# uzh-rpg/ess

Hardware: AMD Instinct MI355X
Metric: UDA train-step throughput (voxel grids/s = N*B*T/step_time) (higher is better)
Workload: dtype f16 forward / bf16 backward

## Files before the change

### ess_amd/copies.py

```python
import collections

import torch

_ATTR = 'ess_copies'


class Copies:
    __slots__ = ('stamp', 'c8', 'h16', 'f32c8', 'pair', 'mixed', 'unwritten')

    def __init__(self, stamp, unwritten):
        self.stamp, self.unwritten = stamp, unwritten
        self.c8 = self.h16 = self.f32c8 = self.pair = self.mixed = None


_NONE = collections.namedtuple('NoCopies', Copies.__slots__)(None, None, None, None, None, None, False)
_UNWRITTEN = _NONE._replace(unwritten=True)


def of(t):
    r = getattr(t, _ATTR, None)
    if r is None:
        return _NONE
    if r.stamp == t._version:
        return r
    return _UNWRITTEN if r.unwritten else _NONE


def attach(t, **fields):
    r = getattr(t, _ATTR, None)
    if r is None or r.stamp != t._version:
        r = Copies(t._version, r is not None and r.unwritten)
        setattr(t, _ATTR, r)
    for k, v in fields.items():
        setattr(r, k, v)
    return t


def placeholder(shape, device, **fields):
    return attach(torch.empty((), dtype=torch.float32, device=device).expand(*shape), unwritten=True, **fields)


def carry(dst, src, *names):
    r = of(src)
    found = {k: getattr(r, k) for k in names if getattr(r, k) is not None and getattr(r, k) is not False}
    return attach(dst, **found) if found else dst


def require_fp32(t):
    if of(t).unwritten:
        from .hip import EssHipError
        raise EssHipError('this tensor was produced as a BF16_C8 copy only (lean recurrent state / internal activation); '
                          'its fp32 values do not exist')
    return t
```

### ess_amd/csrc/conv_bf16.hip

```cpp
#include "conv_bf16_common.h"
#include <atomic>

namespace {

using namespace essconv;

__global__ void pack_weights_bf16_kernel(const float* w, const float* w2, __bf16* out, int64_t total, int cot, int ck,
                                         int n_chunks, int ks, int cin, int cout, int epi, int hid, int w_kind, int split, int f16) {
  const int64_t i = (int64_t)blockIdx.x * blockDim.x + threadIdx.x;
  if (i >= total) return;
  int64_t t = i;
  const int kp = t & 7; t >>= 3;
  const int col = t % cot; t /= cot;
  const int cb8 = ck >> 3;
  const int cb = t % cb8; t /= cb8;
  const int tap = t % (ks * ks); t /= ks * ks;
  int lo = 0;
  if (split) { lo = (int)(t & 1); t >>= 1; }
  const int ch = t % n_chunks;
  const int ct = t / n_chunks;
  const int c = ch * ck + cb * 8 + kp;
  int sel;
  const int row = map_row(ct * cot + col, epi, hid, cout, &sel);
  float v = 0.f;
// ... 205 lines not shown
bool wide_pick(const EssConvDesc* d, const EssConvPlan& pl, const Geom& g, const ConvKArgs& a, bool c8, WidePick* out) {
  if (d->epilogue != ESS_EPI_LINEAR) return wide_pick_recurrent(d, pl, g, a, c8, out);
  const int mode = wide_mode();
  if (!mode || !c8 || a.fmt_out != ESS_FMT_BF16_C8 || d->epilogue != ESS_EPI_LINEAR || a.out_bf) return false;
  const bool relu = d->act == ESS_ACT_RELU, res = a.residual != nullptr;
  if (!(d->act == ESS_ACT_NONE || relu)) return false;
  if (a.out_f16 && (relu || res)) return false;
  if (a.f16 && res) return false;
  if (d->out_split > 0 && (relu || res || a.out_f16 || (d->out_split & 15) || a.scale)) return false;
  const double kappa = tuning().kappa;
  const int mb = pl.cout_tile / 32;
  const int std_tiles = g.tiles_x * g.tiles_y * pl.n_cout_tiles * d->N;
  const double c_std = std_cost(std_tiles, pl.cout_tile, 2) * (mb == 1 ? tuning().narrow_tile : 1.0);
  const int cands[4][2] = {{2, 2}, {2, 1}, {1, 2}, {1, 1}};
  double best = 1e300;
  for (const auto& c : cands) {
    const int mbw = c[0], cw = c[1], cot = mbw * cw * 32;
    if ((mb == 2) != (cot >= 64) || mb > 2) continue;
    if (d->C_out % cot) continue;
    if (d->out_split > 0 && (d->out_split % (mbw * 32))) continue;
    int th, tw;
    conv_bf16_wide_tile(mbw, cw, &th, &tw);
    const int tx = ceil_div(d->W_out, tw), ty = ceil_div(d->H_out, th);
    const int tiles = tx * ty * (d->C_out / cot) * d->N;
    const double cost = kappa * ceil_div(tiles, tuning().cus) * (double)cot * th * tw;
    if (cost < best) { best = cost; *out = WidePick{mbw, cw, th, tx, ty, tiles}; }
  }
  if (best >= 1e300) return false;
  return mode >= 2 || best < c_std;
}
}

void conv_bf16_s2d_pick(const EssConvDesc* d, int* cw_out, int* tiles_out, int* tx_out, int* ty_out) {
  const int cus = tuning().cus;
  double best = 1e300;
  *cw_out = 0; *tiles_out = 0; *tx_out = 0; *ty_out = 0;
  for (int cw = 2; cw >= 1; --cw) {
    const int cot = 64 * cw;
    if (d->C_out % cot) continue;
    int th, tw;
    conv_bf16_wide_tile(2, cw, &th, &tw);
    const int tx = ceil_div(d->W_out, tw), ty = ceil_div(d->H_out, th);
    const int tiles = tx * ty * (d->C_out / cot) * d->N;
    const double cost = (double)ceil_div(tiles, cus) * cot * th * tw;
    if (cost < best) { best = cost; *cw_out = cw; *tiles_out = tiles; *tx_out = tx; *ty_out = ty; }
  }
}
bool conv_bf16_s2d_preferred(const EssConvDesc* d) {
  int cw, tiles, tx, ty;
  conv_bf16_s2d_pick(d, &cw, &tiles, &tx, &ty);
  return cw > 0 && 4 * tiles >= 3 * tuning().cus;
}

int conv_bf16_launch(const EssConvDesc* d, const EssConvPlan& pl, const Geom& g, const ConvKArgs& a, hipStream_t st) {
  ESS_CHECK_ARG(g.IH * g.IW <= kpc(d->ksize, d->stride) * 256, "conv(bf16): input tile of %d positions exceeds the staging capacity",
                g.IH * g.IW);
  ESS_CHECK_ARG((int64_t)(d->C0 > d->C1 ? d->C0 : d->C1) * d->H_in * d->W_in * 4 < (int64_t)1 << 31,
                "conv(bf16): one sample of a source must stay below 2 GiB (32-bit buffer offsets)");
  ESS_CHECK_ARG(d->C1 == 0 || (d->C0 % 8) == 0, "conv(bf16): the first source of a concat must have a multiple of 8 channels");
  const dim3 grid((unsigned)(g.tiles_x * g.tiles_y * pl.n_cout_tiles * d->N));
  const int mb = pl.cout_tile / 32;
  const bool c8 = a.fmt0 == ESS_FMT_BF16_C8;
  const bool split_generic = d->ksize == 3 && d->stride == 2 && d->epilogue == ESS_EPI_LINEAR;
  ESS_CHECK_ARG(!a.split || (((ws_enabled() && d->ksize == 3 && d->stride == 1 && pl.ck == 16) || is_paired(d) || split_generic) && !c8 && a.fmt_out == ESS_FMT_F32_NCHW),
                "conv(bf16): split operands run on the 3x3 / stride-1 wave-specialised, the 5x5 tap-paired and the 3x3 / stride-2 generic kernels with fp32 tensors");
  if (c8) ESS_CHECK_ARG((((uintptr_t)a.src0 | (uintptr_t)a.src1) & 15) == 0, "conv(bf16): BF16_C8 sources must be 16-byte aligned");
  if (a.f16)
    ESS_CHECK_ARG(c8 || (is_paired(d) && !a.residual && !a.split && conv_bf16_head_applies(d, pl)),
                  "conv(f16): sources must be F16_C8 tensors (fp32 NCHW only for the 2..5-channel 5x5 head)");
  if (a.f16) ESS_CHECK_ARG(!a.split && d->act != ESS_ACT_SUMPOOL2 && (a.fmt_out == ESS_FMT_F32_NCHW || d->out_split == 0 || d->epilogue != ESS_EPI_LINEAR),
                           "conv(f16): forward forms only");
  if (!c8 && !a.residual && conv_bf16_stem_applies(d, pl)) {
    conv_bf16_launch_stem(d, pl, st, a);
    return ess_launch_status("conv2d_forward(bf16, 7x7 stem)");
  }
  if (is_paired(d) && !c8 && !a.residual && !a.split && conv_bf16_head_applies(d, pl)) {
    conv_bf16_launch_head(d, pl, st, a);
    return ess_launch_status("conv2d_forward(bf16, 5x5 head)");
  }
  if (is_paired(d)) {
    const size_t lds2 = 2 * (size_t)pl.lds_bytes;
    ESS_CHECK_ARG(lds2 <= 160 * 1024, "conv(bf16, 5x5): two stages of %d B exceed the 160 KiB LDS", pl.lds_bytes);
    {
      static const int persist = [] { const char* e = getenv("ESS_WS_PERSIST"); return e ? atoi(e) : 1; }();
      const int by_regs = (d->stride == 2 && mb == 2) ? 1 : 2, by_lds = (int)((160 * 1024) / lds2);
      const int slots = tuning().cus * (by_regs < by_lds ? by_regs : by_lds);
      if (persist && (int)grid.x > slots) {
        ConvKArgs t = a;
        t.persist = 1;
        conv_bf16_launch_pair(d->stride, mb, c8, dim3((unsigned)slots), lds2, st, t);
        return ess_launch_status("conv2d_forward(bf16, tap-paired, persistent)");
      }
    }
    conv_bf16_launch_pair(d->stride, mb, c8, grid, lds2, st, a);
    return ess_launch_status("conv2d_forward(bf16, tap-paired)");
  }
  if (d->mode0 == ESS_SRC_S2D) {
    ESS_CHECK_ARG(c8 && a.fmt_out == ESS_FMT_BF16_C8 && !a.out_bf && !a.residual && !a.out_f16 && pl.ck == 16 && pl.cout_tile == 64 && (!a.hilo || (d->C_out % 64) == 0) &&
                      (d->act == ESS_ACT_NONE || d->act == ESS_ACT_RELU),
                  "conv(bf16, S2D): BF16_C8 in and out, no residual / copy, act in {none, relu}");
    const int cus = tuning().cus;
    int best_cw = 0, best_tiles = 0, best_tx = 0, best_ty = 0;
    conv_bf16_s2d_pick(d, &best_cw, &best_tiles, &best_tx, &best_ty);
    ESS_CHECK_ARG(best_cw > 0, "conv(bf16, S2D): C_out %d is not a multiple of 64", d->C_out);
    ConvKArgs t = a;
    t.tiles_x = best_tx; t.n_tiles = best_tx * best_ty;
    t.persist = best_tiles > cus ? 1 : 0;
    t.slab = pl.cout_tile;
    conv_bf16_launch_wide(2, best_cw, d->epilogue, dim3((unsigned)(best_tiles > cus ? cus : best_tiles)), st, t);
    return ess_launch_status("conv2d_forward(bf16, wide tile, space-to-depth 5x5/s2)");
  }
  static const bool poly_on = [] { const char* e = getenv("ESS_CONV_POLY"); return !(e && e[0] == '0'); }();
  if (poly_on && ws_enabled() && c8 && a.fmt_out == ESS_FMT_BF16_C8 && d->ksize == 3 && d->stride == 1 && d->pad == 1 && pl.ck == 16 &&
      d->mode0 == ESS_SRC_NEAREST_UP2 && d->C1 == 0 && d->epilogue == ESS_EPI_LINEAR && d->out_split == 0 && !a.out_bf &&
      (d->act == ESS_ACT_NONE || d->act == ESS_ACT_RELU) && (d->C_out % 32) == 0 && (d->C0 % 16) == 0 && !(d->H_in & 1) && !(d->W_in & 1) &&
      (pl.cout_tile == 32 || pl.cout_tile == 64)) {
    int th, tw, max_cin;
    conv_bf16_poly_tile(&th, &tw, &max_cin);
    if (d->C0 <= max_cin) {
    ConvKArgs t = a;
    t.Hin = d->H_in >> 1; t.Win = d->W_in >> 1;
    t.tiles_x = ceil_div(t.Win, tw);
    t.n_tiles = t.tiles_x * ceil_div(t.Hin, th);
    t.n_cout_tiles = d->C_out / 32;
    t.slab = pl.cout_tile;
    const int cus = tuning().cus, nct = t.n_cout_tiles, ptiles = t.n_tiles * d->N;
    int per_ct = cus / nct > 0 ? cus / nct : 1;
    if (per_ct > ptiles) per_ct = ptiles;
    t.persist = 1;
    conv_bf16_launch_poly(dim3((unsigned)(per_ct * nct)), st, t);
    return ess_launch_status("conv2d_forward(bf16, polyphase nearest-up2)");
    }
  }
  if (ws_enabled() && d->ksize == 3 && d->stride == 1 && pl.ck == 16) {
    const size_t lds2 = 2 * (size_t)pl.lds_bytes;
    WidePick wp;
    if (wide_pick(d, pl, g, a, c8, &wp)) {
      ConvKArgs t = a;
      t.tiles_x = wp.tiles_x; t.n_tiles = wp.tiles_x * wp.tiles_y;
      const int cus = tuning().cus;
      t.persist = wp.tiles > cus ? 1 : 0;
      t.slab = pl.cout_tile;
      conv_bf16_launch_wide(wp.mbw, wp.cw, d->epilogue, dim3((unsigned)(wp.tiles > cus ? cus : wp.tiles)), st, t);
      return ess_launch_status("conv2d_forward(bf16, wide tile)");
    }
    if (lds2 <= 160 * 1024) {
      static const int persist = [] { const char* e = getenv("ESS_WS_PERSIST"); return e ? atoi(e) : 1; }();
      const int per_cu_lds = (int)((160 * 1024) / lds2), per_cu = (mb == 4 ? 1 : 2) < per_cu_lds ? (mb == 4 ? 1 : 2) : per_cu_lds;
      const int slots = tuning().cus * per_cu;
      if (persist && (int)grid.x > slots) {
        ConvKArgs t = a;
        t.persist = 1;
        conv_bf16_launch_ws(mb, d->epilogue, c8, dim3((unsigned)slots), lds2, st, t);
        return ess_launch_status("conv2d_forward(bf16, wave-specialised, persistent)");
      }
      conv_bf16_launch_ws(mb, d->epilogue, c8, grid, lds2, st, a);
      return ess_launch_status("conv2d_forward(bf16, wave-specialised)");
    }
  }
  const int key = d->ksize * 10 + d->stride;
  ESS_CHECK_ARG(!a.split || split_generic, "conv(bf16): split operands reached the generic tile kernel (k%d s%d, %zu B of LDS for two stages)",
                d->ksize, d->stride, 2 * (size_t)pl.lds_bytes);
  if (c8)
    ESS_CHECK_ARG(d->epilogue == ESS_EPI_LINEAR && (key == 11 || key == 12 || key == 31 || key == 32),
                  "conv(bf16): the generic tile kernel stages BF16_C8 sources for 1x1 and 3x3 LINEAR convolutions only");
  ESS_CHECK_ARG(key == 11 || key == 12 || key == 31 || key == 32 || key == 51 || key == 52 || key == 71 || key == 72,
                "conv: no kernel for k%d s%d", d->ksize, d->stride);
  conv_bf16_launch_generic(key, mb, pl.ck / 8, d->epilogue, c8, grid, pl.lds_bytes, st, a);
  return ess_launch_status("conv2d_forward(bf16)");
}

}
```

### ess_amd/csrc/conv_bf16_wide.hip

```cpp
#include "conv_bf16_common.h"

namespace {

using namespace essconv;

__host__ __device__ constexpr int s2d_ntaps(int q) { return q == 0 ? 9 : (q == 3 ? 4 : 6); }
__host__ __device__ constexpr int s2d_class(int p, int nq) { return p < 2 * nq ? ((p & 1) ? 2 : 0) : ((p & 1) ? 3 : 1); }
__host__ __device__ constexpr int s2d_group(int p, int nq) { return (p < 2 * nq ? p : p - 2 * nq) >> 1; }
constexpr int WIDE_NB = 5;
constexpr int WIDE_RP = 32;
constexpr int WIDE_IW = 18;

template <int MBW, int CW, int EPI = ESS_EPI_LINEAR, bool S2D = false, bool H = false>
__global__ __launch_bounds__(512, 2) void conv_bf16_wide_kernel(const ConvKArgs a) {
  extern __shared__ __attribute__((aligned(16))) u32x4 smem16[];
  constexpr int KS = 3, CB8 = 2, CK = 16, NB = WIDE_NB, RP = WIDE_RP;
  constexpr int PW = 4 / CW;
  constexpr int TH = PW * NB * 2, TW = 16;
  constexpr int IH = TH + 2, IW = WIDE_IW;
  constexpr int PLANE = IH * RP;
  constexpr int COT = MBW * CW * 32;
  constexpr int WSZ = KS * KS * CB8 * COT;
  constexpr int WV = (WSZ + 255) / 256;
  constexpr int NPOS = IH * IW;
  constexpr int KPC = (NPOS + 255) / 256;
  constexpr int BUFSZ = CB8 * PLANE + WSZ;
  const int role = __builtin_amdgcn_readfirstlane(threadIdx.x >> 8);
  const int SLAB = a.slab;
  const int NSLAB = COT / SLAB;
  const int n_ct = a.n_cout_tiles / NSLAB;
  int t_start, t_count, t_first = 0, t_step = 1;
  if (a.persist) {
    const int total = n_ct * a.n_tiles * a.N, q = total >> 3, r = total & 7, xcd = (int)(blockIdx.x & 7);
    t_start = xcd < r ? xcd * (q + 1) : r * (q + 1) + (xcd - r) * q;
    t_count = q + (xcd < r ? 1 : 0);
    t_first = (int)(blockIdx.x >> 3);
    t_step = (int)(gridDim.x >> 3);
  } else {
    t_start = xcd_remap(blockIdx.x, gridDim.x);
    t_count = 1;
  }
#define ESS_TILE_LOOP for (int ti = t_first; ti < t_count; ti += t_step)
#define ESS_TILE_DECODE                                                    \
  const int logical = t_start + ti;                                        \
  const int ct = logical % n_ct;                                           \
  const int sp = logical / n_ct;                                           \
  const int tile = sp % a.n_tiles, n = sp / a.n_tiles;                     \
  const int ty = tile / a.tiles_x, tx = tile - ty * a.tiles_x;             \
  const int y0 = ty * TH, x0 = tx * TW;

  if (role == 1) {
    const int tid = threadIdx.x & 255;
    ESS_TILE_LOOP {
    ESS_TILE_DECODE
    const int iy0 = y0 - a.pad, ix0 = x0 - a.pad;
    const int sh0 = S2D ? 0 : (a.mode0 != ESS_SRC_DIRECT ? 1 : 0), sh1 = a.mode1 != ESS_SRC_DIRECT ? 1 : 0;
    const int Wp0 = S2D ? 2 * a.Win : (a.Win >> sh0), Wp1 = a.Win >> sh1;
    const size_t hw0 = S2D ? (size_t)4 * a.Hin * a.Win : (size_t)(a.Hin >> sh0) * Wp0, hw1 = (size_t)(a.Hin >> sh1) * Wp1;
    const int nb0 = S2D ? (a.C0 >> 5) : ((a.C0 + 7) >> 3), nb1 = (a.C1 + 7) >> 3;
    const int nq = S2D ? (a.n_chunks >> 2) : 1;
    const u32x4* s0 = (const u32x4*)a.src0 + (size_t)n * nb0 * hw0;
    const u32x4* s1 = a.C1 ? (const u32x4*)a.src1 + (size_t)n * nb1 * hw1 : s0;
    unsigned v_pos0[KPC], v_pos1[KPC], v_keep0[KPC], v_keep1[KPC];
    int v_lds[KPC];
#pragma unroll
    for (int k = 0; k < KPC; ++k) {
      const int vi = tid + k * 256;
// ... 201 lines not shown
  {
    ESS_READ_TAP(f0, 0, lds0)
    if constexpr (S2D) {
      const int nq = nch >> 2;
      for (int ch = 0; ch < 2 * nq; ch += 4) {
        ESS_CHUNK(f0, f1, ch)
        ESS_CHUNK6(f1, f0, ch + 1, 1, 3, 4, 6, 7)
        ESS_CHUNK(f1, f0, ch + 2)
        ESS_CHUNK6(f0, f1, ch + 3, 1, 3, 4, 6, 7)
      }
      for (int ch = 2 * nq; ch < nch; ch += 2) {
        ESS_CHUNK6(f0, f1, ch, 1, 2, 3, 4, 5)
        ESS_CHUNK4(f0, f1, ch + 1, 1, 3, 4)
      }
    } else {
    for (int ch = 0; ch < nch; ch += 2) {
      ESS_CHUNK(f0, f1, ch)
      if (ch + 1 < nch) ESS_CHUNK(f1, f0, ch + 1)
    }
    }
    asm volatile("s_waitcnt lgkmcnt(0)" ::: "memory");
  }
#undef ESS_CHUNK4
#undef ESS_CHUNK6
#undef ESS_CHUNK_TAIL_EVEN
#undef ESS_STEP
#undef ESS_READ_TS
#undef ESS_CHUNK
#undef ESS_TIE
#undef ESS_READ_TAP
#undef ESS_WAIT
#undef ESS_MMA
  __builtin_amdgcn_s_setprio(0);
#ifdef ESS_ABLATE
  if (a.deep & 8) continue;
#endif
  if constexpr (EPI == ESS_EPI_LSTM) {
    int pixi[NB];
#pragma unroll
    for (int nb = 0; nb < NB; ++nb) {
      const int y = y0 + ly[nb], x = x0 + ox;
      pixi[nb] = (y < a.Hout && x < a.Wout) ? y * a.Wout + x : -1;
    }
    conv_epilogue_lstm_c8<MBW, NB, H>(a, acc, ct_w, n, half, pixi, (unsigned)(a.Hout * a.Wout));
  } else if constexpr (EPI == ESS_EPI_GRU_UR || EPI == ESS_EPI_GRU_OUT) {
    int pixi[NB];
#pragma unroll
    for (int nb = 0; nb < NB; ++nb) {
      const int y = y0 + ly[nb], x = x0 + ox;
      pixi[nb] = (y < a.Hout && x < a.Wout) ? y * a.Wout + x : -1;
    }
    if constexpr (EPI == ESS_EPI_GRU_UR) conv_epilogue_gru_ur_c8<MBW, NB, H>(a, acc, ct_w, n, half, pixi, (unsigned)(a.Hout * a.Wout));
    else conv_epilogue_gru_out_c8<MBW, NB, H>(a, acc, ct_w, n, half, pixi, (unsigned)(a.Hout * a.Wout));
  } else {
    conv_epilogue_c8_wide<MBW, NB, H>(a, acc, ct_w, n, half, x0 + ox, y0, ly, biased);
  }
  }
#undef ESS_TILE_LOOP
#undef ESS_TILE_DECODE
}

template <int MBW, int CW, int EPI = ESS_EPI_LINEAR, bool S2D = false>
void launch_wide_t(dim3 grid, hipStream_t st, const ConvKArgs& a) {
  constexpr int PW = 4 / CW, TH = PW * WIDE_NB * 2, PLANE = (TH + 2) * WIDE_RP, COT = MBW * CW * 32;
  constexpr size_t lds = 2 * (size_t)(2 * PLANE + 9 * 2 * COT) * 16;
  static_assert(lds <= 160 * 1024, "two stages must fit the 160 KiB LDS");
  if (a.f16) {
    ess_allow_lds(conv_bf16_wide_kernel<MBW, CW, EPI, S2D, true>, lds);
    hipLaunchKernelGGL((conv_bf16_wide_kernel<MBW, CW, EPI, S2D, true>), grid, dim3(512), lds, st, a);
    return;
  }
  ess_allow_lds(conv_bf16_wide_kernel<MBW, CW, EPI, S2D>, lds);
  hipLaunchKernelGGL((conv_bf16_wide_kernel<MBW, CW, EPI, S2D>), grid, dim3(512), lds, st, a);
}

}

namespace essconv {

void conv_bf16_wide_tile(int mbw, int cw, int* th, int* tw) {
  *tw = 16;
  *th = (4 / cw) * WIDE_NB * 2;
  (void)mbw;
}

void conv_bf16_launch_wide(int mbw, int cw, int epi, dim3 grid, hipStream_t st, const ConvKArgs& a) {
  if (a.mode0 == ESS_SRC_S2D) {
    if (cw == 2) launch_wide_t<2, 2, ESS_EPI_LINEAR, true>(grid, st, a);
    else launch_wide_t<2, 1, ESS_EPI_LINEAR, true>(grid, st, a);
    return;
  }
  if (epi == ESS_EPI_LSTM) { launch_wide_t<2, 2, ESS_EPI_LSTM>(grid, st, a); return; }
  if (epi == ESS_EPI_GRU_UR) { launch_wide_t<2, 2, ESS_EPI_GRU_UR>(grid, st, a); return; }
  if (epi == ESS_EPI_GRU_OUT) { launch_wide_t<2, 2, ESS_EPI_GRU_OUT>(grid, st, a); return; }
  if (mbw == 2 && cw == 2) launch_wide_t<2, 2>(grid, st, a);
  else if (mbw == 2 && cw == 1) launch_wide_t<2, 1>(grid, st, a);
  else if (mbw == 1 && cw == 2) launch_wide_t<1, 2>(grid, st, a);
  else launch_wide_t<1, 1>(grid, st, a);
}

}
```

### ess_amd/csrc/conv_bf16_ws.hip

```cpp
#ifdef ESS_CV_TRACE
__device__ unsigned long long g_cv_trace[2048 * 8 * 48];
#define ESS_CT(i_) do { if ((threadIdx.x & 63) == 0 && blockIdx.x < 2048) g_cv_trace[(blockIdx.x * 8 + (threadIdx.x >> 6)) * 48 + (i_)] = __builtin_readcyclecounter(); } while (0)
#define ESS_EPI_STAMP(i_) ESS_CT(i_)
#define ESS_CW(i_) do { if ((threadIdx.x & 63) == 0 && blockIdx.x < 2048) g_cv_trace[(blockIdx.x * 8 + (threadIdx.x >> 6)) * 48 + (i_)] = wall_clock64(); } while (0)
#define ESS_SYNC_ACC(acc_) do { const unsigned long long t0_ = __builtin_readcyclecounter(); __syncthreads(); acc_ += __builtin_readcyclecounter() - t0_; } while (0)
#define ESS_CT_VAL(i_, v_) do { if ((threadIdx.x & 63) == 0 && blockIdx.x < 2048) g_cv_trace[(blockIdx.x * 8 + (threadIdx.x >> 6)) * 48 + (i_)] = (v_); } while (0)
#else
#define ESS_SYNC_ACC(acc_) __syncthreads()
#define ESS_CT_VAL(i_, v_) do { } while (0)
#define ESS_CW(i_) do { } while (0)
#define ESS_CT(i_) do { } while (0)
#endif
#include "conv_bf16_common.h"

namespace {

using namespace essconv;

template <int MB, int EPI, bool SRCBF, bool OUT8 = false, bool H = false>
__global__ __launch_bounds__(512, MB == 4 ? 2 : 4) void conv_bf16_ws_k3s1_kernel(const ConvKArgs a) {
  static_assert(!H || SRCBF, "half operands come as F16_C8 tensors");
  extern __shared__ __attribute__((aligned(16))) u32x4 smem16[];
  constexpr int KS = 3, CB8 = 2, CK = 16;
  constexpr int COT = MB * 32;
  constexpr int KPC = kpc(3, 1);
  constexpr int WSZ = KS * KS * CB8 * COT;
  constexpr int WV = (WSZ + 255) / 256;
  const int role = __builtin_amdgcn_readfirstlane(threadIdx.x >> 8);
  const int tid = threadIdx.x & 255, lane = tid & 63, wave = tid >> 6, half = lane >> 5, p = lane & 31;
  const int BW = 1 << a.bwl, WX = 1 << a.wxl, RB = 32 >> a.bwl;
  const int TW = WX << a.bwl, TH = (4 >> a.wxl) * NBW * RB;
  int t_start, t_count, t_first = 0, t_step = 1;
  if (a.persist) {
    const int total = a.n_cout_tiles * a.n_tiles * a.N, q = total >> 3, r = total & 7, xcd = (int)(blockIdx.x & 7);
    t_start = xcd < r ? xcd * (q + 1) : r * (q + 1) + (xcd - r) * q;
    t_count = q + (xcd < r ? 1 : 0);
    t_first = (int)(blockIdx.x >> 3);
    t_step = (int)(gridDim.x >> 3);
  } else {
    t_start = xcd_remap(blockIdx.x, gridDim.x);
    t_count = 1;
  }
#define ESS_TILE_LOOP for (int ti = t_first; ti < t_count; ti += t_step)
#define ESS_TILE_DECODE                                                    \
  const int logical = t_start + ti;                                        \
  const int ct = logical % a.n_cout_tiles;                                 \
  const int sp = logical / a.n_cout_tiles;                                 \
  const int tile = sp % a.n_tiles, n = sp / a.n_tiles;                     \
  const int ty = tile / a.tiles_x, tx = tile - ty * a.tiles_x;             \
  const int y0 = ty * TH, x0 = tx * TW;
  const int bufsz = CB8 * a.plane + WSZ;
  ESS_CT(0);
  ESS_CW(46);

  if (role == 1 && SRCBF) {
    ESS_TILE_LOOP {
    ESS_TILE_DECODE
    const int iy0 = y0 - a.pad, ix0 = x0 - a.pad;
    const int sh0 = a.mode0 != ESS_SRC_DIRECT ? 1 : 0, sh1 = a.mode1 != ESS_SRC_DIRECT ? 1 : 0;
    const int Wp0 = a.Win >> sh0, Wp1 = a.Win >> sh1;
    const size_t hw0 = (size_t)(a.Hin >> sh0) * Wp0, hw1 = (size_t)(a.Hin >> sh1) * Wp1;
    const int nb0 = (a.C0 + 7) >> 3, nb1 = (a.C1 + 7) >> 3;
    const u32x4* s0 = (const u32x4*)a.src0 + (size_t)n * nb0 * hw0;
    const u32x4* s1 = a.C1 ? (const u32x4*)a.src1 + (size_t)n * nb1 * hw1 : s0;
    unsigned v_pos0[KPC], v_pos1[KPC], v_keep0[KPC], v_keep1[KPC];
    int v_lds[KPC];
    const int npos = a.IH * a.IW;
#pragma unroll
    for (int k = 0; k < KPC; ++k) {
      const int vi = tid + k * 256;
      const int iy = vi / a.IW, ix = vi - iy * a.IW;
      const int gy = iy0 + iy, gx = ix0 + ix;
      const bool in = vi < npos && gy >= 0 && gy < a.Hin && gx >= 0 && gx < a.Win;
      const bool odd = ((gy | gx) & 1) != 0;
// ... 219 lines not shown
    if (ch < 40) ESS_CT(3 + ch);
    const unsigned stage_b = lds0 + (ch & 1) * buf_bytes;
    const unsigned wa = stage_b + w_off + a_base;
    unsigned ba[NBW][KS];
#pragma unroll
    for (int nb = 0; nb < NBW; ++nb)
#pragma unroll
      for (int ky = 0; ky < KS; ++ky) ba[nb][ky] = stage_b + b_base[nb][ky];
    Frags f0, f1;
#define ESS_READ_TAP(F_, TAP_)                                                                                                   \
    {                                                                                                                            \
      constexpr int ky_ = (TAP_) / KS, kx_ = (TAP_) % KS;                                                                        \
      _Pragma("unroll") for (int mb = 0; mb < MB; ++mb)                                                                          \
        asm volatile("ds_read_b128 %0, %1 offset:%2" : "=v"(F_.a[mb]) : "v"(wa + (unsigned)(mb * 32 * 16)), "n"((TAP_) * CB8 * COT * 16)); \
      _Pragma("unroll") for (int nb = 0; nb < NBW; ++nb)                                                                         \
        asm volatile("ds_read_b128 %0, %1 offset:%2" : "=v"(F_.b[nb]) : "v"(ba[nb][ky_]), "n"(kx_ * 16));                       \
    }
#define ESS_WAIT(F_, N_)                                                                                                         \
    {                                                                                                                            \
      if constexpr (MB == 1) asm volatile("s_waitcnt lgkmcnt(%3)" : "+v"(F_.a[0]), "+v"(F_.b[0]), "+v"(F_.b[1]) : "n"(N_));      \
      else if constexpr (MB == 2) asm volatile("s_waitcnt lgkmcnt(%4)" : "+v"(F_.a[0]), "+v"(F_.a[MB > 1 ? 1 : 0]), "+v"(F_.b[0]), "+v"(F_.b[1]) : "n"(N_)); \
      else asm volatile("s_waitcnt lgkmcnt(%6)" : "+v"(F_.a[0]), "+v"(F_.a[MB > 1 ? 1 : 0]), "+v"(F_.a[MB > 2 ? 2 : 0]), "+v"(F_.a[MB > 3 ? 3 : 0]), "+v"(F_.b[0]), "+v"(F_.b[1]) : "n"(N_)); \
    }
#define ESS_MMA(F_)                                                                                                              \
    _Pragma("unroll") for (int mb = 0; mb < MB; ++mb)                                                                            \
      _Pragma("unroll") for (int nb = 0; nb < NBW; ++nb)                                                                         \
        acc[mb][nb] = ess_mfma16<H>(F_.a[mb], F_.b[nb], acc[mb][nb]);
    constexpr int NR = MB + NBW;
#ifdef ESS_ABLATE
    if (a.deep & 2) { __syncthreads(); continue; }
#endif
    ESS_READ_TAP(f0, 0)
    ESS_READ_TAP(f1, 1) ESS_WAIT(f0, NR) ESS_MMA(f0)
    ESS_READ_TAP(f0, 2) ESS_WAIT(f1, NR) ESS_MMA(f1)
    ESS_READ_TAP(f1, 3) ESS_WAIT(f0, NR) ESS_MMA(f0)
    ESS_READ_TAP(f0, 4) ESS_WAIT(f1, NR) ESS_MMA(f1)
    ESS_READ_TAP(f1, 5) ESS_WAIT(f0, NR) ESS_MMA(f0)
    ESS_READ_TAP(f0, 6) ESS_WAIT(f1, NR) ESS_MMA(f1)
    ESS_READ_TAP(f1, 7) ESS_WAIT(f0, NR) ESS_MMA(f0)
    ESS_READ_TAP(f0, 8) ESS_WAIT(f1, NR) ESS_MMA(f1)
    ESS_WAIT(f0, 0) ESS_MMA(f0)
#undef ESS_READ_TAP
#undef ESS_WAIT
#undef ESS_MMA
    if (ch == nvc_c - 1) ESS_CT(44);
    ESS_SYNC_ACC(cbar_acc);
  }
  ESS_CT_VAL(42, cbar_acc);
  ESS_CT(45);
  __builtin_amdgcn_s_setprio(0);
#ifdef ESS_ABLATE
  if (a.deep & 8) continue;
#endif
  if constexpr (OUT8) conv_epilogue_c8<MB, H>(a, acc, ct, n, half, x0 + lx, y0, ly, biased);
  else conv_epilogue<MB, EPI, false, H>(a, acc, ct, n, half, x0 + lx, y0, ly, biased);
  ESS_CT(47);
  if constexpr (EPI != ESS_EPI_LSTM) ESS_CW(43);
  }
#undef ESS_TILE_LOOP
#undef ESS_TILE_DECODE
}


template <int MB, bool SRCBF>
void launch_ws(int epi, dim3 grid, size_t lds, hipStream_t st, const ConvKArgs& a) {
  if constexpr (SRCBF) {
    if (a.f16) {
#define ESS_WSH(E_, O8_) { ess_allow_lds(conv_bf16_ws_k3s1_kernel<MB, E_, true, O8_, true>, lds); hipLaunchKernelGGL((conv_bf16_ws_k3s1_kernel<MB, E_, true, O8_, true>), grid, dim3(512), lds, st, a); }
      if (a.fmt_out == ESS_FMT_BF16_C8) ESS_WSH(ESS_EPI_LINEAR, true)
      else if (epi == ESS_EPI_LSTM) ESS_WSH(ESS_EPI_LSTM, false)
      else if (epi == ESS_EPI_GRU_UR) ESS_WSH(ESS_EPI_GRU_UR, false)
      else if (epi == ESS_EPI_GRU_OUT) ESS_WSH(ESS_EPI_GRU_OUT, false)
      else ESS_WSH(ESS_EPI_LINEAR, false)
#undef ESS_WSH
      return;
    }
  }
  if (a.fmt_out == ESS_FMT_BF16_C8) {
    ess_allow_lds(conv_bf16_ws_k3s1_kernel<MB, ESS_EPI_LINEAR, SRCBF, true>, lds);
    hipLaunchKernelGGL((conv_bf16_ws_k3s1_kernel<MB, ESS_EPI_LINEAR, SRCBF, true>), grid, dim3(512), lds, st, a);
    return;
  }
#define ESS_WS(E_) { ess_allow_lds(conv_bf16_ws_k3s1_kernel<MB, E_, SRCBF>, lds); hipLaunchKernelGGL((conv_bf16_ws_k3s1_kernel<MB, E_, SRCBF>), grid, dim3(512), lds, st, a); }
  switch (epi) {
    case ESS_EPI_LSTM: ESS_WS(ESS_EPI_LSTM) break;
    case ESS_EPI_GRU_UR: ESS_WS(ESS_EPI_GRU_UR) break;
    case ESS_EPI_GRU_OUT: ESS_WS(ESS_EPI_GRU_OUT) break;
    default: ESS_WS(ESS_EPI_LINEAR) break;
  }
#undef ESS_WS
}
template <bool SRCBF>
void launch_ws_mb(int mb, int epi, dim3 grid, size_t lds, hipStream_t st, const ConvKArgs& a) {
  if (mb == 4) launch_ws<4, SRCBF>(epi, grid, lds, st, a);
  else if (mb == 2) launch_ws<2, SRCBF>(epi, grid, lds, st, a);
  else launch_ws<1, SRCBF>(epi, grid, lds, st, a);
}
}

namespace essconv {

void conv_bf16_launch_ws(int mb, int epi, bool c8, dim3 grid, size_t lds, hipStream_t st, const ConvKArgs& a) {
  if (c8) launch_ws_mb<true>(mb, epi, grid, lds, st, a);
  else launch_ws_mb<false>(mb, epi, grid, lds, st, a);
}

}

#ifdef ESS_CV_TRACE
extern "C" int ess_debug_conv_trace(unsigned long long* host_out, size_t n) {
  (void)hipMemset((void*)nullptr, 0, 0);
  return (int)hipMemcpyFromSymbol(host_out, HIP_SYMBOL(g_cv_trace), n * sizeof(unsigned long long));
}
extern "C" int ess_debug_conv_trace_clear() {
  void* p = nullptr;
  if (hipGetSymbolAddress(&p, HIP_SYMBOL(g_cv_trace)) != hipSuccess) return -1;
  return (int)hipMemset(p, 0, sizeof(unsigned long long) * 2048 * 8 * 48);
}
#endif
// ... 1 lines not shown
```

### ess_amd/csrc/conv_common.h

```cpp
#pragma once
#include "common.h"
#include <stdlib.h>

#ifndef ESS_EPI_AUX
#define ESS_EPI_AUX 2
#endif
#ifndef ESS_GRU_AUX
#define ESS_GRU_AUX 2
#endif
#ifndef ESS_C8_AUX
#define ESS_C8_AUX 0
#endif
namespace essconv {

constexpr int NBW = 2;

struct ConvKArgs {
  const float* src0;
  const float* src1;
  const void* wpk;
  const float* scale;
  const float* shift;
  const float* residual;
  const float* aux0;
  const float* aux1;
  float* out;
  float* out2;
  int N, Hin, Win, C0, C1, mode0, mode1;
  int Cout, Hout, Wout, pad;
  int bwl, wxl, tiles_x, n_tiles, n_cout_tiles;
  int IH, IW, row_pitch, par_off, plane;
  int ck, n_chunks;
  int act, hid, out_split;
  void* out_bf;
  int fmt0, fmt1;
  int fmt_out;
  int fmt_res;
  int out_f16;
  int persist;
  int slab;
  int split;
  int deep;
  int f16;
  int hilo;
};

template <bool H> __device__ __forceinline__ uint2 ess_cvt4(float v0, float v1, float v2, float v3);
template <bool H> __device__ __forceinline__ void ess_up4(uint2 r, float (&f)[4]);


#ifndef ESS_EPI_STAMP
#define ESS_EPI_STAMP(i_) do { } while (0)
#endif
typedef __amdgpu_buffer_rsrc_t ess_rsrc;
constexpr unsigned ESS_OOB = 0x80000000u;
__device__ __forceinline__ ess_rsrc ess_make_rsrc(const void* p, size_t bytes) {
  return __builtin_amdgcn_make_buffer_rsrc((void*)p, 0, (int)(unsigned)bytes, 0x00020000);
}
__device__ __forceinline__ _Float16 ess_f16_sat(float v) {
  const float c = __builtin_amdgcn_fmed3f(v, -65504.f, 65504.f);
  return (_Float16)(v != v ? v : c);
}
template <> __device__ __forceinline__ uint2 ess_cvt4<false>(float v0, float v1, float v2, float v3) {
  typedef __bf16 bf16x4 __attribute__((ext_vector_type(4)));
  bf16x4 b;
  b[0] = (__bf16)v0; b[1] = (__bf16)v1; b[2] = (__bf16)v2; b[3] = (__bf16)v3;
  return __builtin_bit_cast(uint2, b);
}
template <> __device__ __forceinline__ uint2 ess_cvt4<true>(float v0, float v1, float v2, float v3) {
  typedef _Float16 f16x4 __attribute__((ext_vector_type(4)));
  f16x4 h;
  h[0] = ess_f16_sat(v0); h[1] = ess_f16_sat(v1); h[2] = ess_f16_sat(v2); h[3] = ess_f16_sat(v3);
  return __builtin_bit_cast(uint2, h);
}
__device__ __forceinline__ uint2 ess_cvt4_lo(float v0, float v1, float v2, float v3) {
  typedef _Float16 f16x4 __attribute__((ext_vector_type(4)));
  f16x4 h;
  h[0] = (_Float16)(v0 - (float)ess_f16_sat(v0)); h[1] = (_Float16)(v1 - (float)ess_f16_sat(v1));
  h[2] = (_Float16)(v2 - (float)ess_f16_sat(v2)); h[3] = (_Float16)(v3 - (float)ess_f16_sat(v3));
  return __builtin_bit_cast(uint2, h);
}
template <> __device__ __forceinline__ void ess_up4<false>(uint2 r, float (&f)[4]) {
  typedef __bf16 bf16x4 __attribute__((ext_vector_type(4)));
  const bf16x4 b = __builtin_bit_cast(bf16x4, r);
#pragma unroll
  for (int i = 0; i < 4; ++i) f[i] = (float)b[i];
}
template <> __device__ __forceinline__ void ess_up4<true>(uint2 r, float (&f)[4]) {
  typedef _Float16 f16x4 __attribute__((ext_vector_type(4)));
  const f16x4 b = __builtin_bit_cast(f16x4, r);
#pragma unroll
  for (int i = 0; i < 4; ++i) f[i] = (float)b[i];
}
__device__ __forceinline__ float ess_bload(ess_rsrc r, unsigned voff, unsigned soff) {
  return __builtin_bit_cast(float, __builtin_amdgcn_raw_buffer_load_b32(r, (int)voff, (int)soff, 0));
}
__device__ __forceinline__ void ess_bstore(float v, ess_rsrc r, unsigned voff, unsigned soff) {
// ... 559 lines not shown
            ess_up4<H>(rr, rf);
#pragma unroll
            for (int i = 0; i < 4; ++i) v[nb][i] += rf[i];
          }
#pragma unroll
          for (int i = 0; i < 4; ++i) {
            if (relu) v[nb][i] = fmaxf(v[nb][i], 0.f);
            if (c0 + i >= c_out) v[nb][i] = 0.f;
          }
        }
        if (pool && blk < nb_first) {
#pragma unroll
          for (int i = 0; i < 4; ++i) {
            if (rows1) {
              v[0][i] = v[0][i] + v[1][i];
              v[0][i] += xor1(v[0][i]);
            } else {
#pragma unroll
              for (int nb = 0; nb < NBW; ++nb) {
                v[nb][i] = v[nb][i] + __shfl_xor(v[nb][i], BW, 64);
                v[nb][i] += xor1(v[nb][i]);
              }
            }
          }
        }
#pragma unroll
        for (int nb = 0; nb < NBW; ++nb) {
          if (H || a.out_f16) {
            pk[jj][nb] = ess_cvt4<true>(v[nb][0], v[nb][1], v[nb][2], v[nb][3]);
          } else {
            pk[jj][nb] = ess_cvt4<false>(v[nb][0], v[nb][1], v[nb][2], v[nb][3]);
          }
        }
      }
      const bool to1 = myblk < nb_first;
#pragma unroll
      for (int nb = 0; nb < NBW; ++nb) {
        const auto s0 = __builtin_amdgcn_permlane32_swap(pk[0][nb].x, pk[1][nb].x, false, false);
        const auto s1 = __builtin_amdgcn_permlane32_swap(pk[0][nb].y, pk[1][nb].y, false, false);
        const u32x4e vec = {s0[0], s1[0], s0[1], s1[1]};
        if (blk0 < nb_first) {
          const unsigned o = (to1 && st1_16[nb] != ESS_OOB) ? (unsigned)myblk * HW1 * 16u + st1_16[nb] : ESS_OOB;
          __builtin_amdgcn_raw_buffer_store_b128(vec, r_o1, (int)o, 0, 0);
        }
        if (split > 0 && blk0 + 1 >= nb_first) {
          const unsigned o = (!to1 && myblk < nb_all && pix16[nb] != ESS_OOB) ? (unsigned)(myblk - nb_first) * HW * 16u + pix16[nb] : ESS_OOB;
          __builtin_amdgcn_raw_buffer_store_b128(vec, r_o2, (int)o, 0, 0);
        }
      }
    }
  }
}

template <int MB, bool SC, bool SH, bool F16, bool RELU, bool RES, int NB, bool H = false, bool HILO = false>
__device__ __forceinline__ void conv_epilogue_c8_plain(const ConvKArgs& a, f32x16 (&acc)[MB][NB], int ct, int n, int half,
                                                       int x, int y0, const int (&ly)[NB]) {
  static_assert(!HILO || H, "a [hi | lo] output is a half tensor");
  typedef unsigned int u32x4e __attribute__((ext_vector_type(4)));
  constexpr int COT = MB * 32;
  const unsigned HW = (unsigned)(a.Hout * a.Wout);
  const int nblk = a.Cout >> 3;
  const ess_rsrc r_o = ess_make_rsrc((const char*)a.out + (size_t)n * (HILO ? 2 : 1) * nblk * HW * 16, (size_t)(HILO ? 2 : 1) * nblk * HW * 16);
  const ess_rsrc r_rs = ess_make_rsrc((const char*)(RES ? a.residual : a.out) + (size_t)n * nblk * HW * 16, RES ? (size_t)nblk * HW * 16 : 0);
  unsigned pix16[NB];
#pragma unroll
  for (int nb = 0; nb < NB; ++nb) {
    const int y = y0 + ly[nb];
    pix16[nb] = ((y < a.Hout) & (x < a.Wout)) ? (unsigned)(y * a.Wout + x) * 16u : ESS_OOB;
  }
#pragma unroll
  for (int mb = 0; mb < MB; ++mb) {
    const int rowbase = ct * COT + mb * 32;
    float4 scv[4], shv[4];
    u32x4e rva[2][NB];
    if constexpr (SC || SH || RES) {
      asm volatile("" ::: "memory");
#pragma unroll
      for (int j = 0; j < 4; ++j) {
        const int c0 = rowbase + j * 8 + 4 * half;
        if constexpr (SC) scv[j] = *(const float4*)(a.scale + c0);
        if constexpr (SH) shv[j] = *(const float4*)(a.shift + c0);
      }
      if constexpr (RES) {
#pragma unroll
        for (int jh = 0; jh < 2; ++jh)
#pragma unroll
          for (int nb = 0; nb < NB; ++nb) {
            const unsigned pl = (unsigned)((rowbase >> 3) + 2 * jh + half) * HW * 16u;
            rva[jh][nb] = __builtin_amdgcn_raw_buffer_load_b128(r_rs, (int)(pix16[nb] != ESS_OOB ? pl + pix16[nb] : ESS_OOB), 0, 0);
          }
      }
    }
#pragma unroll
    for (int jp = 0; jp < 4; jp += 2) {
      uint2 pk[2][NB];
      uint2 pl[HILO ? 2 : 1][HILO ? NB : 1];
      uint2 rr[2][NB];
      if constexpr (RES) {
#pragma unroll
        for (int nb = 0; nb < NB; ++nb) {
          const u32x4e rv = rva[jp >> 1][nb];
          const auto s0 = __builtin_amdgcn_permlane32_swap(rv[0], rv[2], false, false);
          const auto s1 = __builtin_amdgcn_permlane32_swap(rv[1], rv[3], false, false);
          rr[0][nb] = make_uint2(s0[0], s1[0]);
          rr[1][nb] = make_uint2(s0[1], s1[1]);
        }
      }
#pragma unroll
      for (int jj = 0; jj < 2; ++jj) {
        const int j = jp + jj;
#pragma unroll
        for (int nb = 0; nb < NB; ++nb) {
          float v[4];
#pragma unroll
          for (int i = 0; i < 4; ++i) v[i] = acc[mb][nb][4 * j + i];
          if constexpr (SC && SH) {
            v[0] = v[0] * scv[j].x + shv[j].x; v[1] = v[1] * scv[j].y + shv[j].y; v[2] = v[2] * scv[j].z + shv[j].z; v[3] = v[3] * scv[j].w + shv[j].w;
          } else if constexpr (SC) {
            v[0] *= scv[j].x; v[1] *= scv[j].y; v[2] *= scv[j].z; v[3] *= scv[j].w;
          } else if constexpr (SH) {
            v[0] += shv[j].x; v[1] += shv[j].y; v[2] += shv[j].z; v[3] += shv[j].w;
          }
          if constexpr (RES) {
            float rf[4];
            ess_up4<H>(rr[jj][nb], rf);
#pragma unroll
            for (int i = 0; i < 4; ++i) v[i] += rf[i];
          }
          if constexpr (RELU) {
#pragma unroll
            for (int i = 0; i < 4; ++i) v[i] = fmaxf(v[i], 0.f);
          }
          pk[jj][nb] = ess_cvt4<F16 || H>(v[0], v[1], v[2], v[3]);
          if constexpr (HILO) pl[jj][nb] = ess_cvt4_lo(v[0], v[1], v[2], v[3]);
        }
      }
      const unsigned plane = (unsigned)((rowbase >> 3) + jp + half) * HW * 16u;
#pragma unroll
      for (int nb = 0; nb < NB; ++nb) {
        const auto s0 = __builtin_amdgcn_permlane32_swap(pk[0][nb].x, pk[1][nb].x, false, false);
        const auto s1 = __builtin_amdgcn_permlane32_swap(pk[0][nb].y, pk[1][nb].y, false, false);
        const u32x4e vec = {s0[0], s1[0], s0[1], s1[1]};
        __builtin_amdgcn_raw_buffer_store_b128(vec, r_o, (int)(pix16[nb] != ESS_OOB ? plane + pix16[nb] : ESS_OOB), 0, ESS_C8_AUX);
        if constexpr (HILO) {
          const auto t0 = __builtin_amdgcn_permlane32_swap(pl[0][nb].x, pl[1][nb].x, false, false);
          const auto t1 = __builtin_amdgcn_permlane32_swap(pl[0][nb].y, pl[1][nb].y, false, false);
          const u32x4e vlo = {t0[0], t1[0], t0[1], t1[1]};
          __builtin_amdgcn_raw_buffer_store_b128(vlo, r_o, (int)(pix16[nb] != ESS_OOB ? plane + (unsigned)nblk * HW * 16u + pix16[nb] : ESS_OOB), 0, ESS_C8_AUX);
        }
      }
    }
  }
}

template <int MB, bool POOL, int NB>
__device__ __forceinline__ void conv_epilogue_c8_dgrad(const ConvKArgs& a, f32x16 (&acc)[MB][NB], int ct, int n, int half,
                                                       int x, int y0, const int (&ly)[NB]) {
  static_assert(!POOL || NB == 2, "the one-row pooled pairing assumes two pixel blocks per wave");
  typedef __bf16 bf16x4 __attribute__((ext_vector_type(4)));
  typedef unsigned int u32x4e __attribute__((ext_vector_type(4)));
  constexpr int COT = MB * 32;
  const unsigned HW = (unsigned)(a.Hout * a.Wout);
  const int split = a.out_split;
  const int nb_first = (split > 0 ? split : a.Cout) >> 3, nb_second = split > 0 ? (a.Cout - split) >> 3 : 0;
  const int Wl = a.Wout >> 1;
  const unsigned HW1 = POOL ? (unsigned)((a.Hout >> 1) * Wl) : HW;
  const ess_rsrc r_o1 = ess_make_rsrc((const char*)a.out + (size_t)n * nb_first * HW1 * 16, (size_t)nb_first * HW1 * 16);
  const ess_rsrc r_o2 = ess_make_rsrc(split > 0 ? (const char*)a.out2 + (size_t)n * nb_second * HW * 16 : (const char*)a.out,
                                      split > 0 ? (size_t)nb_second * HW * 16 : 0);
  unsigned pix16[NB];
#pragma unroll
  for (int nb = 0; nb < NB; ++nb) {
    const int y = y0 + ly[nb];
    pix16[nb] = ((y < a.Hout) & (x < a.Wout)) ? (unsigned)(y * a.Wout + x) * 16u : ESS_OOB;
  }
  unsigned st_pool = ESS_OOB;
  if constexpr (POOL) {
    const int y = y0 + ly[0];
    if ((y < a.Hout) & (x < a.Wout) & !(x & 1) & !(y & 1)) st_pool = (unsigned)((y >> 1) * Wl + (x >> 1)) * 16u;
  }
  auto xor1 = [](float f) {
    return __builtin_bit_cast(float, __builtin_amdgcn_update_dpp(0, __builtin_bit_cast(int, f), 0xB1, 0xf, 0xf, true));
  };
#pragma unroll
  for (int mb = 0; mb < MB; ++mb) {
    const int rowbase = ct * COT + mb * 32;
#pragma unroll
    for (int jp = 0; jp < 4; jp += 2) {
      const int blk0 = (rowbase >> 3) + jp;
      const bool first = blk0 < nb_first;
      if (POOL && first) {
        uint2 pk[2];
#pragma unroll
        for (int jj = 0; jj < 2; ++jj) {
          bf16x4 b;
#pragma unroll
          for (int i = 0; i < 4; ++i) {
            float p = acc[mb][0][4 * (jp + jj) + i] + acc[mb][1][4 * (jp + jj) + i];
            p += xor1(p);
            b[i] = (__bf16)p;
          }
// ... 85 lines not shown
    else conv_epilogue_c8_sel<MB, false, false, H>(a, acc, ct, n, half, x, y0, ly);
  }
  return;
#endif
  if (biased) {
    conv_epilogue_c8_impl<MB, false, false>(a, acc, ct, n, half, x, y0, ly);
  } else if (a.scale) {
    if (a.shift) conv_epilogue_c8_impl<MB, true, true>(a, acc, ct, n, half, x, y0, ly);
    else conv_epilogue_c8_impl<MB, true, false>(a, acc, ct, n, half, x, y0, ly);
  } else {
    if (a.shift) conv_epilogue_c8_impl<MB, false, true>(a, acc, ct, n, half, x, y0, ly);
    else conv_epilogue_c8_impl<MB, false, false>(a, acc, ct, n, half, x, y0, ly);
  }
}

template <int MB, bool SC, bool SH, int NB, bool H = false>
__device__ __forceinline__ void conv_epilogue_c8_wide_sel(const ConvKArgs& a, f32x16 (&acc)[MB][NB], int ct, int n, int half, int x,
                                                          int y0, const int (&ly)[NB]) {
  const bool relu = a.act == ESS_ACT_RELU, res = a.residual != nullptr;
  if constexpr (H) {
    if (a.hilo) {
      if (relu) conv_epilogue_c8_plain<MB, SC, SH, true, true, false, NB, true, true>(a, acc, ct, n, half, x, y0, ly);
      else conv_epilogue_c8_plain<MB, SC, SH, true, false, false, NB, true, true>(a, acc, ct, n, half, x, y0, ly);
    } else {
      if (relu) conv_epilogue_c8_plain<MB, SC, SH, true, true, false, NB, true>(a, acc, ct, n, half, x, y0, ly);
      else conv_epilogue_c8_plain<MB, SC, SH, true, false, false, NB, true>(a, acc, ct, n, half, x, y0, ly);
    }
    return;
  }
  if constexpr (!SC && !SH) {
    if (a.out_split > 0) { conv_epilogue_c8_dgrad<MB, false>(a, acc, ct, n, half, x, y0, ly); return; }
  }
  if (a.out_f16) {
    conv_epilogue_c8_plain<MB, SC, SH, true, false, false>(a, acc, ct, n, half, x, y0, ly);
  } else if (res) {
    if (relu) conv_epilogue_c8_plain<MB, SC, SH, false, true, true>(a, acc, ct, n, half, x, y0, ly);
    else conv_epilogue_c8_plain<MB, SC, SH, false, false, true>(a, acc, ct, n, half, x, y0, ly);
  } else {
    if (relu) conv_epilogue_c8_plain<MB, SC, SH, false, true, false>(a, acc, ct, n, half, x, y0, ly);
    else conv_epilogue_c8_plain<MB, SC, SH, false, false, false>(a, acc, ct, n, half, x, y0, ly);
  }
}
template <int MB, int NB, bool H = false>
__device__ __forceinline__ void conv_epilogue_c8_wide(const ConvKArgs& a, f32x16 (&acc)[MB][NB], int ct, int n, int half, int x,
                                                      int y0, const int (&ly)[NB], bool biased) {
  if (biased) {
    conv_epilogue_c8_wide_sel<MB, false, false, NB, H>(a, acc, ct, n, half, x, y0, ly);
  } else if (a.scale) {
    if (a.shift) conv_epilogue_c8_wide_sel<MB, true, true, NB, H>(a, acc, ct, n, half, x, y0, ly);
    else conv_epilogue_c8_wide_sel<MB, true, false, NB, H>(a, acc, ct, n, half, x, y0, ly);
  } else {
    if (a.shift) conv_epilogue_c8_wide_sel<MB, false, true, NB, H>(a, acc, ct, n, half, x, y0, ly);
    else conv_epilogue_c8_wide_sel<MB, false, false, NB, H>(a, acc, ct, n, half, x, y0, ly);
  }
}

template <int MB, int NB, bool H = false>
__device__ __forceinline__ void conv_epilogue_lstm_c8(const ConvKArgs& a, f32x16 (&acc)[MB][NB], int ct, int n, int half,
                                                      const int (&pixi)[NB], unsigned HW) {
  typedef unsigned int u32x4c __attribute__((ext_vector_type(4)));
  const int nbh = a.hid >> 3;
  const int ncp = (H && a.hilo) ? 2 : 1;
  const size_t state_b = (size_t)nbh * HW * 32;
  const ess_rsrc r_prev = ess_make_rsrc(a.aux0 ? (const char*)(a.aux0 + (size_t)n * nbh * 8 * HW) : (const char*)a.out2, a.aux0 ? state_b : 0);
  const ess_rsrc r_c = ess_make_rsrc(a.out2 + (size_t)n * nbh * 8 * HW, state_b);
  const ess_rsrc r_h = ess_make_rsrc(a.out ? a.out + (size_t)n * nbh * 8 * HW : a.out2, a.out ? state_b : 0);
  const ess_rsrc r_hb = ess_make_rsrc(a.out_bf ? (const char*)a.out_bf + (size_t)n * ncp * nbh * HW * 16 : (const char*)a.out2, a.out_bf ? (size_t)ncp * nbh * HW * 16 : 0);
  unsigned vo[MB][NB];
  u32x4c cp[MB][NB];
#pragma unroll
  for (int mb = 0; mb < MB; ++mb)
#pragma unroll
    for (int nb = 0; nb < NB; ++nb) {
      vo[mb][nb] = pixi[nb] >= 0 ? ((unsigned)(ct * MB + mb) * HW + (unsigned)pixi[nb]) * 32u + 16u * half : ESS_OOB;
      cp[mb][nb] = __builtin_amdgcn_raw_buffer_load_b128(r_prev, (int)vo[mb][nb], 0, ESS_EPI_AUX);
    }
  __builtin_amdgcn_sched_barrier(0);
  float igc[MB][NB][4], gf[MB][NB][4], go[MB][NB][4];
#pragma unroll
  for (int mb = 0; mb < MB; ++mb)
#pragma unroll
    for (int nb = 0; nb < NB; ++nb)
#pragma unroll
      for (int jj = 0; jj < 4; ++jj) {
        igc[mb][nb][jj] = ess_sigmoid(acc[mb][nb][jj]) * ess_tanh(acc[mb][nb][12 + jj]);
        gf[mb][nb][jj] = ess_sigmoid(acc[mb][nb][4 + jj]);
        go[mb][nb][jj] = ess_sigmoid(acc[mb][nb][8 + jj]);
      }
  float hn[MB][NB][4];
#pragma unroll
  for (int mb = 0; mb < MB; ++mb)
#pragma unroll
    for (int nb = 0; nb < NB; ++nb) {
      u32x4c cv;
#pragma unroll
      for (int jj = 0; jj < 4; ++jj) {
        const float cprev = __builtin_bit_cast(float, (unsigned)cp[mb][nb][jj]);
        const float cn = gf[mb][nb][jj] * cprev + igc[mb][nb][jj];
        cv[jj] = __builtin_bit_cast(unsigned, cn);
        hn[mb][nb][jj] = go[mb][nb][jj] * ess_tanh(cn);
      }
      __builtin_amdgcn_raw_buffer_store_b128(cv, r_c, (int)vo[mb][nb], 0, ESS_EPI_AUX);
    }
  if (a.out) {
#pragma unroll
    for (int mb = 0; mb < MB; ++mb)
// ... 435 lines not shown
__device__ __forceinline__ int map_row(int prow, int epi, int hid, int cout, int* sel) {
  *sel = 0;
  if (epi == ESS_EPI_LSTM) {
    const int b = prow >> 5, q = (prow & 31) >> 3, j = prow & 7;
    const int hc = b * 8 + j;
    return hc < hid ? q * hid + hc : -1;
  }
  if (epi == ESS_EPI_GRU_UR) {
    const int b = prow >> 5, q = (prow & 31) >> 3, j = prow & 7;
    const int hc = b * 16 + (q >> 1) * 8 + j;
    *sel = q & 1;
    return hc < hid ? hc : -1;
  }
  return prow < cout ? prow : -1;
}

static __global__ void pack_weights_kernel(const float* w, const float* w2, float* out, int64_t total, int cot, int ck,
                                    int n_chunks, int ks, int cin, int cout, int epi, int hid, int w_kind) {
  const int64_t i = (int64_t)blockIdx.x * blockDim.x + threadIdx.x;
  if (i >= total) return;
  int64_t t = i;
  const int col = t % cot; t /= cot;
  const int cb = t % ck; t /= ck;
  const int tap = t % (ks * ks); t /= ks * ks;
  const int ch = t % n_chunks;
  const int ct = t / n_chunks;
  const int c = ch * ck + cb;
  int sel;
  const int row = map_row(ct * cot + col, epi, hid, cout, &sel);
  float v = 0.f;
  if (row >= 0 && c < cin) {
    const int ky = tap / ks, kx = tap - ky * ks;
    const float* src = sel ? w2 : w;
    if (w_kind == ESS_W_CONV) {
      v = src[(((size_t)row * cin + c) * ks + ky) * ks + kx];
    } else {
      const int rows_src = (epi == ESS_EPI_GRU_UR) ? hid : cout;
      v = src[(((size_t)c * rows_src + row) * ks + (ks - 1 - ky)) * ks + (ks - 1 - kx)];
    }
  }
  out[i] = v;
}

static __global__ void pack_rows_kernel(const float* v, const float* v2, float fill, float* out, int rows_padded, int epi,
                                 int hid, int cout) {
  const int i = blockIdx.x * blockDim.x + threadIdx.x;
  if (i >= rows_padded) return;
  int sel;
  const int row = map_row(i, epi, hid, cout, &sel);
  out[i] = row >= 0 ? (sel ? v2[row] : v[row]) : fill;
}


int conv_bf16_launch(const EssConvDesc* d, const EssConvPlan& pl, const Geom& g, const ConvKArgs& a, hipStream_t st);
int conv_bf16_pack_weights(const EssConvDesc* d, const EssConvPlan& pl, int w_kind, const float* w, const float* w2, void* packed,
                           hipStream_t st, bool split = false, bool f16 = false);
int conv_bf16_pack_weights_multi(const EssConvDesc* descs, const int32_t* kinds, const float* const* w, void* const* packed, int count,
                                 hipStream_t st);
void conv_bf16_s2d_pick(const EssConvDesc* d, int* cw, int* tiles, int* tiles_x, int* tiles_y);
bool conv_bf16_s2d_preferred(const EssConvDesc* d);

}
```

### ess_amd/csrc/conv_fwd.hip

```cpp
#include "conv_common.h"

namespace {

using namespace essconv;

constexpr int kpc32(int ks, int s) { return stage_kpc(ks, s); }
constexpr unsigned OOB32 = 0x80000000u;

template <int KS, int S, int MB, int EPI, int CB>
__global__ __launch_bounds__(256) void conv_f32_kernel(const ConvKArgs a) {
  extern __shared__ __attribute__((aligned(16))) float smem[];
  constexpr int COT = MB * 32;
  constexpr int KPC = kpc32(KS, S);
  constexpr int WSZ = KS * KS * CB * COT;
  constexpr int WV = (WSZ / 4 + 255) / 256;
  const int tid = threadIdx.x, lane = tid & 63, wave = tid >> 6, half = lane >> 5, p = lane & 31;
  const int BW = 1 << a.bwl, WX = 1 << a.wxl, RB = 32 >> a.bwl;
  const int TW = WX << a.bwl, TH = (4 >> a.wxl) * NBW * RB;
  const int logical = xcd_remap(blockIdx.x, gridDim.x);
  const int ct = logical % a.n_cout_tiles;
  const int sp = logical / a.n_cout_tiles;
  const int tile = sp % a.n_tiles, n = sp / a.n_tiles;
  const int ty = tile / a.tiles_x, tx = tile - ty * a.tiles_x;
  const int y0 = ty * TH, x0 = tx * TW;
// ... 137 lines not shown
  if (rc) return rc;
  ESS_CHECK_ARG(plan != nullptr, "conv: null plan");
  const ResolvedDesc rd = resolve_compute(d);
  make_plan(&rd.d, plan, rd.split);
  return ESS_OK;
}

extern "C" int ess_conv2d_s2d_preferred(const EssConvDesc* d) {
  if (validate(d) != ESS_OK || d->mode0 != ESS_SRC_S2D) return 0;
  return conv_bf16_s2d_preferred(d) ? 1 : 0;
}

extern "C" int ess_conv2d_pack_weights(const EssConvDesc* d, int w_kind, const float* w, const float* w2, void* packed,
                                       ess_stream_t stream) {
  int rc = validate(d);
  if (rc) return rc;
  ESS_CHECK_ARG(w && packed, "pack_weights: null pointer");
  ESS_CHECK_ARG(d->epilogue != ESS_EPI_GRU_UR || w2, "pack_weights: GRU_UR needs the reset-gate weight as w2");
  ESS_CHECK_ARG(w_kind == ESS_W_CONV || w_kind == ESS_W_TRANSPOSED || w_kind == ESS_W_CONV5_S2D, "pack_weights: bad w_kind");
  ESS_CHECK_ARG((w_kind == ESS_W_CONV5_S2D) == (d->mode0 == ESS_SRC_S2D), "pack_weights: ESS_W_CONV5_S2D goes with an ESS_SRC_S2D descriptor, and only with one");
  const ResolvedDesc rd = resolve_compute(d);
  d = &rd.d;
  EssConvPlan pl;
  make_plan(d, &pl, rd.split);
  if (is_bf16(d)) return conv_bf16_pack_weights(d, pl, w_kind, w, w2, packed, (hipStream_t)stream, rd.split, rd.f16);
  const int64_t total = pl.packed_elems;
  hipLaunchKernelGGL(pack_weights_kernel, dim3((unsigned)ceil_div64(total, 256)), dim3(256), 0, (hipStream_t)stream, w, w2,
                     (float*)packed, total, pl.cout_tile, pl.ck, pl.n_chunks, d->ksize, d->C0 + d->C1, d->C_out, d->epilogue,
                     d->hidden, w_kind);
  return ess_launch_status("pack_weights");
}

extern "C" int ess_conv2d_pack_weights_multi(const EssConvDesc* descs, const int32_t* w_kinds, const float* const* w,
                                             void* const* packed, int32_t count, ess_stream_t stream) {
  ESS_CHECK_ARG(descs && w_kinds && w && packed && count > 0, "pack_weights_multi: bad arguments");
  return conv_bf16_pack_weights_multi(descs, w_kinds, w, packed, count, (hipStream_t)stream);
}

extern "C" int ess_conv2d_pack_rows(const EssConvDesc* d, const float* v, const float* v2, float fill, float* packed,
                                    ess_stream_t stream) {
  int rc = validate(d);
  if (rc) return rc;
  ESS_CHECK_ARG(v && packed, "pack_rows: null pointer");
  ESS_CHECK_ARG(d->epilogue != ESS_EPI_GRU_UR || v2, "pack_rows: GRU_UR needs the reset-gate vector as v2");
  const ResolvedDesc rd = resolve_compute(d);
  d = &rd.d;
  EssConvPlan pl;
  make_plan(d, &pl, rd.split);
  hipLaunchKernelGGL(pack_rows_kernel, dim3(ceil_div(pl.rows_padded, 256)), dim3(256), 0, (hipStream_t)stream, v, v2, fill,
                     packed, pl.rows_padded, d->epilogue, d->hidden, d->C_out);
  return ess_launch_status("pack_rows");
}

extern "C" int ess_conv2d_forward(const EssConvDesc* d, const void* src0, const void* src1, const void* packed_w,
                                  const float* scale, const float* shift, const void* residual, const float* aux0,
                                  const float* aux1, void* out, void* out2, void* out_bf16, ess_stream_t stream) {
  EssConvDesc dcopy;
  bool out_f16 = false;
  if (d && d->fmt_out == ESS_FMT_F16_C8 && d->compute != ESS_COMPUTE_F16) {
    ESS_CHECK_ARG(d->act != ESS_ACT_SUMPOOL2 && d->out_split == 0 && (d->fmt_res == ESS_FMT_F32_NCHW || d->fmt_res == ESS_FMT_BF16_C8),
                  "conv: an F16_C8 output takes no SUMPOOL2 / out_split; a residual comes as BF16_C8");
    dcopy = *d;
    dcopy.fmt_out = ESS_FMT_BF16_C8;
    if (residual) dcopy.fmt_res = ESS_FMT_BF16_C8;
    d = &dcopy;
    out_f16 = true;
  }
  int rc = validate(d);
  if (rc) return rc;
  const ResolvedDesc rd = resolve_compute(d);
  d = &rd.d;
  ESS_CHECK_ARG(src0 && packed_w, "conv: null pointer");
  ESS_CHECK_ARG(d->mode0 != ESS_SRC_S2D || (d->fmt0 == ESS_FMT_BF16_C8 && d->fmt_out == ESS_FMT_BF16_C8), "conv: an ESS_SRC_S2D source is a BF16_C8 tensor, and so is the output");
  ESS_CHECK_ARG(out || (out_bf16 && d->out_split == 0 && (d->epilogue == ESS_EPI_LINEAR || d->epilogue == ESS_EPI_LSTM || d->epilogue == ESS_EPI_GRU_OUT)),
                "conv: `out` may only be NULL when the BF16_C8 copy is requested (LINEAR / LSTM / GRU_OUT epilogues)");
  ESS_CHECK_ARG(d->C1 == 0 || src1, "conv: second source missing");
  if (d->epilogue != ESS_EPI_LINEAR) ESS_CHECK_ARG(shift && !scale && !residual, "conv: a recurrent epilogue takes a bias (shift) and no scale / residual");
  if (d->epilogue == ESS_EPI_LSTM) ESS_CHECK_ARG(out2, "conv: the LSTM epilogue needs the second output (c')");
  if (d->epilogue == ESS_EPI_GRU_UR) ESS_CHECK_ARG(out2 || out_bf16 || !aux0, "conv: GRU_UR needs an output for r*h (out2 or out_bf16)");
  if (d->epilogue == ESS_EPI_GRU_OUT) ESS_CHECK_ARG(aux1, "conv: GRU_OUT needs u (aux1); h_prev (aux0) may be NULL = zeros");
  if (d->out_split > 0) ESS_CHECK_ARG(out2, "conv: out_split needs out2");
  if (out_bf16)
    ESS_CHECK_ARG(d->compute == ESS_COMPUTE_BF16 && d->out_split == 0, "conv: the BF16_C8 output copy exists for bf16 compute, no out_split");
  if (d->act == ESS_ACT_SUMPOOL2)
    ESS_CHECK_ARG(out && !scale && !residual && !out_bf16, "conv: SUMPOOL2 takes no scale / residual / BF16_C8 copy");
  if (d->fmt_out == ESS_FMT_BF16_C8) {
    ESS_CHECK_ARG(out && !out_bf16, "conv: a BF16_C8 output goes to `out` (no separate copy)");
    ESS_CHECK_ARG(((((uintptr_t)out) | ((uintptr_t)out2) | ((uintptr_t)residual)) & 15) == 0, "conv: BF16_C8 tensors must be 16-byte aligned");
  }
  ESS_CHECK_ARG(!residual || d->fmt_res == d->fmt_out, "conv: the residual must come in the output's format");
  EssConvPlan pl;
  make_plan(d, &pl, rd.split);
  ESS_CHECK_ARG(pl.lds_bytes <= 160 * 1024, "conv: LDS tile %d B exceeds 160 KiB", pl.lds_bytes);
  if (d->epilogue == ESS_EPI_GRU_UR && d->act == ESS_GRU_U_F16 && d->fmt_out == ESS_FMT_F32_C8)
    ESS_CHECK_ARG(shift && d->fmt0 == ESS_FMT_BF16_C8 && (d->hidden % (pl.cout_tile / 2)) == 0 && out && !out2 && (!aux0 || d->fmt_res == ESS_FMT_F32_C8),
                  "conv(GRU_UR): an F16_C8 update gate (ESS_GRU_U_F16 with channel-blocked outputs) needs BF16_C8 sources, a bias, hidden %% %d == 0, "
                  "no fp32 r*h output and a channel-blocked h_prev", pl.cout_tile / 2);
  const Geom g = choose_geom(d);
  ConvKArgs a{};
  a.src0 = (const float*)src0; a.src1 = (const float*)src1; a.wpk = packed_w;
  a.out_bf = out_bf16; a.fmt0 = d->fmt0; a.fmt1 = d->C1 ? d->fmt1 : d->fmt0; a.scale = scale; a.shift = shift; a.residual = (const float*)residual;
  a.aux0 = aux0; a.aux1 = aux1; a.out = (float*)out; a.out2 = (float*)out2; a.fmt_out = d->fmt_out; a.fmt_res = d->fmt_res;
#ifdef ESS_ABLATE
  { static const int abl = [] { const char* b = getenv("ESS_WS_ABL"); return b ? atoi(b) & ~1 : 0; }(); a.deep = abl; }
#endif
  a.out_f16 = out_f16 ? 1 : 0;
  a.split = rd.split ? 1 : 0;
  a.f16 = rd.f16 ? 1 : 0;
  a.hilo = rd.hilo ? 1 : 0;
  if (rd.hilo && d->epilogue == ESS_EPI_LINEAR)
    ESS_CHECK_ARG(!residual && (d->C_out % pl.cout_tile) == 0 && d->fmt_out == ESS_FMT_BF16_C8, "conv(f16): a [hi | lo] output takes no residual and whole channel tiles");
  if (rd.hilo && d->epilogue == ESS_EPI_GRU_OUT)
    ESS_CHECK_ARG(out_bf16 && shift && d->fmt_res == ESS_FMT_F32_C8 && aux1 && (!out || d->fmt_out == ESS_FMT_F32_C8) && (d->hidden % pl.cout_tile) == 0,
                  "conv(f16, GRU_OUT): a [hi | lo] copy of h' exists in the straight-line form only (channel-blocked states, whole tiles of hidden channels)");
  if (rd.hilo && d->epilogue == ESS_EPI_LSTM)
    ESS_CHECK_ARG(out_bf16 && shift && d->fmt_out == ESS_FMT_F32_C8 && (!aux0 || d->fmt_res == ESS_FMT_F32_C8) && (d->hidden % (8 * (pl.cout_tile / 32))) == 0 && pl.cout_tile >= 64,
                  "conv(f16, LSTM): a [hi | lo] copy of h' exists in the lean form only (channel-blocked cell states, whole hidden blocks per tile)");
  a.N = d->N; a.Hin = d->H_in; a.Win = d->W_in; a.C0 = d->C0; a.C1 = d->C1; a.mode0 = d->mode0; a.mode1 = d->mode1;
  a.Cout = d->C_out; a.Hout = d->H_out; a.Wout = d->W_out; a.pad = d->pad;
  a.bwl = g.bwl; a.wxl = g.wxl; a.tiles_x = g.tiles_x; a.n_tiles = g.tiles_x * g.tiles_y; a.n_cout_tiles = pl.n_cout_tiles;
  a.IH = g.IH; a.IW = g.IW; a.row_pitch = g.row_pitch; a.par_off = g.par_off; a.plane = g.plane;
  a.ck = pl.ck; a.n_chunks = pl.n_chunks; a.act = d->act; a.hid = d->hidden; a.out_split = d->out_split;
  hipStream_t st = (hipStream_t)stream;
  if (is_bf16(d)) return conv_bf16_launch(d, pl, g, a, st);
  ESS_CHECK_ARG(g.IH * g.IW <= kpc32(d->ksize, d->stride) * 256, "conv: input tile of %d positions exceeds the staging capacity",
                g.IH * g.IW);
  ESS_CHECK_ARG((int64_t)(d->C0 > d->C1 ? d->C0 : d->C1) * d->H_in * d->W_in * 4 < (int64_t)1 << 31,
                "conv: one sample of a source must stay below 2 GiB (32-bit buffer offsets)");
  const dim3 grid((unsigned)(g.tiles_x * g.tiles_y * pl.n_cout_tiles * d->N));
  const int mb = pl.cout_tile / 32;
  const int key = d->ksize * 10 + d->stride;
  switch (key) {
    case 11: launch_mb<1, 1>(mb, pl.ck, d->epilogue, grid, pl.lds_bytes, st, a); break;
    case 12: launch_mb<1, 2>(mb, pl.ck, d->epilogue, grid, pl.lds_bytes, st, a); break;
    case 31: launch_mb<3, 1>(mb, pl.ck, d->epilogue, grid, pl.lds_bytes, st, a); break;
    case 32: launch_mb<3, 2>(mb, pl.ck, d->epilogue, grid, pl.lds_bytes, st, a); break;
    case 51: launch_mb<5, 1>(mb, pl.ck, d->epilogue, grid, pl.lds_bytes, st, a); break;
    case 52: launch_mb<5, 2>(mb, pl.ck, d->epilogue, grid, pl.lds_bytes, st, a); break;
    case 71: launch_mb<7, 1>(mb, pl.ck, d->epilogue, grid, pl.lds_bytes, st, a); break;
    case 72: launch_mb<7, 2>(mb, pl.ck, d->epilogue, grid, pl.lds_bytes, st, a); break;
    default: ess_set_error("conv: no kernel for k%d s%d", d->ksize, d->stride); return ESS_ENOTSUP;
  }
  return ess_launch_status("conv2d_forward");
}
```

### ess_amd/csrc/norm_c8.hip

```cpp
#include <atomic>
#include "common.h"
#include <stdlib.h>

#ifndef ESS_REDUCE1_U
#define ESS_REDUCE1_U 4
#endif
namespace {

typedef unsigned int u32x4n __attribute__((ext_vector_type(4)));
typedef __bf16 bf16x8n __attribute__((ext_vector_type(8)));

__device__ __forceinline__ void unpack8(u32x4n v, float (&f)[8]) {
#pragma unroll
  for (int q = 0; q < 4; ++q) {
    f[2 * q] = __builtin_bit_cast(float, v[q] << 16);
    f[2 * q + 1] = __builtin_bit_cast(float, v[q] & 0xffff0000u);
  }
}
__device__ __forceinline__ void unpack8h(u32x4n v, float (&f)[8]) {
  typedef _Float16 f16x2n __attribute__((ext_vector_type(2)));
#pragma unroll
  for (int q = 0; q < 4; ++q) {
    const unsigned w = v[q];
    const f16x2n h = __builtin_bit_cast(f16x2n, w);
// ... 367 lines not shown
#pragma unroll
          for (int j = 0; j < 8; ++j) { p0[j] += f[j]; p1[j] = fmaf(f[j], f[j], p1[j]); }
        } else {
          float gg[8], yy[8];
          unpack8(gv[u], gg);
          if (relu && relu_from_y) unpack8(yv[u], yy);
#pragma unroll
          for (int j = 0; j < 8; ++j) {
            const float xh = (f[j] - mean[j]) * rstd[j];
            const bool off = relu && (relu_from_y ? yy[j] <= 0.f : (affine_mask ? f[j] * ma[j] + mb[j] <= 0.f : xh <= 0.f));
            const float gr = off ? 0.f : gg[j];
            p0[j] += gr;
            p1[j] = fmaf(gr, xh, p1[j]);
          }
        }
      }
#pragma unroll
      for (int j = 0; j < 8; ++j) { s0[j] += (double)p0[j]; s1[j] += (double)p1[j]; }
    }
  }
  const int lane = threadIdx.x & 63, w = threadIdx.x >> 6;
#pragma unroll
  for (int j = 0; j < 8; ++j) {
    const double a = wave_sum_d(s0[j]), b = wave_sum_d(s1[j]);
    if (lane == 0) { redd[w * 16 + 2 * j] = a; redd[w * 16 + 2 * j + 1] = b; }
  }
  __syncthreads();
  if (threadIdx.x < 16) {
    double t = 0;
    for (int i = 0; i < 4; ++i) t += redd[i * 16 + threadIdx.x];
    sums[((size_t)g * nsl + sl) * 16 + threadIdx.x] = t;
  }
}

__device__ __forceinline__ void group_total8(const double* sums, int g, int nsl, double (&t0)[8], double (&t1)[8]) {
  __shared__ double part[64 * 16];
  __shared__ double tot[16];
  const int j = threadIdx.x & 15, k0 = threadIdx.x >> 4, ng = blockDim.x >> 4;
  {
    const double* p = sums + (size_t)g * nsl * 16 + j;
    double t = 0;
    for (int k = k0; k < nsl; k += ng) t += p[(size_t)k * 16];
    part[k0 * 16 + j] = t;
  }
  __syncthreads();
  if (threadIdx.x < 16) {
    double t = 0;
    for (int i = 0; i < ng; ++i) t += part[i * 16 + threadIdx.x];
    tot[threadIdx.x] = t;
  }
  __syncthreads();
#pragma unroll
  for (int jj = 0; jj < 8; ++jj) { t0[jj] = tot[2 * jj]; t1[jj] = tot[2 * jj + 1]; }
}

__global__ __launch_bounds__(256) void in_apply_c8_kernel(const u32x4n* __restrict__ x, const u32x4n* __restrict__ res,
                                                          u32x4n* __restrict__ y, float* __restrict__ stats, const double* sums,
                                                          int nsl, int CB, int C, int hw, float eps, int relu) {
  const int xf16 = relu >> 8;
  relu &= 0xff;
  const int g = blockIdx.x, n = g / CB, cb = g - n * CB;
  double t0[8], t1[8];
  group_total8(sums, g, nsl, t0, t1);
  float mean[8], rstd[8];
#pragma unroll
  for (int j = 0; j < 8; ++j) {
    const double m = t0[j] / hw;
    double var = t1[j] / hw - m * m;
    if (var < 0) var = 0;
    mean[j] = (float)m;
    rstd[j] = (float)(1.0 / sqrt(var + (double)eps));
  }
  if (blockIdx.y == 0 && threadIdx.x == 0) {
#pragma unroll
    for (int j = 0; j < 8; ++j)
      if (cb * 8 + j < C) { stats[2 * ((size_t)n * C + cb * 8 + j)] = mean[j]; stats[2 * ((size_t)n * C + cb * 8 + j) + 1] = rstd[j]; }
  }
  const size_t base = (size_t)g * hw;
  constexpr int U = 4;
  const int stride = gridDim.y * 256;
  for (int i = blockIdx.y * 256 + threadIdx.x; i < hw; i += stride * U) {
    u32x4n xv[U], rv[U];
#pragma unroll
    for (int u = 0; u < U; ++u) {
      const int ii = i + u * stride, ic = ii < hw ? ii : hw - 1;
      xv[u] = x[base + ic];
      if (res) rv[u] = res[base + ic];
    }
#pragma unroll
    for (int u = 0; u < U; ++u) {
      const int ii = i + u * stride;
      if (ii >= hw) continue;
      float f[8], rf[8];
      unpack8x(xv[u], f, xf16);
      if (res) unpack8(rv[u], rf);
#pragma unroll
      for (int j = 0; j < 8; ++j) {
        float t = (f[j] - mean[j]) * rstd[j];
        if (relu) t = fmaxf(t, 0.f);
        if (res) t += rf[j];
        f[j] = cb * 8 + j < C ? t : 0.f;
      }
      y[base + ii] = pack8n(f);
    }
  }
}
// ... 376 lines not shown
  }
  int rc = need_ws(workspace, ess_norm_workspace_c8(groups), workspace_bytes, "instnorm_backward_c8");
  if (rc) return rc;
  const int nsl = split_for8(groups, hw);
  hipLaunchKernelGGL((c8_reduce_kernel<1>), dim3(groups, nsl), dim3(256), 0, st, xs, nullptr, gs, stats, (double*)workspace, hw, 1, 0, CB,
                     C, 1, relu, 0, nullptr, nullptr, xcb);
  hipLaunchKernelGGL(in_bwd_apply_c8_kernel, dim3(groups, chunks_for8(groups, hw)), dim3(256), 0, st, xs, gs, stats,
                     (const double*)workspace, nsl, ds, CB, C, hw, relu, xcb);
  return ess_launch_status("instnorm_backward_c8(split)");
}

extern "C" int ess_batchnorm_train_forward_c8(const void* x, const void* residual, const float* gamma, const float* beta,
                                              float* running_mean, float* running_var, float momentum, float eps, void* y,
                                              float* stats, int32_t N, int32_t C, int32_t hw, int32_t relu, int32_t x_f16, void* workspace,
                                              size_t workspace_bytes, ess_stream_t stream) {
  ESS_CHECK_ARG(x && gamma && beta && y && stats && N > 0 && C > 0 && hw > 0, "batchnorm_train_forward_c8: bad arguments");
  ESS_CHECK_ARG((running_mean == nullptr) == (running_var == nullptr), "batchnorm_train_forward_c8: running stats come in pairs");
  ESS_CHECK_ARG(al16(x, residual, y), "batchnorm_train_forward_c8: BF16_C8 tensors must be 16-byte aligned");
  hipStream_t st = (hipStream_t)stream;
  relu = (relu & 1) | (x_f16 ? 0x100 : 0);
  const int CB = (C + 7) / 8;
  int rc = need_ws(workspace, ess_norm_workspace_c8(CB), workspace_bytes, "batchnorm_train_forward_c8");
  if (rc) return rc;
  const int nsl = split_for8(CB, hw);
  hipLaunchKernelGGL((c8_reduce_kernel<0>), dim3(CB, nsl), dim3(256), 0, st, (const u32x4n*)x, nullptr, nullptr, nullptr,
                     (double*)workspace, hw, N, CB, CB, C, 0, relu & 0x100, 0);
  hipLaunchKernelGGL(bn_apply_c8_kernel, dim3(N * CB, chunks_for8(N * CB, hw)), dim3(256), 0, st, (const u32x4n*)x,
                     (const u32x4n*)residual, gamma, beta, running_mean, running_var, momentum, eps, (u32x4n*)y, stats,
                     (const double*)workspace, nsl, N, CB, C, hw, relu);
  return ess_launch_status("batchnorm_train_forward_c8");
}

extern "C" int ess_batchnorm_train_backward_c8(const void* x, const void* y, const void* dy, const float* gamma, const float* beta,
                                               const float* stats, void* dx, void* d_residual, float* dgamma, float* dbeta,
                                               int32_t accumulate, int32_t N, int32_t C, int32_t hw, int32_t relu, int32_t x_f16,
                                               void* workspace, size_t workspace_bytes, ess_stream_t stream) {
  const bool mask_x = (relu & 1) && beta != nullptr;
  ESS_CHECK_ARG(x && (y || mask_x || !(relu & 1)) && dy && gamma && stats && N > 0 && C > 0 && hw > 0, "batchnorm_train_backward_c8: bad arguments");
  ESS_CHECK_ARG(!(mask_x && d_residual), "batchnorm_train_backward_c8: a residual gradient needs the mask of the saved output (beta must be NULL)");
  ESS_CHECK_ARG(al16(x, y, dy, dx, d_residual), "batchnorm_train_backward_c8: BF16_C8 tensors must be 16-byte aligned");
  hipStream_t st = (hipStream_t)stream;
  relu = (relu & 1) | (x_f16 ? 0x100 : 0);
  const int CB = (C + 7) / 8;
  int rc = need_ws(workspace, ess_norm_workspace_c8(CB), workspace_bytes, "batchnorm_train_backward_c8");
  if (rc) return rc;
  const int nsl = split_for8(CB, hw);
  hipLaunchKernelGGL((c8_reduce_kernel<1>), dim3(CB, nsl), dim3(256), 0, st, (const u32x4n*)x, (const u32x4n*)y, (const u32x4n*)dy,
                     stats, (double*)workspace, hw, N, CB, CB, C, 0, relu, mask_x ? 0 : 1, mask_x ? gamma : nullptr, mask_x ? beta : nullptr);
  hipLaunchKernelGGL(bn_bwd_apply_c8_kernel, dim3(N * CB, chunks_for8(N * CB, hw)), dim3(256), 0, st, (const u32x4n*)x,
                     (const u32x4n*)y, (const u32x4n*)dy, gamma, stats, (const double*)workspace, nsl, (u32x4n*)dx,
                     (u32x4n*)d_residual, dgamma, dbeta, accumulate, N, CB, C, hw, relu, mask_x ? beta : nullptr);
  return ess_launch_status("batchnorm_train_backward_c8");
}
```

### ess_amd/functional.py

```python
import os
import weakref

import torch

from . import copies, hip

DIRECT_GRAD_ACCUM = False

class direct_grad_accum:

    def __init__(self, on):
        self.on = bool(on)

    def __enter__(self):
        global DIRECT_GRAD_ACCUM
        self.prev, DIRECT_GRAD_ACCUM = DIRECT_GRAD_ACCUM, self.on

    def __exit__(self, *a):
        global DIRECT_GRAD_ACCUM
        DIRECT_GRAD_ACCUM = self.prev


def _direct(p):
    return DIRECT_GRAD_ACCUM and getattr(p, '_ess_direct_grad', False) and p.is_leaf and p.grad is not None and p.grad.is_contiguous()
# ... 140 lines not shown


def packed_weight(spec, w, w2=None, kind=hip.W_CONV):
    return derived((w,) if w2 is None else (w, w2), ('pack', spec.key, kind),
                   lambda: hip.pack_weights(spec, w.detach(), None if w2 is None else w2.detach(), kind))


def packed_rows(spec, v, v2=None):
    def build():
        pr = hip.pack_rows(spec, v.detach(), None if v2 is None else v2.detach())
        pr.ess_spec = spec
        return pr
    return derived((v,) if v2 is None else (v, v2), ('rows', spec.plan.rows_padded, spec.desc.epilogue), build)


def columns(weight, cols):
    cols = tuple(cols)
    tf = FIRST_COLUMNS if len(cols) == 1 and cols[0][0] == 0 else REPEATED_COLUMNS

    def build():
        with torch.no_grad():
            w = weight.detach()
            return torch.cat([w[:, a:b] for (a, b) in cols], dim=1).contiguous()
    return derived((weight,), ('cols', cols), build, tf)


def _virt(x, mode):
    m = 2 if mode != hip.SRC_DIRECT else 1
    return x.shape[2] * m, x.shape[3] * m


def _blocked(x):
    return hip.is_c8(x)


def _channels(x):
    return x.shape[1] * 8 if _blocked(x) else x.shape[1]


def _fmt(x):
    return hip.FMT_BF16_C8 if hip.is_c8(x) else hip.FMT_F32_NCHW


PRE_NORM = 'f16'
PRE_NORM_HILO = 'f16hilo'


def mixed():
    return hip.mixed()


def half_of(x):
    return copies.of(x).h16 or (hip.bf16_c8_to_f16_c8(x.detach().contiguous()), False)


def _hilo_placeholder(N, C, H, W, device, buf):
    return copies.attach(torch.empty((), dtype=torch.bfloat16, device=device).expand(N, C // 8, H, W, 8), pair=buf)


def _empty_act(N, C, H, W, device, c8):
    if c8:
        if C % 8:
            raise hip.EssHipError(f'a BF16_C8 activation needs a multiple of 8 channels, got {C}')
        return hip.f16_c8_empty(N, C, H, W, device) if c8 == PRE_NORM else hip.bf16_c8_empty(N, C, H, W, device)
    return torch.empty(N, C, H, W, dtype=torch.float32, device=device)


def pre_norm_fmt():
    import os
    if not c8_mode():
        return False
    return PRE_NORM if os.environ.get('ESS_PRE_NORM_F16', '1')[:1] != '0' else True


def c8_mode():
    return hip.get_compute() == 'bf16'


class ToC8Fn(torch.autograd.Function):

    @staticmethod
    def forward(ctx, x):
        ctx.C = x.shape[1]
        return hip.to_bf16_c8(x.contiguous())

    @staticmethod
    def backward(ctx, dy):
        return hip.from_bf16_c8(dy.contiguous(), ctx.C)


class FromC8Fn(torch.autograd.Function):
    @staticmethod
    def forward(ctx, x, C):
        return hip.from_bf16_c8(x.contiguous(), C)

    @staticmethod
    def backward(ctx, dy):
        return hip.to_bf16_c8(dy.contiguous()), None


def as_c8(x, want_hilo=False):
    if hip.is_c8(x):
        return x
    if x.shape[1] % 8:
        raise hip.EssHipError(f'as_c8: {x.shape[1]} channels are not a whole number of 8-channel blocks')
    if hip.mixed() and not x.requires_grad:
# ... 14 lines not shown
        copies.attach(c8t, h16=h)
        copies.attach(x, mixed=(c8t, want_hilo))
        return c8t
    r = copies.of(x)
    if r.c8 is not None and not x.requires_grad:
        return r.c8
    if r.unwritten:
        raise hip.EssHipError('as_c8: the tensor was produced as a staging copy only and the copy is gone (modified / detached without '
                              'detach_keep_c8): its fp32 values were never written')
    return ToC8Fn.apply(x)


def from_c8(x, C=None):
    return FromC8Fn.apply(x, x.shape[1] * 8 if C is None else C) if hip.is_c8(x) else x


def detach_keep_c8(x):
    return copies.carry(x.detach(), x, 'c8', 'h16', 'unwritten')


class ForkFn(torch.autograd.Function):

    @staticmethod
    def forward(ctx, x, n):
        ctx.set_materialize_grads(False)
        return tuple(copies.carry(x.detach(), x, 'h16') for _ in range(n))

    @staticmethod
    def backward(ctx, *gs):
        gs = [g.contiguous() for g in gs if g is not None]
        if not gs:
            return None, None
        acc = gs[0]
        if acc.dtype == torch.bfloat16:
            i = 1
            while i < len(gs):
                acc = hip.add_bf16(acc, gs[i], gs[i + 1] if i + 1 < len(gs) else None)
                i += 2
        else:
            for g in gs[1:]:
                acc = hip.add(acc, g)
        return acc, None


def fork(x, n=2):
    if n == 1 or not (torch.is_grad_enabled() and x.requires_grad):
        return (x,) * n
    return ForkFn.apply(x, n)


class Conv2dFn(torch.autograd.Function):

    @staticmethod
    def forward(ctx, x0, x1, weight, bias, stride, pad, mode0, mode1, passthrough=False, out_c8=None, half=False):
        c8in = hip.is_c8(x0)
        if x1 is not None and hip.is_c8(x1) != c8in:
            raise hip.EssHipError('Conv2dFn: the two sources must use the same storage format')
        if out_c8 is None:
            out_c8 = c8in
        N, C0 = x0.shape[0], _channels(x0)
        C1 = _channels(x1) if x1 is not None else 0
        Hv, Wv = _virt(x0, mode0)
        if x1 is not None and _virt(x1, mode1) != (Hv, Wv):
            raise hip.EssHipError('Conv2dFn: the two sources disagree on the (virtual) extent')
        Cout, k = weight.shape[0], weight.shape[2]
        if weight.shape[1] != C0 + C1:
            raise hip.EssHipError(f'Conv2dFn: weight expects {weight.shape[1]} input channels, got {C0}+{C1}')
        spec = hip.conv_spec(N, Hv, Wv, C0, C1, Cout, k, stride, pad, mode0, mode1)
        if half and c8in and hip.mixed():
            h0, hl0 = half_of(x0)
            h1, hl1 = half_of(x1) if x1 is not None else (None, False)
            fspec = hip.conv_spec(N, Hv, Wv, C0 * (2 if hl0 else 1), C1 * (2 if hl1 else 1), Cout, k, stride, pad, mode0, mode1,
                                  compute=hip.COMPUTE_F16)
            cols = [(0, C0)] * (2 if hl0 else 1) + ([(C0, C0 + C1)] * (2 if hl1 else 1) if C1 else [])
            pw = packed_weight(fspec, columns(weight, cols) if (hl0 or hl1) else weight)
            shift = packed_rows(fspec, bias) if bias is not None else None
            if out_c8 == PRE_NORM_HILO and Cout % fspec.plan.cout_tile:
                out_c8 = PRE_NORM
            if out_c8 == PRE_NORM_HILO:
                buf = hip.f16_blocks_empty(N, Cout, spec.H_out, spec.W_out, x0.device, hilo=True)
                hip.conv_forward_h16(fspec, h0, h1, pw, None, shift, out=buf, out_fmt=hip.FMT_F16_C8_HILO)
                out = _hilo_placeholder(N, Cout, spec.H_out, spec.W_out, x0.device, buf)
            elif out_c8 == PRE_NORM:
                out = hip.f16_c8_empty(N, Cout, spec.H_out, spec.W_out, x0.device)
                hip.conv_forward_h16(fspec, h0, h1, pw, None, shift, out=out.view(torch.float16), out_fmt=hip.FMT_F16_C8)
            elif not out_c8:
                out = torch.empty(N, Cout, spec.H_out, spec.W_out, dtype=torch.float32, device=x0.device)
                hip.conv_forward_h16(fspec, h0, h1, pw, None, shift, out=out, out_fmt=hip.FMT_F32_NCHW)
            else:
                raise hip.EssHipError('Conv2dFn(mixed): a half-operand convolution writes a pre-norm tensor or fp32 NCHW')
        else:
            if out_c8 == PRE_NORM_HILO:
                out_c8 = PRE_NORM
            shift = packed_rows(spec, bias) if bias is not None else None
            out = _empty_act(N, Cout, spec.H_out, spec.W_out, x0.device, out_c8)
            hip.conv_forward(spec, x0, x1, packed_weight(spec, weight), None, shift, out=out, src_fmt=_fmt(x0),
                             out_fmt=hip.FMT_F16_C8 if out_c8 == PRE_NORM else _fmt(out))
        ctx.spec = spec
        ctx.has_x1, ctx.has_bias = x1 is not None, bias is not None
        ctx.bias_ref = weakref.ref(bias) if bias is not None else None
        ctx.save_for_backward(x0, x1, weight)
        ctx.passthrough = passthrough
        return (out, x0) if passthrough else out

    @staticmethod
    def backward(ctx, dy, d_skip=None):
        x0, x1, weight = ctx.saved_tensors
        spec = ctx.spec
        (N, Hv, Wv, C0, C1, mode0, mode1, Cout, k, s, p, _, _, _, _, _) = spec.key
        dy = dy.contiguous()
        c8in = hip.is_c8(x0)
        need0, need1, needw, needb = ctx.needs_input_grad[0], ctx.needs_input_grad[1] and ctx.has_x1, \
            ctx.needs_input_grad[2], ctx.needs_input_grad[3] and ctx.has_bias
        d0 = d1 = dw = db = None
        if need0 or need1:
            split = C0 if C1 > 0 else 0
            wd, c_dg = weight, C0 + C1
            if C1 > 0 and need0 and not need1:
                wd, c_dg, split = columns(weight, [(0, C0)]), C0, 0
            pool0 = s == 1 and need0 and mode0 == hip.SRC_NEAREST_UP2 and (C1 == 0 or mode1 == hip.SRC_DIRECT) and \
                not (Hv & 1) and not (Wv & 1)
            if c8in and ((mode0 == hip.SRC_NEAREST_UP2 and need0 and not pool0) or (mode1 == hip.SRC_NEAREST_UP2 and need1)):
                raise hip.EssHipError('Conv2dFn(BF16_C8): only the first source may be nearest-upsampled (pooled data-gradient)')
            if s == 1:
                dspec = hip.conv_spec(N, spec.H_out, spec.W_out, Cout, 0, c_dg, k, 1, k - 1 - p, out_split=split,
                                      act=hip.ACT_SUMPOOL2 if pool0 else hip.ACT_NONE)
            else:
                if (Hv & 1) or (Wv & 1):
                    raise hip.EssHipError('data-gradient of a stride-2 conv needs even input extents')
                dspec = hip.conv_spec(N, 2 * spec.H_out, 2 * spec.W_out, Cout, 0, c_dg, k, 1, k - 1 - p,
                                      mode0=hip.SRC_ZERO_UP2, out_split=split)
            assert (dspec.H_out, dspec.W_out) == (Hv, Wv), (dspec.H_out, dspec.W_out, Hv, Wv)
            dv0 = _empty_act(N, C0, Hv // 2 if (s == 1 and pool0) else Hv, Wv // 2 if (s == 1 and pool0) else Wv, dy.device, c8in)
            dv1 = _empty_act(N, C1, Hv, Wv, dy.device, c8in) if split > 0 else None
            fuse_skip = d_skip is not None and need0 and C1 == 0 and mode0 == hip.SRC_DIRECT
            hip.conv_forward(dspec, dy, None, packed_weight(dspec, wd, kind=hip.W_TRANSPOSED),
                             residual=d_skip.contiguous() if fuse_skip else None, out=dv0, out2=dv1, src_fmt=_fmt(dy),
                             out_fmt=_fmt(dv0))
            if fuse_skip:
                d_skip = None
            if need0:
                d0 = hip.sumpool2x2(dv0) if (mode0 == hip.SRC_NEAREST_UP2 and not (s == 1 and pool0)) else dv0
            if need1:
                d1 = hip.sumpool2x2(dv1) if mode1 == hip.SRC_NEAREST_UP2 else dv1
        s2_1x1 = s == 2 and k == 1 and C1 == 0 and mode0 == hip.SRC_DIRECT and not (Hv & 1) and not (Wv & 1)
        s2_lib = s == 2 and k == 3 and p == 1 and c8in and C1 == 0 and mode0 == hip.SRC_DIRECT and not (Hv & 1) and not (Wv & 1)
        direct = needw and _direct(weight) and (not (s == 2 and k == 3) or s2_lib)
        if direct:
            bias = ctx.bias_ref() if ctx.bias_ref is not None else None
            db_t = bias.grad if (needb and bias is not None and _direct(bias)) else None
            if needb and db_t is None:
                direct = False
        if direct:
            if s2_1x1 and not c8in:
                sp1 = hip.conv_spec(N, Hv // 2, Wv // 2, C0, 0, Cout, 1, 1, 0)
                hip.conv_wgrad(sp1, x0[:, :, ::2, ::2].contiguous(), None, dy, weight.grad, db_t, accumulate=True)
                done = True
            else:
                done = True
                defer = WGRAD_DEFER is not None and c8in and hip.is_c8(dy) and k == 3 and s == 1 and p == 1
                held = WGRAD_DEFER.pop(id(weight), None) if defer else None
                if held is not None and held[0].key == spec.key and held[4] is weight:
                    hip.conv_wgrad_sets(spec, [(held[1], held[2], held[3]), (x0, x1, dy)], weight.grad, db_t, accumulate=True)
                elif defer and held is None and WGRAD_STASHING:
                    WGRAD_DEFER[id(weight)] = (spec, x0, x1, dy, weight, db_t)
                    done = False
                else:
                    if held is not None:
                        hip.conv_wgrad(held[0], held[1], held[2], held[3], weight.grad, held[5], accumulate=True)
                    hip.conv_wgrad(spec, x0, x1, dy, weight.grad, db_t, accumulate=True)
            dw = db = None
            if done and GRAD_READY_HOOK is not None:
                GRAD_READY_HOOK(weight)
        elif needw or needb:
            dw = torch.empty_like(weight)
            db = torch.empty(Cout, dtype=torch.float32, device=dy.device) if ctx.has_bias else None
            if s == 2 and C1 == 0 and mode0 == hip.SRC_DIRECT and not (Hv & 1) and not (Wv & 1) and not s2_lib and \
                    ((k == 3 and p == 1) or (k == 1 and p == 0 and not c8in)):
                _wgrad_stride2_by_phases(x0, dy, dw, db, k)
            else:
                hip.conv_wgrad(spec, x0, x1, dy, dw, db)
            if not needw:
                dw = None
            if not needb:
                db = None
            if dw is not None and _direct(weight) and (db is None or (ctx.bias_ref is not None and ctx.bias_ref() is not None and _direct(ctx.bias_ref()))):
                hip.add(weight.grad, dw, out=weight.grad)
                if db is not None:
                    hip.add(ctx.bias_ref().grad, db, out=ctx.bias_ref().grad)
                dw = db = None
                if GRAD_READY_HOOK is not None:
                    GRAD_READY_HOOK(weight)
        if d_skip is not None and need0:
            d0 = d_skip if d0 is None else (hip.add_bf16(d0, d_skip.contiguous()) if c8in else hip.add(d0, d_skip.contiguous()))
        return d0, d1, dw, db, None, None, None, None, None, None, None


def _wgrad_stride2_by_phases(x, dy, dw, db, k):
    N, C, H, W = x.shape[0], _channels(x), x.shape[2], x.shape[3]
    Cout = _channels(dy)
    Ho, Wo = H // 2, W // 2
    if k == 1:
        spec = hip.conv_spec(N, Ho, Wo, C, 0, Cout, 1, 1, 0)
        hip.conv_wgrad(spec, x[:, :, ::2, ::2].contiguous(), None, dy, dw, db)
        return
    spec = hip.conv_spec(N, Ho, Wo, C, 0, Cout, 3, 1, 1)
    tmp = torch.empty_like(dw)
    for p in (0, 1):
        for q in (0, 1):
            hip.conv_wgrad(spec, x[:, :, p::2, q::2].contiguous(), None, dy, tmp, db if (p, q) == (0, 0) else None)
            kys = (1,) if p == 0 else (0, 2)
            kxs = (1,) if q == 0 else (0, 2)
            for ky in kys:
                for kx in kxs:
                    dw[:, :, ky, kx] = tmp[:, :, 0 if ky == 0 else 1, 0 if kx == 0 else 1]


def conv2d(x0, weight, bias=None, stride=1, pad=0, x1=None, mode0=hip.SRC_DIRECT, mode1=hip.SRC_DIRECT, out_c8=None, half=False):
    return Conv2dFn.apply(x0, x1, weight, bias, stride, pad, mode0, mode1, False, out_c8, half)


def conv2d_passthrough(x0, weight, bias=None, stride=1, pad=0, out_c8=None, half=False):
    return Conv2dFn.apply(x0, None, weight, bias, stride, pad, hip.SRC_DIRECT, hip.SRC_DIRECT, True, out_c8, half)


class InstanceNormFn(torch.autograd.Function):

    @staticmethod
    def forward(ctx, x, residual, relu, eps, x_f16=False):
        x_f16 = bool(x_f16) or hip.is_f16_c8(x)
        if _blocked(x) and hip.mixed():
            buf = copies.of(x).pair
            xin, x_fmt = (buf, 2) if buf is not None else (x, 1 if x_f16 else 0)
            res = residual
            if residual is not None:
                h = copies.of(residual).h16
                if h is not None:
                    res = h[0]
            y, y16, stats = hip.instnorm_forward_c8_mixed(xin, _channels(x), res, relu, eps, x_fmt)
            copies.attach(y, h16=(y16, False))
            ctx.relu, ctx.x_f16 = relu, x_fmt
            ctx.save_for_backward(xin, stats)
            return y
        if _blocked(x):
            y, stats = hip.instnorm_forward_c8(x, _channels(x), residual, relu, eps, x_f16)
        else:
            y, stats = hip.instnorm_forward(x, residual, relu, eps)
        ctx.relu, ctx.x_f16 = relu, x_f16
        ctx.save_for_backward(x, stats)
        return y

    @staticmethod
    def backward(ctx, dy):
        x, stats = ctx.saved_tensors
        dy = dy.contiguous()
        dx = None
        if ctx.needs_input_grad[0]:
            if _blocked(dy):
                dx = hip.instnorm_backward_c8(x, _channels(dy), dy, stats, ctx.relu, ctx.x_f16)
            else:
                dx = hip.instnorm_backward(x, dy, stats, ctx.relu)
        dres = dy if ctx.needs_input_grad[1] else None
        return dx, dres, None, None, None


def instance_norm(x, residual=None, relu=False, eps=1e-5, x_f16=False):
    return InstanceNormFn.apply(x, residual, relu, eps, x_f16)


_MASK_FROM_X = os.environ.get('ESS_BN_MASK_FROM_X', '1') != '0'


class BatchNormTrainFn(torch.autograd.Function):

    @staticmethod
    def forward(ctx, x, residual, gamma, beta, running_mean, running_var, momentum, eps, relu, x_f16=False):
        x_f16 = bool(x_f16) or hip.is_f16_c8(x)
        ctx.x_f16 = x_f16
        if _blocked(x):
            y, stats = hip.batchnorm_train_forward_c8(x, _channels(x), residual, gamma.detach(), beta.detach(), running_mean,
                                                      running_var, momentum, eps, relu, x_f16)
        else:
            y, stats = hip.batchnorm_train_forward(x, residual, gamma.detach(), beta.detach(), running_mean, running_var,
                                                   momentum, eps, relu)
        ctx.relu = relu
        ctx.has_res = residual is not None
        ctx.beta_ref = weakref.ref(beta)
        ctx.save_for_backward(x, y, gamma, stats)
        return y

    @staticmethod
    def backward(ctx, dy):
        x, y, gamma, stats = ctx.saved_tensors
        dy = dy.contiguous()
        need_dx, need_dres, need_g, need_b = ctx.needs_input_grad[0:4]
        beta = ctx.beta_ref()
        if _blocked(x):
            C = _channels(x)
            mask_beta = beta.detach() if (ctx.relu and not ctx.has_res and beta is not None and _MASK_FROM_X) else None
            bwd = lambda *a, **k: hip.batchnorm_train_backward_c8(x, C, *a, x_f16=ctx.x_f16, beta=mask_beta, **k)
        else:
            bwd = lambda *a, **k: hip.batchnorm_train_backward(x, *a, **k)
        direct = need_g and need_b and beta is not None and _direct(gamma) and _direct(beta)
        if direct:
            dx, dres = bwd(y, dy, gamma.detach(), stats, ctx.relu, need_dx, need_dres, gamma.grad, beta.grad, accumulate=True)
            return dx, dres, None, None, None, None, None, None, None, None
        dgamma = torch.empty_like(gamma) if (need_g or need_b) else None
        dbeta = torch.empty_like(gamma) if (need_g or need_b) else None
        dx, dres = bwd(y, dy, gamma.detach(), stats, ctx.relu, need_dx, need_dres, dgamma, dbeta)
        return dx, dres, (dgamma if need_g else None), (dbeta if need_b else None), None, None, None, None, None, None


def batch_norm_train(x, gamma, beta, running_mean, running_var, residual=None, relu=False, momentum=0.1, eps=1e-5, x_f16=False):
    return BatchNormTrainFn.apply(x, residual, gamma, beta, running_mean, running_var, momentum, eps, relu, x_f16)


_UNIT_GRAD = {}


def _unit_grad(device):
    u = _UNIT_GRAD.get(device)
    if u is None:
        u = _UNIT_GRAD[device] = torch.ones((), dtype=torch.float32, device=device)
    return u


def unit_backward(terms):
    terms = [t for t in terms if t.requires_grad]
    if terms:
        torch.autograd.backward(terms, [_unit_grad(t.device) for t in terms])


def _times(grad, g):
    u = _UNIT_GRAD.get(g.device)
# ... 74 lines not shown
```

### ess_amd/hip.py

```python
import ctypes
import os
from ctypes import POINTER, Structure, byref, c_char_p, c_float, c_int, c_int32, c_int64, c_size_t, c_void_p

import torch

from . import copies

_HERE = os.path.dirname(os.path.abspath(__file__))
LIB_PATH = os.path.join(_HERE, 'libess_hip.so')

SRC_DIRECT, SRC_NEAREST_UP2, SRC_ZERO_UP2, SRC_S2D = 0, 1, 2, 3
EPI_LINEAR, EPI_LSTM, EPI_GRU_UR, EPI_GRU_OUT = 0, 1, 2, 3
ACT_NONE, ACT_RELU, ACT_SIGMOID, ACT_TANH, ACT_SUMPOOL2 = 0, 1, 2, 3, 4
W_CONV, W_TRANSPOSED, W_ROWS, W_CONV5_S2D = 0, 1, 2, 3
GRU_U_F32, GRU_U_F16 = 0, 1
COMPUTE_FP32, COMPUTE_BF16, COMPUTE_BF16X3, COMPUTE_F16 = 0, 1, 2, 3
FMT_F32_NCHW, FMT_BF16_C8, FMT_F32_C8, FMT_F16_C8, FMT_F16_C8_HILO = 0, 1, 2, 3, 4
LSTM_H_HILO = 1
GRU_H_HILO = 2

_default_compute = COMPUTE_FP32
_mixed = False


def set_compute(kind):
    global _default_compute, _mixed
    _mixed = kind == 'mixed'
    if _mixed:
        kind = 'bf16'
    _default_compute = {'fp32': COMPUTE_FP32, 'bf16': COMPUTE_BF16, 'bf16x3': COMPUTE_BF16X3, COMPUTE_FP32: COMPUTE_FP32,
                        COMPUTE_BF16: COMPUTE_BF16, COMPUTE_BF16X3: COMPUTE_BF16X3}[kind]


def get_compute():
    return {COMPUTE_FP32: 'fp32', COMPUTE_BF16: 'bf16', COMPUTE_BF16X3: 'bf16x3'}[_default_compute]


def mixed():
    return _mixed


def compute_name():
    return 'mixed' if _mixed else get_compute()

EXPORTS = [
    'ess_last_error', 'ess_version', 'ess_conv2d_plan', 'ess_conv2d_pack_weights', 'ess_conv2d_pack_rows',
    'ess_conv2d_forward', 'ess_to_bf16_c8', 'ess_conv2d_wgrad_workspace', 'ess_conv2d_wgrad', 'ess_conv2d_wgrad_sets', 'ess_norm_workspace', 'ess_instnorm_forward',
    'ess_instnorm_backward', 'ess_batchnorm_train_forward', 'ess_batchnorm_train_backward',
    'ess_upsample_bilinear2x_add', 'ess_sumpool2x2', 'ess_add', 'ess_event_normalize', 'ess_task_loss_workspace',
    'ess_task_loss', 'ess_sym_js_loss', 'ess_l1_loss', 'ess_radam_step', 'ess_argmax_confusion', 'ess_resize_nearest', 'ess_conv2d_pack_weights_multi',
    'ess_voxel_grid_trilinear', 'ess_voxel_grid_trilinear_workspace', 'ess_voxel_grid_temporal', 'ess_voxel_normalize_workspace', 'ess_voxel_normalize',
    'ess_from_bf16_c8', 'ess_norm_workspace_c8', 'ess_instnorm_forward_c8', 'ess_instnorm_backward_c8', 'ess_batchnorm_train_forward_c8',
    'ess_batchnorm_train_backward_c8', 'ess_l1_loss_c8', 'ess_augment_image_label', 'ess_radam_step_dev', 'ess_upsample_bilinear2x_add_c8',
    'ess_upsample_bilinear2x_add_c8_from_c8', 'ess_add_bf16', 'ess_event_normalize_slices', 'ess_sum_scalars',
    'ess_label_confusion', 'ess_augment_perspective_filter', 'ess_tuning_set', 'ess_tuning_get', 'ess_conv2d_s2d_preferred',
    'ess_to_f16_c8', 'ess_bf16_c8_to_f16_c8', 'ess_f16_c8_to_bf16_c8', 'ess_instnorm_forward_c8_mixed', 'ess_seg_head',
    'ess_event_normalize_samples', 'ess_state_carry_masked',
]


class EssConvDesc(Structure):
    _fields_ = [(n, c_int32) for n in (
        'N', 'H_in', 'W_in', 'C0', 'C1', 'mode0', 'mode1', 'C_out', 'H_out', 'W_out', 'ksize', 'stride', 'pad',
        'epilogue', 'act', 'hidden', 'out_split', 'compute', 'fmt0', 'fmt1', 'fmt_out', 'fmt_res')]


class EssConvPlan(Structure):
    _fields_ = [('cout_tile', c_int32), ('ck', c_int32), ('n_chunks', c_int32), ('n_cout_tiles', c_int32),
                ('packed_elems', c_int64), ('packed_bytes', c_int64), ('rows_padded', c_int32), ('lds_bytes', c_int32)]


class EssHipError(RuntimeError):
    pass


_lib = None


def lib():
    global _lib
    if _lib is None:
        if not os.path.exists(LIB_PATH):
            raise EssHipError(f'{LIB_PATH} not found: build it with `python -c "import __graft_entry__ as g; g.build()"` '
                              '(hipcc --offload-arch=gfx950). ess_amd has no CPU or eager fallback.')
        L = ctypes.CDLL(LIB_PATH)
        L.ess_last_error.restype = c_char_p
        L.ess_conv2d_wgrad_workspace.restype = c_size_t
        L.ess_conv2d_wgrad_workspace.argtypes = [POINTER(EssConvDesc)]
        L.ess_task_loss_workspace.restype = c_size_t
        L.ess_task_loss_workspace.argtypes = [c_int32]
        L.ess_norm_workspace.restype = c_size_t
        L.ess_norm_workspace.argtypes = [c_int32]
        L.ess_norm_workspace_c8.restype = c_size_t
        L.ess_norm_workspace_c8.argtypes = [c_int32]
        L.ess_voxel_normalize_workspace.restype = c_size_t
        L.ess_voxel_normalize_workspace.argtypes = [c_int32]
        L.ess_voxel_grid_trilinear_workspace.restype = c_size_t
        L.ess_voxel_grid_trilinear_workspace.argtypes = [c_int64, c_int32, c_int32, c_int32]
        P, F, I, I64 = c_void_p, c_float, c_int32, c_int64
        D = POINTER(EssConvDesc)
        sig = {
            'ess_conv2d_plan': [D, POINTER(EssConvPlan)],
            'ess_conv2d_s2d_preferred': [D],
            'ess_conv2d_pack_weights': [D, c_int, P, P, P, P],
            'ess_conv2d_pack_rows': [D, P, P, F, P, P],
            'ess_conv2d_forward': [D, P, P, P, P, P, P, P, P, P, P, P, P],
            'ess_to_bf16_c8': [P, P, I, I, I, I, P],
            'ess_conv2d_wgrad': [D, P, P, P, P, P, c_int, P, c_size_t, P],
            'ess_conv2d_wgrad_sets': [D, I, P, P, P, P, P, c_int, P, c_size_t, P],
            'ess_instnorm_forward': [P, P, P, P, I, I, F, I, P, c_size_t, P],
            'ess_instnorm_backward': [P, P, P, P, I, I, I, P, c_size_t, P],
            'ess_batchnorm_train_forward': [P, P, P, P, P, P, F, F, P, P, I, I, I, I, P, c_size_t, P],
            'ess_batchnorm_train_backward': [P, P, P, P, P, P, P, P, P, I, I, I, I, I, P, c_size_t, P],
            'ess_upsample_bilinear2x_add': [P, P, P, I, I, I, P],
            'ess_sumpool2x2': [P, P, I, I, I, I, P],
            'ess_add': [P, P, P, I64, P],
            'ess_add_bf16': [P, P, P, P, I64, P],
            'ess_sum_scalars': [P, I, P, P],
            'ess_event_normalize': [P, P, I64, P, P],
            'ess_event_normalize_slices': [P, P, I, I, I64, P, P],
            'ess_task_loss': [P, P, P, P, F, I, I, I, I, I, I, P, c_size_t, P],
            'ess_sym_js_loss': [P, P, P, P, F, I, I, I, P, c_size_t, P],
            'ess_l1_loss': [P, P, P, P, F, I64, P, c_size_t, P],
            'ess_radam_step': [P, P, P, P, I64, F, F, F, F, F, I, P],
            'ess_argmax_confusion': [P, P, P, P, I, I, I, I, P],
            'ess_resize_nearest': [P, P, I, I, I, I, I, P],
            'ess_conv2d_pack_weights_multi': [P, P, P, P, I, P],
            'ess_voxel_grid_trilinear': [P, P, P, P, P, I64, I, I, I, I, P, P, c_size_t, I64, P],
            'ess_voxel_grid_temporal': [P, P, P, P, P, I64, I, I, I, I, I, P, P],
            'ess_voxel_normalize': [P, I, I64, I, P, c_size_t, P],
            'ess_from_bf16_c8': [P, P, I, I, I, I, P],
            'ess_instnorm_forward_c8': [P, P, P, P, I, I, I, F, I, I, P, c_size_t, P],
            'ess_instnorm_backward_c8': [P, P, P, P, I, I, I, I, I, P, c_size_t, P],
            'ess_batchnorm_train_forward_c8': [P, P, P, P, P, P, F, F, P, P, I, I, I, I, I, P, c_size_t, P],
            'ess_batchnorm_train_backward_c8': [P, P, P, P, P, P, P, P, P, P, I, I, I, I, I, I, P, c_size_t, P],
            'ess_l1_loss_c8': [P, P, P, P, F, I64, I64, P, c_size_t, P],
            'ess_to_f16_c8': [P, P, I, I, I, I, I, P],
            'ess_bf16_c8_to_f16_c8': [P, P, I64, P],
            'ess_f16_c8_to_bf16_c8': [P, P, I, I, I, I, I, P],
            'ess_instnorm_forward_c8_mixed': [P, P, P, P, P, I, I, I, F, I, I, I, P, c_size_t, P],
            'ess_augment_image_label': [P, P, P, P, P, P, I, I, I, I, I, P],
            'ess_radam_step_dev': [P, P, P, P, I64, F, F, F, P, P],
            'ess_upsample_bilinear2x_add_c8': [P, P, P, I, I, I, I, P],
            'ess_upsample_bilinear2x_add_c8_from_c8': [P, P, P, I, I, I, I, P],
            'ess_seg_head': [P, I, P, P, P, P, P, P, I, I, I, I, I, I, I, I, I, I, I, P],
            'ess_event_normalize_samples': [P, P, I, I64, P, P, P],
            'ess_state_carry_masked': [P, P, P, I, I, P, P],
        }
        for name, argtypes in sig.items():
            fn = getattr(L, name)
            fn.argtypes = argtypes
            fn.restype = c_int
        _lib = L
    return _lib


def _check(rc, what):
    if rc != 0:
        raise EssHipError(f'{what} failed (rc={rc}): {lib().ess_last_error().decode()}')


def stream():
    return c_void_p(torch.cuda.current_stream().cuda_stream)


def ptr(t, dtype=torch.float32, allow_none=True):
    if t is None:
        if not allow_none:
            raise EssHipError('required tensor is None')
        return c_void_p(0)
    if not t.is_cuda:
        raise EssHipError('ess_amd kernels need CUDA(HIP) tensors; there is no CPU path (got a CPU tensor)')
    if t.dtype != dtype:
        raise EssHipError(f'expected {dtype}, got {t.dtype}')
    if not t.is_contiguous():
        raise EssHipError('expected a contiguous tensor')
    return c_void_p(t.data_ptr())


_desc_cache = {}


class ConvSpec:

    def __init__(self, key):
        (N, H_in, W_in, C0, C1, mode0, mode1, C_out, k, s, p, epi, act, hidden, out_split, compute) = key
        H_out = (H_in + 2 * p - k) // s + 1
        W_out = (W_in + 2 * p - k) // s + 1
        self.desc = EssConvDesc(N, H_in, W_in, C0, C1, mode0, mode1, C_out, H_out, W_out, k, s, p, epi, act, hidden,
                                out_split, compute, FMT_F32_NCHW, FMT_F32_NCHW, FMT_F32_NCHW, FMT_F32_NCHW)
        self._desc_fmt = {}
        self.plan = EssConvPlan()
        _check(lib().ess_conv2d_plan(byref(self.desc), byref(self.plan)), 'ess_conv2d_plan')
        self.key = key
        self.H_out, self.W_out = H_out, W_out
        self.wgrad_ws = None

    def desc_fmt(self, src_fmt=FMT_F32_NCHW, out_fmt=FMT_F32_NCHW, res_fmt=FMT_F32_NCHW):
        key = (src_fmt, out_fmt, res_fmt)
        d = self._desc_fmt.get(key)
# ... 6 lines not shown

    def desc_c8(self):
        return self.desc_fmt(FMT_BF16_C8)


def conv_spec(N, H_in, W_in, C0, C1, C_out, k, s, p, mode0=SRC_DIRECT, mode1=SRC_DIRECT, epi=EPI_LINEAR, act=ACT_NONE,
              hidden=0, out_split=0, compute=None):
    if compute is None:
        compute = _default_compute
    key = (N, H_in, W_in, C0, C1, mode0, mode1, C_out, k, s, p, epi, act, hidden, out_split, compute)
    sp = _desc_cache.get(key)
    if sp is None:
        sp = _desc_cache[key] = ConvSpec(key)
    return sp


def s2d_preferred(spec):
    v = getattr(spec, '_s2d_pref', None)
    if v is None:
        v = spec._s2d_pref = bool(lib().ess_conv2d_s2d_preferred(byref(spec.desc)))
    return v


def spec_of(key):
    sp = _desc_cache.get(key)
    if sp is None:
        sp = _desc_cache[key] = ConvSpec(key)
    return sp


def pack_weights(spec, w, w2=None, kind=W_CONV):
    out = torch.empty(spec.plan.packed_bytes, dtype=torch.uint8, device=w.device)
    _check(lib().ess_conv2d_pack_weights(byref(spec.desc), kind, ptr(w), ptr(w2), c_void_p(out.data_ptr()), stream()),
           'ess_conv2d_pack_weights')
    return out


def pack_weights_multi(jobs):
    n = len(jobs)
    descs = (EssConvDesc * n)(*[j[0].desc for j in jobs])
    kinds = (c_int32 * n)(*[int(j[1]) for j in jobs])
    ws = (c_void_p * n)(*[ptr(j[2]).value for j in jobs])
    outs = (c_void_p * n)(*[j[3].data_ptr() for j in jobs])
    _check(lib().ess_conv2d_pack_weights_multi(descs, kinds, ws, outs, n, stream()), 'ess_conv2d_pack_weights_multi')


def pack_rows(spec, v, v2=None, fill=0.0):
    out = torch.empty(spec.plan.rows_padded, dtype=torch.float32, device=v.device)
    _check(lib().ess_conv2d_pack_rows(byref(spec.desc), ptr(v), ptr(v2), c_float(fill), ptr(out), stream()),
           'ess_conv2d_pack_rows')
    return out


def conv_forward(spec, src0, src1, packed_w, scale=None, shift=None, residual=None, aux0=None, aux1=None, out=None,
                 out2=None, out_bf=None, src_fmt=FMT_F32_NCHW, out_fmt=FMT_F32_NCHW, aux_fmt=FMT_F32_NCHW):
    if is_f16_c8(src0) or is_f16_c8(src1) or is_f16_c8(residual):
        raise EssHipError('conv_forward: an F16_C8 (pre-norm) tensor is read by the norm kernels only, not as a BF16_C8 source / residual')
    if out_fmt == FMT_F16_C8 and not is_f16_c8(out):
        raise EssHipError('conv_forward: an F16_C8 output must come from f16_c8_empty (the tag is how its consumers know the format)')
    sdt = torch.bfloat16 if src_fmt == FMT_BF16_C8 else torch.float32
    odt = torch.bfloat16 if out_fmt in (FMT_BF16_C8, FMT_F16_C8) else torch.float32
    rdt = torch.bfloat16 if out_fmt in (FMT_BF16_C8, FMT_F16_C8) else torch.float32
    res_fmt = aux_fmt if aux_fmt != FMT_F32_NCHW else ((FMT_BF16_C8 if out_fmt == FMT_F16_C8 else out_fmt) if residual is not None else FMT_F32_NCHW)
    desc = spec.desc if (src_fmt, out_fmt, res_fmt) == (FMT_F32_NCHW,) * 3 else spec.desc_fmt(src_fmt, out_fmt, res_fmt)
    u16 = spec.desc.act == GRU_U_F16 and spec.desc.epilogue in (EPI_GRU_UR, EPI_GRU_OUT)
    udt_out = torch.float16 if (u16 and spec.desc.epilogue == EPI_GRU_UR and out_fmt == FMT_F32_C8) else odt
    udt_aux = torch.float16 if (u16 and spec.desc.epilogue == EPI_GRU_OUT and res_fmt == FMT_F32_C8) else torch.float32
    _check(lib().ess_conv2d_forward(byref(desc), ptr(src0, sdt), ptr(src1, sdt),
                                    ptr(packed_w, torch.uint8), ptr(scale), ptr(shift), ptr(residual, rdt), ptr(aux0), ptr(aux1, udt_aux),
                                    ptr(out, udt_out), ptr(out2, odt), ptr(out_bf, torch.bfloat16), stream()),
           'ess_conv2d_forward')
    return out


def c8_stageable(ksize, stride, pad):
    if ksize in (1, 3):
        return True
    if ksize == 5:
        return os.environ.get('ESS_CONV_PAIR', '1')[:1] != '0'
    return False


def bf16_c8_empty(N, C, H, W, device):
    return torch.empty(N, (C + 7) // 8, H, W, 8, dtype=torch.bfloat16, device=device)


def f16_c8_raw_empty(N, C, H, W, device):
    return torch.empty(N, (C + 7) // 8, H, W, 8, dtype=torch.float16, device=device)


def f32_c8_empty(N, C, H, W, device):
    return torch.empty(N, (C + 7) // 8, H, W, 8, dtype=torch.float32, device=device)


def to_bf16_c8(x):
    N, C, H, W = x.shape
    y = bf16_c8_empty(N, C, H, W, x.device)
    _check(lib().ess_to_bf16_c8(ptr(x), ptr(y, torch.bfloat16), N, C, H, W, stream()), 'ess_to_bf16_c8')
    return y


def from_bf16_c8(y, C):
    N, nb, H, W, _ = y.shape
    if is_f16_c8(y):
        raise EssHipError('from_bf16_c8: the tensor holds IEEE half elements (F16_C8): use f16_c8_to_float')
    if not 0 < C <= nb * 8:
        raise EssHipError(f'from_bf16_c8: {C} channels do not fit {nb} blocks')
    x = torch.empty(N, C, H, W, dtype=torch.float32, device=y.device)
    _check(lib().ess_from_bf16_c8(ptr(y, torch.bfloat16), ptr(x), N, C, H, W, stream()), 'ess_from_bf16_c8')
    return x


def is_c8(t):
    return t is not None and t.dtype == torch.bfloat16 and t.dim() == 5 and t.shape[-1] == 8


def f16_c8_empty(N, C, H, W, device):
    t = torch.empty(N, (C + 7) // 8, H, W, 8, dtype=torch.bfloat16, device=device)
    t.ess_f16 = True
    return t


def is_f16_c8(t):
    return t is not None and getattr(t, 'ess_f16', False)

# ... 52 lines not shown
    ws = workspace(nbytes, dy.device, 'wgrad')
    n = len(sets)
    a0s = (c_void_p * n)(*[ptr(t[0], sdt).value for t in sets])
    a1s = (c_void_p * n)(*[(ptr(t[1], sdt).value if t[1] is not None else None) for t in sets])
    gs = (c_void_p * n)(*[ptr(t[2], ddt).value for t in sets])
    _check(lib().ess_conv2d_wgrad_sets(byref(desc), n, a0s, a1s, gs, ptr(dw), ptr(db), int(accumulate), c_void_p(ws.data_ptr()),
                                       c_size_t(ws.numel()), stream()), 'ess_conv2d_wgrad_sets')


def instnorm_forward(x, residual, relu, eps=1e-5):
    N, C, H, W = x.shape
    y = torch.empty_like(x)
    stats = torch.empty(N * C, 2, dtype=torch.float32, device=x.device)
    ws = workspace(lib().ess_norm_workspace(N * C), x.device, 'norm')
    _check(lib().ess_instnorm_forward(ptr(x), ptr(residual), ptr(y), ptr(stats), N * C, H * W, c_float(eps), int(relu),
                                      c_void_p(ws.data_ptr()), c_size_t(ws.numel()), stream()), 'ess_instnorm_forward')
    return y, stats


def instnorm_backward(x, dy, stats, relu):
    N, C, H, W = x.shape
    dx = torch.empty_like(x)
    ws = workspace(lib().ess_norm_workspace(N * C), x.device, 'norm')
    _check(lib().ess_instnorm_backward(ptr(x), ptr(dy), ptr(stats), ptr(dx), N * C, H * W, int(relu),
                                       c_void_p(ws.data_ptr()), c_size_t(ws.numel()), stream()), 'ess_instnorm_backward')
    return dx


def batchnorm_train_forward(x, residual, gamma, beta, running_mean, running_var, momentum, eps, relu):
    N, C, H, W = x.shape
    y = torch.empty_like(x)
    stats = torch.empty(C, 2, dtype=torch.float32, device=x.device)
    ws = workspace(lib().ess_norm_workspace(C), x.device, 'norm')
    _check(lib().ess_batchnorm_train_forward(ptr(x), ptr(residual), ptr(gamma), ptr(beta), ptr(running_mean),
                                             ptr(running_var), c_float(momentum), c_float(eps), ptr(y), ptr(stats), N, C,
                                             H * W, int(relu), c_void_p(ws.data_ptr()), c_size_t(ws.numel()), stream()),
           'ess_batchnorm_train_forward')
    return y, stats


def batchnorm_train_backward(x, y, dy, gamma, stats, relu, need_dx=True, need_dres=False, dgamma=None, dbeta=None,
                             accumulate=False):
    N, C, H, W = x.shape
    dx = torch.empty_like(x) if need_dx else None
    dres = torch.empty_like(x) if need_dres else None
    ws = workspace(lib().ess_norm_workspace(C), x.device, 'norm')
    _check(lib().ess_batchnorm_train_backward(ptr(x), ptr(y), ptr(dy), ptr(gamma), ptr(stats), ptr(dx), ptr(dres),
                                              ptr(dgamma), ptr(dbeta), int(accumulate), N, C, H * W, int(relu),
                                              c_void_p(ws.data_ptr()), c_size_t(ws.numel()), stream()),
           'ess_batchnorm_train_backward')
    return dx, dres


def instnorm_forward_c8(x, C, residual, relu, eps=1e-5, x_f16=False):
    N, CB, H, W, _ = x.shape
    y = torch.empty(x.shape, dtype=torch.bfloat16, device=x.device)
    stats = torch.empty(N * C, 2, dtype=torch.float32, device=x.device)
    L = lib()
    xdt, xf = torch.bfloat16, int(bool(x_f16))
    ws = workspace(L.ess_norm_workspace_c8(N * CB), x.device, 'norm8')
    _check(L.ess_instnorm_forward_c8(ptr(x, xdt), ptr(residual, torch.bfloat16), ptr(y, torch.bfloat16), ptr(stats), N, C,
                                     H * W, c_float(eps), int(relu), xf, c_void_p(ws.data_ptr()), c_size_t(ws.numel()), stream()),
           'ess_instnorm_forward_c8')
    return y, stats


def instnorm_backward_c8(x, C, dy, stats, relu, x_f16=False):
    N, CB, H, W, _ = x.shape
    if int(x_f16) == 2:
        CB //= 2
    dx = torch.empty(N, CB, H, W, 8, dtype=torch.bfloat16, device=x.device)
    L = lib()
    xdt, xf = x.dtype, int(x_f16)
    ws = workspace(L.ess_norm_workspace_c8(N * CB), x.device, 'norm8')
    _check(L.ess_instnorm_backward_c8(ptr(x, xdt), ptr(dy, torch.bfloat16), ptr(stats), ptr(dx, torch.bfloat16), N, C, H * W,
                                      int(relu), xf, c_void_p(ws.data_ptr()), c_size_t(ws.numel()), stream()), 'ess_instnorm_backward_c8')
    return dx


def batchnorm_train_forward_c8(x, C, residual, gamma, beta, running_mean, running_var, momentum, eps, relu, x_f16=False):
    N, CB, H, W, _ = x.shape
    y = torch.empty(x.shape, dtype=torch.bfloat16, device=x.device)
    stats = torch.empty(2, C, 2, dtype=torch.float32, device=x.device)
    L = lib()
    xdt, xf = torch.bfloat16, int(bool(x_f16))
    ws = workspace(L.ess_norm_workspace_c8(CB), x.device, 'norm8')
    _check(L.ess_batchnorm_train_forward_c8(ptr(x, xdt), ptr(residual, torch.bfloat16), ptr(gamma), ptr(beta),
                                            ptr(running_mean), ptr(running_var), c_float(momentum), c_float(eps),
                                            ptr(y, torch.bfloat16), ptr(stats), N, C, H * W, int(relu), xf, c_void_p(ws.data_ptr()),
                                            c_size_t(ws.numel()), stream()), 'ess_batchnorm_train_forward_c8')
    return y, stats


def batchnorm_train_backward_c8(x, C, y, dy, gamma, stats, relu, need_dx=True, need_dres=False, dgamma=None, dbeta=None,
                                accumulate=False, x_f16=False, beta=None):
    if stats.numel() != 4 * C:
        raise EssHipError(f'batchnorm_train_backward_c8: stats must be the forward\'s [2, C, 2] tensor, got {tuple(stats.shape)}')
    N, CB, H, W, _ = x.shape
    dx = torch.empty(x.shape, dtype=torch.bfloat16, device=x.device) if need_dx else None
    dres = torch.empty(x.shape, dtype=torch.bfloat16, device=x.device) if need_dres else None
    L = lib()
    xdt, xf = torch.bfloat16, int(bool(x_f16))
    ws = workspace(L.ess_norm_workspace_c8(CB), x.device, 'norm8')
    _check(L.ess_batchnorm_train_backward_c8(ptr(x, xdt), ptr(y, torch.bfloat16), ptr(dy, torch.bfloat16), ptr(gamma), ptr(beta),
                                             ptr(stats), ptr(dx, torch.bfloat16), ptr(dres, torch.bfloat16), ptr(dgamma), ptr(dbeta),
                                             int(accumulate), N, C, H * W, int(relu), xf, c_void_p(ws.data_ptr()), c_size_t(ws.numel()),
                                             stream()), 'ess_batchnorm_train_backward_c8')
    return dx, dres


def upsample_bilinear2x_add(a, b=None):
    N, C, H, W = a.shape
    y = torch.empty(N, C, 2 * H, 2 * W, dtype=torch.float32, device=a.device)
    _check(lib().ess_upsample_bilinear2x_add(ptr(a), ptr(b), ptr(y), N * C, H, W, stream()), 'ess_upsample_bilinear2x_add')
    return y


def upsample_bilinear2x_add_c8(a, b=None):
    N, C, H, W = a.shape
    y = bf16_c8_empty(N, C, 2 * H, 2 * W, a.device)
    _check(lib().ess_upsample_bilinear2x_add_c8(ptr(a), ptr(b), ptr(y, torch.bfloat16), N, C, H, W, stream()),
           'ess_upsample_bilinear2x_add_c8')
    return y


def upsample_bilinear2x_add_c8_from_c8(a8, b8=None):
    N, CB, H, W, _ = a8.shape
    y = torch.empty(N, CB, 2 * H, 2 * W, 8, dtype=torch.bfloat16, device=a8.device)
    _check(lib().ess_upsample_bilinear2x_add_c8_from_c8(ptr(a8, torch.bfloat16), ptr(b8, torch.bfloat16), ptr(y, torch.bfloat16), N,
                                                        CB * 8, H, W, stream()), 'ess_upsample_bilinear2x_add_c8_from_c8')
    return y


def sumpool2x2(x, out=None, accumulate=False):
    N, C, H, W = x.shape
    if out is None:
        out = torch.empty(N, C, H // 2, W // 2, dtype=torch.float32, device=x.device)
    _check(lib().ess_sumpool2x2(ptr(x), ptr(out), N * C, H // 2, W // 2, int(accumulate), stream()), 'ess_sumpool2x2')
# ... 322 lines not shown
        got = f'{palette.dtype}{tuple(palette.shape)}' if torch.is_tensor(palette) else type(palette).__name__
        raise EssHipError(f'seg_head: palette must be a uint8 [K={K}, 3] tensor, got {got}')
    y0, x0, h, w = (0, 0, H, W) if window is None else (int(v) for v in window)
    if y0 < 0 or x0 < 0 or h <= 0 or w <= 0 or y0 + h > H or x0 + w > W:
        raise EssHipError(f'seg_head: window {(y0, x0, h, w)} leaves the {H} x {W} source plane')
    Ho, Wo = (h, w) if out_hw is None else (int(out_hw[0]), int(out_hw[1]))
    if Ho <= 0 or Wo <= 0:
        raise EssHipError(f'seg_head: out_hw {(Ho, Wo)} is empty')
    dev = x.device
    labels = torch.empty(N, Ho, Wo, dtype=torch.uint8, device=dev)
    colour = torch.empty(N, Ho, Wo, 3, dtype=torch.uint8, device=dev) if palette is not None else None
    conf = torch.empty(N, Ho, Wo, dtype=torch.float32, device=dev) if want_confidence else None
    _check(lib().ess_seg_head(ptr(x, x.dtype, allow_none=False), fmt, ptr(weight.detach(), allow_none=False), ptr(bias.detach(), allow_none=False),
                              ptr(palette, torch.uint8), ptr(labels, torch.uint8), ptr(colour, torch.uint8), ptr(conf), N, C, K, H, W,
                              y0, x0, h, w, Ho, Wo, stream()), 'ess_seg_head')
    return labels, colour, conf


def f16_blocks_empty(N, C, H, W, device, hilo=False):
    return torch.empty(N, ((C + 7) // 8) * (2 if hilo else 1), H, W, 8, dtype=torch.float16, device=device)


def h16_of(t):
    return copies.of(t).h16


def attach_h16(t, h16, hilo=False):
    return copies.attach(t, h16=(h16, bool(hilo)))


def to_f16_c8(x, hilo=False):
    N, C, H, W = x.shape
    y = f16_blocks_empty(N, C, H, W, x.device, hilo)
    _check(lib().ess_to_f16_c8(ptr(x), ptr(y, torch.float16), N, C, H, W, int(bool(hilo)), stream()), 'ess_to_f16_c8')
    return y


def bf16_c8_to_f16_c8(x):
    y = torch.empty(x.shape, dtype=torch.float16, device=x.device)
    _check(lib().ess_bf16_c8_to_f16_c8(ptr(x, torch.bfloat16), ptr(y, torch.float16), x.numel() // 8, stream()), 'ess_bf16_c8_to_f16_c8')
    return y


def f16_c8_to_bf16_c8(x, hilo=False):
    N, nb, H, W, _ = x.shape
    CB = nb // 2 if hilo else nb
    y = torch.empty(N, CB, H, W, 8, dtype=torch.bfloat16, device=x.device)
    _check(lib().ess_f16_c8_to_bf16_c8(ptr(x, torch.float16), ptr(y, torch.bfloat16), N, CB * 8, H, W, int(bool(hilo)), stream()),
           'ess_f16_c8_to_bf16_c8')
    return y


def conv_forward_h16(spec, src0, src1, packed_w, scale=None, shift=None, residual=None, aux0=None, aux1=None, out=None, out2=None,
                     out_h16=None, out_fmt=FMT_F32_NCHW, aux_fmt=FMT_F32_NCHW, src_fp32=False):
    if spec.desc.compute != COMPUTE_F16:
        raise EssHipError('conv_forward_h16: the spec was not created with compute=COMPUTE_F16')
    sdt = torch.float32 if src_fp32 else torch.float16
    sfmt = FMT_F32_NCHW if src_fp32 else FMT_F16_C8
    half_out = out_fmt in (FMT_F16_C8, FMT_F16_C8_HILO)
    odt = torch.float16 if half_out else torch.float32
    res_fmt = aux_fmt if aux_fmt != FMT_F32_NCHW else ((FMT_F16_C8 if half_out else out_fmt) if residual is not None else FMT_F32_NCHW)
    desc = spec.desc_fmt(sfmt, out_fmt, res_fmt)
    u16 = (spec.desc.act & 1) == GRU_U_F16 and spec.desc.epilogue in (EPI_GRU_UR, EPI_GRU_OUT)
    udt_out = torch.float16 if (u16 and spec.desc.epilogue == EPI_GRU_UR and out_fmt == FMT_F32_C8) else odt
    udt_aux = torch.float16 if (u16 and spec.desc.epilogue == EPI_GRU_OUT and res_fmt == FMT_F32_C8) else torch.float32
    _check(lib().ess_conv2d_forward(byref(desc), ptr(src0, sdt), ptr(src1, sdt), ptr(packed_w, torch.uint8), ptr(scale), ptr(shift),
                                    ptr(residual, torch.float16 if half_out else torch.float32), ptr(aux0), ptr(aux1, udt_aux),
                                    ptr(out, udt_out), ptr(out2, odt), ptr(out_h16, torch.float16), stream()), 'ess_conv2d_forward(f16)')
    return out


def instnorm_forward_c8_mixed(x, C, residual, relu, eps=1e-5, x_fmt=1, want_bf16=True):
    N, nb, H, W, _ = x.shape
    CB = nb // 2 if x_fmt == 2 else nb
    y = torch.empty(N, CB, H, W, 8, dtype=torch.bfloat16, device=x.device) if want_bf16 else None
    y16 = torch.empty(N, CB, H, W, 8, dtype=torch.float16, device=x.device)
    stats = torch.empty(N * C, 2, dtype=torch.float32, device=x.device)
    L = lib()
    ws = workspace(L.ess_norm_workspace_c8(N * CB), x.device, 'norm8')
    res_f16 = 0
    if residual is not None and residual.dtype == torch.float16:
        res_f16 = 2 if residual.shape[1] == 2 * CB else 1
    _check(L.ess_instnorm_forward_c8_mixed(ptr(x, x.dtype), ptr(residual, residual.dtype if residual is not None else torch.float16),
                                           ptr(y, torch.bfloat16), ptr(y16, torch.float16), ptr(stats), N, C, H * W, c_float(eps),
                                           int(relu), int(x_fmt), int(res_f16), c_void_p(ws.data_ptr()), c_size_t(ws.numel()), stream()),
           'ess_instnorm_forward_c8_mixed')
    return y, y16, stats
```

### ess_amd/models/style_networks.py

```python
import torch
import torch.nn as nn

from .. import functional as Fn
from .. import copies, hip
from .submodules import InterpolationLayer


def gaussian_weights_init(m):
    if m.__class__.__name__.find('Conv') == 0:
        m.weight.data.normal_(0.0, 0.02)


class ReLUINSConv2d(nn.Module):

    def __init__(self, n_in, n_out, kernel_size, stride, padding=0):
        super().__init__()
        self.model = nn.Sequential(nn.Conv2d(n_in, n_out, kernel_size=kernel_size, stride=stride, padding=padding, bias=True),
                                   nn.InstanceNorm2d(n_out, affine=False), nn.ReLU(inplace=True))
        self.model.apply(gaussian_weights_init)

    def forward_fused(self, x, skip=None, up=False):
        c = self.model[0]
        pre = Fn.pre_norm_fmt() if hip.is_c8(x) else None
        y = Fn.conv2d(x, c.weight, c.bias, c.stride[0], c.padding[0], x1=skip,
                      mode0=hip.SRC_NEAREST_UP2 if up else hip.SRC_DIRECT, out_c8=pre, half=True)
        return Fn.instance_norm(y, None, True, self.model[1].eps, x_f16=pre == Fn.PRE_NORM)

    def forward(self, x):
        return self.forward_fused(x)


class INSResBlock(nn.Module):

    def conv3x3(self, inplanes, out_planes, stride=1):
        return [nn.Conv2d(inplanes, out_planes, kernel_size=3, stride=stride, padding=1)]

    def __init__(self, inplanes, planes, stride=1, dropout=0.0):
        super().__init__()
        if dropout > 0:
            raise NotImplementedError('INSResBlock dropout is never enabled by SemSegE2VID')
        layers = self.conv3x3(inplanes, planes, stride) + [nn.InstanceNorm2d(planes), nn.ReLU(inplace=True)]
        layers += self.conv3x3(planes, planes) + [nn.InstanceNorm2d(planes)]
        self.model = nn.Sequential(*layers)
        self.model.apply(gaussian_weights_init)

    def forward(self, x, first=False):
        c1, c2 = self.model[0], self.model[3]
        pre = Fn.pre_norm_fmt() if hip.is_c8(x) else None
        pre1 = pre
        if first and pre == Fn.PRE_NORM and Fn.mixed() and c1.out_channels % 64 == 0:
            pre1 = Fn.PRE_NORM_HILO
        y, skip = Fn.conv2d_passthrough(x, c1.weight, c1.bias, c1.stride[0], 1, out_c8=pre1, half=True)
        if copies.of(skip).h16 is None:
            copies.carry(skip, x, 'h16')
        y = Fn.instance_norm(y, None, True, self.model[1].eps, x_f16=pre == Fn.PRE_NORM)
        y = Fn.conv2d(y, c2.weight, c2.bias, 1, 1, out_c8=pre, half=True)
        return Fn.instance_norm(y, skip, False, self.model[4].eps, x_f16=pre == Fn.PRE_NORM)


class SemSegE2VID(nn.Module):

    def __init__(self, input_c, output_c, skip_connect=False, skip_type='sum', input_index_map=False):
        super().__init__()
        if input_index_map:
            raise NotImplementedError('input_index_map is never enabled by the ESS trainers')
        if skip_connect and skip_type != 'concat':
            raise ValueError("skip_connect=True only works with skip_type='concat' (decoder_scale_2 is built for "
                             "2x channels, reference :25)")
        self.skip_connect, self.skip_type, self.input_index_map = skip_connect, skip_type, input_index_map
        self.index_coords = None
        tch = input_c
        if skip_connect:
            blocks = [INSResBlock(tch, tch) for _ in range(5)]
            blocks += [ReLUINSConv2d(tch, tch // 2, kernel_size=3, stride=1, padding=1)]
            self.decoder_scale_1 = nn.Sequential(*blocks)
            self.decoder_scale_2 = nn.Sequential(ReLUINSConv2d(tch, tch // 2, kernel_size=3, stride=1, padding=1),
                                                 ReLUINSConv2d(tch // 2, tch // 4, kernel_size=3, stride=1, padding=1))
            tch //= 2
            self.decoder_scale_3 = nn.Sequential(ReLUINSConv2d(tch, tch // 2, kernel_size=3, stride=1, padding=1),
                                                 ReLUINSConv2d(tch // 2, tch // 2, kernel_size=3, stride=1, padding=1))
            tch //= 2
            self.decoder_scale_4 = nn.Sequential(ReLUINSConv2d(tch, tch // 2, kernel_size=3, stride=1, padding=1))
            tch //= 2
        else:
            self.decoder_scale_1 = nn.Sequential(*[INSResBlock(tch, tch) for _ in range(3)])
            for name in ('decoder_scale_2', 'decoder_scale_3', 'decoder_scale_4'):
                setattr(self, name, nn.Sequential(InterpolationLayer(scale_factor=2, mode='nearest'),
                                                  ReLUINSConv2d(tch, tch // 2, kernel_size=3, stride=1, padding=1)))
                tch //= 2
        self.decoder_scale_5 = nn.Sequential(nn.Conv2d(tch, output_c, kernel_size=1, stride=1, padding=0))

    def update_skip_dict(self, skips, x, sz_in):
        rem, scale = sz_in % x.shape[3], sz_in // x.shape[3]
        assert rem == 0
        skips[scale] = x

    def forward(self, input_dict):
        sz_in = input_dict[1].shape[3]
        out = {8: input_dict[8]}
        x = self._trunk(input_dict, out, sz_in)
        c5 = self.decoder_scale_5[0]
        x = Fn.conv2d(x, c5.weight, c5.bias, 1, 0, out_c8=False, half=True)
        self.update_skip_dict(out, x, sz_in)
        return out

    def _trunk(self, input_dict, out, sz_in):
        x = input_dict[8]
        c8 = Fn.c8_mode()
        lat = (lambda t, deep=False: Fn.as_c8(t, want_hilo=deep).contiguous()) if c8 else (lambda t, deep=False: t.contiguous())
# ... 10 lines not shown
            x = self.decoder_scale_1[0](x, first=True)
            for blk in list(self.decoder_scale_1)[1:]:
                x = blk(x)
            x = self.decoder_scale_2[0].forward_fused(x, lat(input_dict[4]), up=True)
            x = record(self.decoder_scale_2[1](x))
            x = self.decoder_scale_3[0].forward_fused(x, lat(input_dict[2]), up=True)
            x = record(self.decoder_scale_3[1](x))
            x = self.decoder_scale_4[0].forward_fused(x, None, up=True)
        else:
            x = self.decoder_scale_1[0](x, first=True)
            for blk in list(self.decoder_scale_1)[1:]:
                x = blk(x)
            x = record(self.decoder_scale_2[1].forward_fused(x, None, up=True))
            x = record(self.decoder_scale_3[1].forward_fused(x, None, up=True))
            x = self.decoder_scale_4[1].forward_fused(x, None, up=True)
        return x

    def predict(self, input_dict, out_hw=None, window=None, palette=None, want_confidence=False):
        with torch.no_grad():
            x = self._trunk(input_dict, None, input_dict[1].shape[3])
            c5 = self.decoder_scale_5[0]
            if hip.is_c8(x):
                C = x.shape[1] * 8
                if hip.mixed():
                    h, hilo = Fn.half_of(x)
                    if hilo:
                        raise hip.EssHipError('SemSegE2VID.predict: the last activation came as a [hi | lo] half pair')
                    x = h
            else:
                C = x.shape[1]
            return hip.seg_head(x.contiguous(), C, c5.weight, c5.bias, out_hw=out_hw, window=window, palette=palette,
                                want_confidence=want_confidence)


_PENDING_BN_COUNTERS = []


def flush_bn_counters():
    if _PENDING_BN_COUNTERS:
        with torch.no_grad():
            torch._foreach_add_(_PENDING_BN_COUNTERS, 1)
        _PENDING_BN_COUNTERS.clear()


class _ConvBN(nn.Module):

    @staticmethod
    def run(conv, bn, x, residual=None, relu=True, passthrough=False):
        out_c8 = Fn.c8_mode()
        if bn.training:
            pre = Fn.pre_norm_fmt()
            if passthrough:
                y, skip = Fn.Conv2dFn.apply(x, None, conv.weight, None, conv.stride[0], conv.padding[0], hip.SRC_DIRECT,
                                            hip.SRC_DIRECT, True, pre)
            else:
                y = Fn.conv2d(x, conv.weight, None, conv.stride[0], conv.padding[0], out_c8=pre)
            out = Fn.batch_norm_train(y, bn.weight, bn.bias, bn.running_mean, bn.running_var, residual, relu,
                                      bn.momentum, bn.eps, x_f16=pre == Fn.PRE_NORM)
            _PENDING_BN_COUNTERS.append(bn.num_batches_tracked)
            return (out, skip) if passthrough else out
        if passthrough:
            raise NotImplementedError('passthrough is a train-mode (autograd) feature')
        if torch.is_grad_enabled() and (x.requires_grad or conv.weight.requires_grad):
            raise NotImplementedError('eval-mode BatchNorm is forward-only here (validation runs under no_grad, '
                                      'training/base_trainer.py:419)')
        N, C, H, W = x.shape[0], Fn._channels(x), x.shape[2], x.shape[3]
        spec = hip.conv_spec(N, H, W, C, 0, conv.out_channels, conv.kernel_size[0], conv.stride[0], conv.padding[0],
                             act=hip.ACT_RELU if relu else hip.ACT_NONE)
        with torch.no_grad():
            scale = bn.weight / torch.sqrt(bn.running_var + bn.eps)
            shift = bn.bias - bn.running_mean * scale
        out = Fn._empty_act(N, conv.out_channels, spec.H_out, spec.W_out, x.device, out_c8)
        return hip.conv_forward(spec, x.contiguous(), None, Fn.packed_weight(spec, conv.weight),
                                hip.pack_rows(spec, scale.contiguous(), fill=1.0), hip.pack_rows(spec, shift.contiguous()),
                                residual, out=out, src_fmt=Fn._fmt(x), out_fmt=Fn._fmt(out))


class BasicBlock(nn.Module):
    expansion = 1

    def __init__(self, inplanes, planes, stride=1):
        super().__init__()
        self.conv1 = nn.Conv2d(inplanes, planes, 3, stride, 1, bias=False)
        self.bn1 = nn.BatchNorm2d(planes)
        self.relu = nn.ReLU(inplace=True)
        self.conv2 = nn.Conv2d(planes, planes, 3, 1, 1, bias=False)
        self.bn2 = nn.BatchNorm2d(planes)
        self.downsample = None
        if stride != 1 or inplanes != planes:
            self.downsample = nn.Sequential(nn.Conv2d(inplanes, planes, 1, stride, bias=False), nn.BatchNorm2d(planes))
        self.stride = stride

    def forward(self, x):
        if self.downsample is not None:
            xa, xb = Fn.fork(x)
            identity = _ConvBN.run(self.downsample[0], self.downsample[1], xa, None, relu=False)
            out = _ConvBN.run(self.conv1, self.bn1, xb, None, relu=True)
        elif self.bn1.training:
            out, identity = _ConvBN.run(self.conv1, self.bn1, x, None, relu=True, passthrough=True)
        else:
            identity = x
            out = _ConvBN.run(self.conv1, self.bn1, x, None, relu=True)
        return _ConvBN.run(self.conv2, self.bn2, out, identity, relu=True)


def _resnet_init(module):
    for m in module.modules():
        if isinstance(m, nn.Conv2d):
            nn.init.kaiming_normal_(m.weight, mode='fan_out', nonlinearity='relu')
# ... 71 lines not shown
```

### include/ess_hip.h

```cpp
#ifndef ESS_HIP_H
#define ESS_HIP_H

#include <stddef.h>
#include <stdint.h>

#ifdef __cplusplus
extern "C" {
#endif

typedef void* ess_stream_t;

enum { ESS_OK = 0, ESS_EINVAL = -22, ESS_ENOTSUP = -95, ESS_ELAUNCH = -5 };

enum { ESS_SRC_DIRECT = 0, ESS_SRC_NEAREST_UP2 = 1, ESS_SRC_ZERO_UP2 = 2,
       ESS_SRC_S2D = 3  };
enum {
  ESS_EPI_LINEAR = 0,
  ESS_EPI_LSTM = 1,
  ESS_EPI_GRU_UR = 2,
  ESS_EPI_GRU_OUT = 3
};
enum { ESS_ACT_NONE = 0, ESS_ACT_RELU = 1, ESS_ACT_SIGMOID = 2, ESS_ACT_TANH = 3, ESS_ACT_SUMPOOL2 = 4 };
enum { ESS_COMPUTE_FP32 = 0, ESS_COMPUTE_BF16 = 1,
       ESS_COMPUTE_BF16X3 = 2,
// ... 6 lines not shown
enum {
  ESS_W_CONV = 0,
  ESS_W_TRANSPOSED = 1,
  ESS_W_ROWS = 2,
  ESS_W_CONV5_S2D = 3
};

typedef struct EssConvDesc {
  int32_t N;
  int32_t H_in, W_in;
  int32_t C0, C1;
  int32_t mode0, mode1;
  int32_t C_out, H_out, W_out;
  int32_t ksize, stride, pad;
  int32_t epilogue;
  int32_t act;
  int32_t hidden;
  int32_t out_split;
  int32_t compute;
  int32_t fmt0, fmt1;
  int32_t fmt_out;
  int32_t fmt_res;
} EssConvDesc;

typedef struct EssConvPlan {
  int32_t cout_tile;
  int32_t ck;
  int32_t n_chunks, n_cout_tiles;
  int64_t packed_elems;
  int64_t packed_bytes;
  int32_t rows_padded;
  int32_t lds_bytes;
} EssConvPlan;

const char* ess_last_error(void);
int ess_version(void);

int ess_conv2d_plan(const EssConvDesc* d, EssConvPlan* plan);

int ess_conv2d_s2d_preferred(const EssConvDesc* d);

int ess_conv2d_pack_weights(const EssConvDesc* d, int w_kind, const float* w, const float* w2,
                            void* packed, ess_stream_t stream);
int ess_conv2d_pack_weights_multi(const EssConvDesc* descs, const int32_t* w_kinds, const float* const* w,
                                  void* const* packed, int32_t count, ess_stream_t stream);

int ess_conv2d_pack_rows(const EssConvDesc* d, const float* v, const float* v2, float fill,
                         float* packed, ess_stream_t stream);

int ess_conv2d_forward(const EssConvDesc* d, const void* src0, const void* src1, const void* packed_w,
                       const float* scale, const float* shift, const void* residual, const float* aux0,
                       const float* aux1, void* out, void* out2, void* out_bf16, ess_stream_t stream);

int ess_to_bf16_c8(const float* x, void* y, int32_t N, int32_t C, int32_t H, int32_t W, ess_stream_t stream);
int ess_from_bf16_c8(const void* x, float* y, int32_t N, int32_t C, int32_t H, int32_t W, ess_stream_t stream);
int ess_to_f16_c8(const float* x, void* y, int32_t N, int32_t C, int32_t H, int32_t W, int32_t hilo, ess_stream_t stream);
int ess_bf16_c8_to_f16_c8(const void* x, void* y, int64_t n_vec, ess_stream_t stream);
int ess_f16_c8_to_bf16_c8(const void* x, void* y, int32_t N, int32_t C, int32_t H, int32_t W, int32_t hilo, ess_stream_t stream);

size_t ess_conv2d_wgrad_workspace(const EssConvDesc* d);
int ess_conv2d_wgrad(const EssConvDesc* d, const void* src0, const void* src1, const void* dy,
                     float* dw, float* db, int accumulate, void* workspace, size_t workspace_bytes,
                     ess_stream_t stream);
int ess_conv2d_wgrad_sets(const EssConvDesc* d, int32_t n_sets, const void* const* src0, const void* const* src1,
                          const void* const* dy, float* dw, float* db, int32_t accumulate, void* workspace,
                          size_t workspace_bytes, ess_stream_t stream);

size_t ess_norm_workspace(int32_t groups);
int ess_instnorm_forward(const float* x, const float* residual, float* y, float* stats, int32_t planes,
                         int32_t hw, float eps, int32_t relu, void* workspace, size_t workspace_bytes,
                         ess_stream_t stream);
int ess_instnorm_backward(const float* x, const float* dy, const float* stats, float* dx, int32_t planes,
                          int32_t hw, int32_t relu, void* workspace, size_t workspace_bytes, ess_stream_t stream);

size_t ess_norm_workspace_c8(int32_t groups);
int ess_instnorm_forward_c8(const void* x, const void* residual, void* y, float* stats, int32_t N, int32_t C, int32_t hw,
                            float eps, int32_t relu, int32_t x_f16, void* workspace, size_t workspace_bytes, ess_stream_t stream);
int ess_instnorm_forward_c8_mixed(const void* x, const void* residual, void* y, void* y16, float* stats, int32_t N, int32_t C, int32_t hw,
                                  float eps, int32_t relu, int32_t x_fmt, int32_t res_f16, void* workspace, size_t workspace_bytes,
                                  ess_stream_t stream);
int ess_instnorm_backward_c8(const void* x, const void* dy, const float* stats, void* dx, int32_t N, int32_t C, int32_t hw,
                             int32_t relu, int32_t x_f16, void* workspace, size_t workspace_bytes, ess_stream_t stream);
int ess_batchnorm_train_forward_c8(const void* x, const void* residual, const float* gamma, const float* beta,
                                   float* running_mean, float* running_var, float momentum, float eps, void* y, float* stats,
                                   int32_t N, int32_t C, int32_t hw, int32_t relu, int32_t x_f16, void* workspace,
                                   size_t workspace_bytes, ess_stream_t stream);
int ess_batchnorm_train_backward_c8(const void* x, const void* y, const void* dy, const float* gamma, const float* beta,
                                    const float* stats, void* dx, void* d_residual, float* dgamma, float* dbeta, int32_t accumulate,
                                    int32_t N, int32_t C, int32_t hw, int32_t relu, int32_t x_f16, void* workspace,
                                    size_t workspace_bytes, ess_stream_t stream);

int ess_batchnorm_train_forward(const float* x, const float* residual, const float* gamma, const float* beta,
                                float* running_mean, float* running_var, float momentum, float eps, float* y,
                                float* stats, int32_t N, int32_t C, int32_t hw, int32_t relu, void* workspace,
                                size_t workspace_bytes, ess_stream_t stream);
int ess_batchnorm_train_backward(const float* x, const float* y, const float* dy, const float* gamma,
                                 const float* stats, float* dx, float* d_residual, float* dgamma, float* dbeta,
                                 int32_t accumulate, int32_t N, int32_t C, int32_t hw, int32_t relu,
                                 void* workspace, size_t workspace_bytes, ess_stream_t stream);

int ess_upsample_bilinear2x_add(const float* a, const float* b, float* y, int32_t planes, int32_t H,
                                int32_t W, ess_stream_t stream);
int ess_upsample_bilinear2x_add_c8(const float* a, const float* b, void* y, int32_t N, int32_t C, int32_t H, int32_t W,
                                   ess_stream_t stream);

int ess_upsample_bilinear2x_add_c8_from_c8(const void* a, const void* b, void* y, int32_t N, int32_t C, int32_t H, int32_t W,
                                           ess_stream_t stream);
int ess_sumpool2x2(const float* x, float* y, int32_t planes, int32_t H_out, int32_t W_out, int32_t accumulate,
                   ess_stream_t stream);
int ess_add(const float* a, const float* b, float* y, int64_t n, ess_stream_t stream);
int ess_sum_scalars(const float* const* terms, int32_t n, float* out, ess_stream_t stream);
int ess_add_bf16(const void* a, const void* b, const void* c, void* y, int64_t n_vectors, ess_stream_t stream);

int ess_event_normalize(const float* x, float* y, int64_t n, void* workspace, ess_stream_t stream);
int ess_event_normalize_slices(const float* x, float* y, int32_t B, int32_t T, int64_t chunk, void* workspace, ess_stream_t stream);
int ess_event_normalize_samples(const float* x, float* y, int32_t S, int64_t chunk, const int32_t* mode, void* workspace,
                                ess_stream_t stream);

enum { ESS_CARRY_HOLD = 0, ESS_CARRY_TAKE = 1, ESS_CARRY_ZERO = 2 };
int ess_state_carry_masked(void* const* dst, const void* const* src, const int64_t* bytes_per_sample, int32_t n_tensors,
                           int32_t n_samples, const int32_t* mode, ess_stream_t stream);

int ess_voxel_grid_trilinear(const float* x, const float* y, const float* pol, const float* t,
                             const int64_t* slice_offsets, int64_t n_events, int32_t n_slices, int32_t channels,
                             int32_t height, int32_t width, float* out, void* workspace, size_t workspace_bytes,
                             int64_t max_events_per_slice, ess_stream_t stream);
size_t ess_voxel_grid_trilinear_workspace(int64_t n_events, int32_t n_slices, int32_t height, int32_t width);
int ess_voxel_grid_temporal(const int32_t* x, const int32_t* y, const double* t, const float* pol,
                            const int64_t* slice_offsets, int64_t n_events, int32_t n_slices, int32_t bins,
                            int32_t height, int32_t width, int32_t separate_pol, float* out, ess_stream_t stream);
size_t ess_voxel_normalize_workspace(int32_t n_slices);
int ess_voxel_normalize(float* grid, int32_t n_slices, int64_t elems_per_slice, int32_t mode, void* workspace,
                        size_t workspace_bytes, ess_stream_t stream);

int ess_augment_image_label(const float* img, const int64_t* label, const float* params, const int64_t* id_lut, float* out_img,
                            int64_t* out_label, int32_t N, int32_t H_src, int32_t W_src, int32_t H, int32_t W,
                            ess_stream_t stream);

int ess_augment_perspective_filter(const float* img, const int64_t* label, const float* params, const int64_t* id_lut,
                                   float* scratch, float* out_img, int64_t* out_label, int32_t N, int32_t H, int32_t W,
                                   ess_stream_t stream);

size_t ess_task_loss_workspace(int32_t K);
// ... 41 lines not shown
```

Before: 1745.

## Fuse norm statistics partials into 3x3 conv epilogues, skip separate reduction pass

The 3x3 stride-1 wave-specialised and wide conv kernels gain a STATS variant whose epilogue reduces per-channel sum and sum-of-squares of the half output into double partials. A finalize kernel turns these into per-channel sums, and new instance/batch norm '_sums' entry points consume them, so the norm layers no longer re-read the activation just to compute statistics. Style network and ResNet call sites request the fusion through norm='in'/'bn'. The cost is extra shuffles and stores in the conv epilogue, more register pressure, and an extra finalize launch; routes that cannot produce partials fall back to the old path.

```diff
diff --git a/ess_amd/copies.py b/ess_amd/copies.py
--- a/ess_amd/copies.py
+++ b/ess_amd/copies.py
@@ -6,14 +6,14 @@
 
 
 class Copies:
-    __slots__ = ('stamp', 'c8', 'h16', 'f32c8', 'pair', 'mixed', 'unwritten')
+    __slots__ = ('stamp', 'c8', 'h16', 'f32c8', 'pair', 'mixed', 'stats', 'unwritten')
 
     def __init__(self, stamp, unwritten):
         self.stamp, self.unwritten = stamp, unwritten
-        self.c8 = self.h16 = self.f32c8 = self.pair = self.mixed = None
+        self.c8 = self.h16 = self.f32c8 = self.pair = self.mixed = self.stats = None
 
 
-_NONE = collections.namedtuple('NoCopies', Copies.__slots__)(None, None, None, None, None, None, False)
+_NONE = collections.namedtuple('NoCopies', Copies.__slots__)(None, None, None, None, None, None, None, False)
 _UNWRITTEN = _NONE._replace(unwritten=True)
 
 
diff --git a/ess_amd/csrc/conv_bf16.hip b/ess_amd/csrc/conv_bf16.hip
--- a/ess_amd/csrc/conv_bf16.hip
+++ b/ess_amd/csrc/conv_bf16.hip
@@ -281,7 +281,16 @@
   return cw > 0 && 4 * tiles >= 3 * tuning().cus;
 }
 
-int conv_bf16_launch(const EssConvDesc* d, const EssConvPlan& pl, const Geom& g, const ConvKArgs& a, hipStream_t st) {
+int conv_bf16_launch(const EssConvDesc* d, const EssConvPlan& pl, const Geom& g, const ConvKArgs& a, hipStream_t st, int* query_nsl,
+                     size_t stats_bytes) {
+  const bool want_stats = a.stats != nullptr || query_nsl != nullptr;
+  if (query_nsl) *query_nsl = 0;
+#define ESS_NO_STATS(ROUTE_)                                                                                                     \
+  if (want_stats) {                                                                                                              \
+    if (query_nsl) return ESS_OK;                                                                                                \
+    ess_set_error("conv: statistics partials were requested, but this launch runs on the %s kernel, which writes none", ROUTE_); \
+    return ESS_ENOTSUP;                                                                                                          \
+  }
   ESS_CHECK_ARG(g.IH * g.IW <= kpc(d->ksize, d->stride) * 256, "conv(bf16): input tile of %d positions exceeds the staging capacity",
                 g.IH * g.IW);
   ESS_CHECK_ARG((int64_t)(d->C0 > d->C1 ? d->C0 : d->C1) * d->H_in * d->W_in * 4 < (int64_t)1 << 31,
@@ -300,14 +309,17 @@
   if (a.f16) ESS_CHECK_ARG(!a.split && d->act != ESS_ACT_SUMPOOL2 && (a.fmt_out == ESS_FMT_F32_NCHW || d->out_split == 0 || d->epilogue != ESS_EPI_LINEAR),
                            "conv(f16): forward forms only");
   if (!c8 && !a.residual && conv_bf16_stem_applies(d, pl)) {
+    ESS_NO_STATS("7x7 stem")
     conv_bf16_launch_stem(d, pl, st, a);
     return ess_launch_status("conv2d_forward(bf16, 7x7 stem)");
   }
   if (is_paired(d) && !c8 && !a.residual && !a.split && conv_bf16_head_applies(d, pl)) {
+    ESS_NO_STATS("5x5 head")
     conv_bf16_launch_head(d, pl, st, a);
     return ess_launch_status("conv2d_forward(bf16, 5x5 head)");
   }
   if (is_paired(d)) {
+    ESS_NO_STATS("5x5 tap-paired")
     const size_t lds2 = 2 * (size_t)pl.lds_bytes;
     ESS_CHECK_ARG(lds2 <= 160 * 1024, "conv(bf16, 5x5): two stages of %d B exceed the 160 KiB LDS", pl.lds_bytes);
     {
@@ -325,6 +337,7 @@
     return ess_launch_status("conv2d_forward(bf16, tap-paired)");
   }
   if (d->mode0 == ESS_SRC_S2D) {
+    ESS_NO_STATS("space-to-depth 5x5")
     ESS_CHECK_ARG(c8 && a.fmt_out == ESS_FMT_BF16_C8 && !a.out_bf && !a.residual && !a.out_f16 && pl.ck == 16 && pl.cout_tile == 64 && (!a.hilo || (d->C_out % 64) == 0) &&
                       (d->act == ESS_ACT_NONE || d->act == ESS_ACT_RELU),
                   "conv(bf16, S2D): BF16_C8 in and out, no residual / copy, act in {none, relu}");
@@ -347,6 +360,7 @@
     int th, tw, max_cin;
     conv_bf16_poly_tile(&th, &tw, &max_cin);
     if (d->C0 <= max_cin) {
+    ESS_NO_STATS("polyphase nearest-up2")
     ConvKArgs t = a;
     t.Hin = d->H_in >> 1; t.Win = d->W_in >> 1;
     t.tiles_x = ceil_div(t.Win, tw);
@@ -364,8 +378,22 @@
   if (ws_enabled() && d->ksize == 3 && d->stride == 1 && pl.ck == 16) {
     const size_t lds2 = 2 * (size_t)pl.lds_bytes;
     WidePick wp;
-    if (wide_pick(d, pl, g, a, c8, &wp)) {
+    const bool wide = wide_pick(d, pl, g, a, c8, &wp);
+    int stats_nsl = 0;
+    if (want_stats) {
+      const bool form = c8 && a.fmt_out == ESS_FMT_BF16_C8 && d->epilogue == ESS_EPI_LINEAR && (a.out_f16 || a.f16) && !a.hilo && !a.split &&
+                        d->act == ESS_ACT_NONE && !a.residual && d->out_split == 0 && !a.out_bf && (d->C_out % pl.cout_tile) == 0 &&
+                        (wide || lds2 <= 160 * 1024);
+      if (!form) { ESS_NO_STATS("3x3 / stride-1 kernel in a form other than the plain pre-norm output") }
+      stats_nsl = wide ? wp.tiles_x * wp.tiles_y * (4 / wp.cw) : g.tiles_x * g.tiles_y * 4;
+      if (query_nsl) { *query_nsl = stats_nsl; return ESS_OK; }
+      const size_t need = (size_t)d->N * (d->C_out / 8) * stats_nsl * 16 * sizeof(double);
+      ESS_CHECK_ARG(stats_bytes >= need, "conv: the statistics partials need %zu bytes, got %zu", need, stats_bytes);
+      ESS_CHECK_ARG(((uintptr_t)a.stats & 7) == 0, "conv: the statistics partials must be 8-byte aligned");
+    }
+    if (wide) {
       ConvKArgs t = a;
+      t.stats_nsl = stats_nsl;
       t.tiles_x = wp.tiles_x; t.n_tiles = wp.tiles_x * wp.tiles_y;
       const int cus = tuning().cus;
       t.persist = wp.tiles > cus ? 1 : 0;
@@ -377,16 +405,19 @@
       static const int persist = [] { const char* e = getenv("ESS_WS_PERSIST"); return e ? atoi(e) : 1; }();
       const int per_cu_lds = (int)((160 * 1024) / lds2), per_cu = (mb == 4 ? 1 : 2) < per_cu_lds ? (mb == 4 ? 1 : 2) : per_cu_lds;
       const int slots = tuning().cus * per_cu;
+      ConvKArgs t = a;
+      t.stats_nsl = stats_nsl;
       if (persist && (int)grid.x > slots) {
-        ConvKArgs t = a;
         t.persist = 1;
         conv_bf16_launch_ws(mb, d->epilogue, c8, dim3((unsigned)slots), lds2, st, t);
         return ess_launch_status("conv2d_forward(bf16, wave-specialised, persistent)");
       }
-      conv_bf16_launch_ws(mb, d->epilogue, c8, grid, lds2, st, a);
+      conv_bf16_launch_ws(mb, d->epilogue, c8, grid, lds2, st, t);
       return ess_launch_status("conv2d_forward(bf16, wave-specialised)");
     }
   }
+  ESS_NO_STATS("generic tile")
+#undef ESS_NO_STATS
   const int key = d->ksize * 10 + d->stride;
   ESS_CHECK_ARG(!a.split || split_generic, "conv(bf16): split operands reached the generic tile kernel (k%d s%d, %zu B of LDS for two stages)",
                 d->ksize, d->stride, 2 * (size_t)pl.lds_bytes);
diff --git a/ess_amd/csrc/conv_bf16_wide.hip b/ess_amd/csrc/conv_bf16_wide.hip
--- a/ess_amd/csrc/conv_bf16_wide.hip
+++ b/ess_amd/csrc/conv_bf16_wide.hip
@@ -11,8 +11,9 @@
 constexpr int WIDE_RP = 32;
 constexpr int WIDE_IW = 18;
 
-template <int MBW, int CW, int EPI = ESS_EPI_LINEAR, bool S2D = false, bool H = false>
+template <int MBW, int CW, int EPI = ESS_EPI_LINEAR, bool S2D = false, bool H = false, bool STATS = false>
 __global__ __launch_bounds__(512, 2) void conv_bf16_wide_kernel(const ConvKArgs a) {
+  static_assert(!STATS || (EPI == ESS_EPI_LINEAR && !S2D), "statistics come with the LINEAR epilogue of a plain 3x3");
   extern __shared__ __attribute__((aligned(16))) u32x4 smem16[];
   constexpr int KS = 3, CB8 = 2, CK = 16, NB = WIDE_NB, RP = WIDE_RP;
   constexpr int PW = 4 / CW;
@@ -320,6 +321,8 @@
     }
     if constexpr (EPI == ESS_EPI_GRU_UR) conv_epilogue_gru_ur_c8<MBW, NB, H>(a, acc, ct_w, n, half, pixi, (unsigned)(a.Hout * a.Wout));
     else conv_epilogue_gru_out_c8<MBW, NB, H>(a, acc, ct_w, n, half, pixi, (unsigned)(a.Hout * a.Wout));
+  } else if constexpr (STATS) {
+    conv_epilogue_c8_stats<MBW, NB, H>(a, acc, ct_w, n, half, x0 + ox, y0, ly, biased, tile * PW + pw);
   } else {
     conv_epilogue_c8_wide<MBW, NB, H>(a, acc, ct_w, n, half, x0 + ox, y0, ly, biased);
   }
@@ -333,6 +336,18 @@
   constexpr int PW = 4 / CW, TH = PW * WIDE_NB * 2, PLANE = (TH + 2) * WIDE_RP, COT = MBW * CW * 32;
   constexpr size_t lds = 2 * (size_t)(2 * PLANE + 9 * 2 * COT) * 16;
   static_assert(lds <= 160 * 1024, "two stages must fit the 160 KiB LDS");
+  if constexpr (EPI == ESS_EPI_LINEAR && !S2D) {
+    if (a.stats) {
+      if (a.f16) {
+        ess_allow_lds(conv_bf16_wide_kernel<MBW, CW, EPI, false, true, true>, lds);
+        hipLaunchKernelGGL((conv_bf16_wide_kernel<MBW, CW, EPI, false, true, true>), grid, dim3(512), lds, st, a);
+      } else {
+        ess_allow_lds(conv_bf16_wide_kernel<MBW, CW, EPI, false, false, true>, lds);
+        hipLaunchKernelGGL((conv_bf16_wide_kernel<MBW, CW, EPI, false, false, true>), grid, dim3(512), lds, st, a);
+      }
+      return;
+    }
+  }
   if (a.f16) {
     ess_allow_lds(conv_bf16_wide_kernel<MBW, CW, EPI, S2D, true>, lds);
     hipLaunchKernelGGL((conv_bf16_wide_kernel<MBW, CW, EPI, S2D, true>), grid, dim3(512), lds, st, a);
diff --git a/ess_amd/csrc/conv_bf16_ws.hip b/ess_amd/csrc/conv_bf16_ws.hip
--- a/ess_amd/csrc/conv_bf16_ws.hip
+++ b/ess_amd/csrc/conv_bf16_ws.hip
@@ -17,9 +17,10 @@
 
 using namespace essconv;
 
-template <int MB, int EPI, bool SRCBF, bool OUT8 = false, bool H = false>
+template <int MB, int EPI, bool SRCBF, bool OUT8 = false, bool H = false, bool STATS = false>
 __global__ __launch_bounds__(512, MB == 4 ? 2 : 4) void conv_bf16_ws_k3s1_kernel(const ConvKArgs a) {
   static_assert(!H || SRCBF, "half operands come as F16_C8 tensors");
+  static_assert(!STATS || (OUT8 && SRCBF && EPI == ESS_EPI_LINEAR), "statistics come with a LINEAR C8 output of C8 sources");
   extern __shared__ __attribute__((aligned(16))) u32x4 smem16[];
   constexpr int KS = 3, CB8 = 2, CK = 16;
   constexpr int COT = MB * 32;
@@ -345,7 +346,8 @@
 #ifdef ESS_ABLATE
   if (a.deep & 8) continue;
 #endif
-  if constexpr (OUT8) conv_epilogue_c8<MB, H>(a, acc, ct, n, half, x0 + lx, y0, ly, biased);
+  if constexpr (STATS) conv_epilogue_c8_stats<MB, NBW, H>(a, acc, ct, n, half, x0 + lx, y0, ly, biased, tile * 4 + wave);
+  else if constexpr (OUT8) conv_epilogue_c8<MB, H>(a, acc, ct, n, half, x0 + lx, y0, ly, biased);
   else conv_epilogue<MB, EPI, false, H>(a, acc, ct, n, half, x0 + lx, y0, ly, biased);
   ESS_CT(47);
   if constexpr (EPI != ESS_EPI_LSTM) ESS_CW(43);
@@ -358,6 +360,16 @@
 template <int MB, bool SRCBF>
 void launch_ws(int epi, dim3 grid, size_t lds, hipStream_t st, const ConvKArgs& a) {
   if constexpr (SRCBF) {
+    if (a.stats) {
+      if (a.f16) {
+        ess_allow_lds(conv_bf16_ws_k3s1_kernel<MB, ESS_EPI_LINEAR, true, true, true, true>, lds);
+        hipLaunchKernelGGL((conv_bf16_ws_k3s1_kernel<MB, ESS_EPI_LINEAR, true, true, true, true>), grid, dim3(512), lds, st, a);
+      } else {
+        ess_allow_lds(conv_bf16_ws_k3s1_kernel<MB, ESS_EPI_LINEAR, true, true, false, true>, lds);
+        hipLaunchKernelGGL((conv_bf16_ws_k3s1_kernel<MB, ESS_EPI_LINEAR, true, true, false, true>), grid, dim3(512), lds, st, a);
+      }
+      return;
+    }
     if (a.f16) {
 #define ESS_WSH(E_, O8_) { ess_allow_lds(conv_bf16_ws_k3s1_kernel<MB, E_, true, O8_, true>, lds); hipLaunchKernelGGL((conv_bf16_ws_k3s1_kernel<MB, E_, true, O8_, true>), grid, dim3(512), lds, st, a); }
       if (a.fmt_out == ESS_FMT_BF16_C8) ESS_WSH(ESS_EPI_LINEAR, true)
diff --git a/ess_amd/csrc/conv_common.h b/ess_amd/csrc/conv_common.h
--- a/ess_amd/csrc/conv_common.h
+++ b/ess_amd/csrc/conv_common.h
@@ -43,6 +43,8 @@
   int deep;
   int f16;
   int hilo;
+  double* stats;
+  int stats_nsl;
 };
 
 template <bool H> __device__ __forceinline__ uint2 ess_cvt4(float v0, float v1, float v2, float v3);
@@ -708,10 +710,11 @@
   }
 }
 
-template <int MB, bool SC, bool SH, bool F16, bool RELU, bool RES, int NB, bool H = false, bool HILO = false>
+template <int MB, bool SC, bool SH, bool F16, bool RELU, bool RES, int NB, bool H = false, bool HILO = false, bool STATS = false>
 __device__ __forceinline__ void conv_epilogue_c8_plain(const ConvKArgs& a, f32x16 (&acc)[MB][NB], int ct, int n, int half,
-                                                       int x, int y0, const int (&ly)[NB]) {
+                                                       int x, int y0, const int (&ly)[NB], int sl = 0) {
   static_assert(!HILO || H, "a [hi | lo] output is a half tensor");
+  static_assert(!STATS || ((F16 || H) && !RELU && !RES && !HILO), "statistics come with a plain pre-norm (half) output");
   typedef unsigned int u32x4e __attribute__((ext_vector_type(4)));
   constexpr int COT = MB * 32;
   const unsigned HW = (unsigned)(a.Hout * a.Wout);
@@ -803,6 +806,41 @@
           const auto t1 = __builtin_amdgcn_permlane32_swap(pl[0][nb].y, pl[1][nb].y, false, false);
           const u32x4e vlo = {t0[0], t1[0], t0[1], t1[1]};
           __builtin_amdgcn_raw_buffer_store_b128(vlo, r_o, (int)(pix16[nb] != ESS_OOB ? plane + (unsigned)nblk * HW * 16u + pix16[nb] : ESS_OOB), 0, ESS_C8_AUX);
+        }
+      }
+      if constexpr (STATS) {
+        double v[16];
+#pragma unroll
+        for (int jj = 0; jj < 2; ++jj) {
+          float s[4] = {0.f, 0.f, 0.f, 0.f}, q[4] = {0.f, 0.f, 0.f, 0.f};
+#pragma unroll
+          for (int nb = 0; nb < NB; ++nb) {
+            float f[4];
+            ess_up4<true>(pk[jj][nb], f);
+#pragma unroll
+            for (int i = 0; i < 4; ++i) {
+              const float g = pix16[nb] != ESS_OOB ? f[i] : 0.f;
+              s[i] += g;
+              q[i] = fmaf(g, g, q[i]);
+            }
+          }
+#pragma unroll
+          for (int i = 0; i < 4; ++i) { v[jj * 8 + i * 2] = (double)s[i]; v[jj * 8 + i * 2 + 1] = (double)q[i]; }
+        }
+        const int pxl = (int)(threadIdx.x & 31);
+#pragma unroll
+        for (int m = 16, h = 8; h >= 1; m >>= 1, h >>= 1) {
+          const bool up = (pxl & m) != 0;
+#pragma unroll
+          for (int t = 0; t < h; ++t) {
+            const double keep = up ? v[t + h] : v[t], send = up ? v[t] : v[t + h];
+            v[t] = keep + __shfl_xor(send, m, 64);
+          }
+        }
+        v[0] += __shfl_xor(v[0], 1, 64);
+        if (!(pxl & 1)) {
+          const int blk = (rowbase >> 3) + jp + (pxl >> 4), ch = 4 * half + ((pxl >> 2) & 3), qi = (pxl >> 1) & 1;
+          a.stats[((((size_t)n * nblk + blk) * a.stats_nsl + sl) * 8 + ch) * 2 + qi] = v[0];
         }
       }
     }
@@ -994,6 +1032,19 @@
   } else {
     if (a.shift) conv_epilogue_c8_wide_sel<MB, false, true, NB, H>(a, acc, ct, n, half, x, y0, ly);
     else conv_epilogue_c8_wide_sel<MB, false, false, NB, H>(a, acc, ct, n, half, x, y0, ly);
+  }
+}
+
+template <int MB, int NB, bool H>
+__device__ __forceinline__ void conv_epilogue_c8_stats(const ConvKArgs& a, f32x16 (&acc)[MB][NB], int ct, int n, int half, int x,
+                                                       int y0, const int (&ly)[NB], bool biased, int sl) {
+  if (biased || (!a.scale && !a.shift)) {
+    conv_epilogue_c8_plain<MB, false, false, true, false, false, NB, H, false, true>(a, acc, ct, n, half, x, y0, ly, sl);
+  } else if (a.scale) {
+    if (a.shift) conv_epilogue_c8_plain<MB, true, true, true, false, false, NB, H, false, true>(a, acc, ct, n, half, x, y0, ly, sl);
+    else conv_epilogue_c8_plain<MB, true, false, true, false, false, NB, H, false, true>(a, acc, ct, n, half, x, y0, ly, sl);
+  } else {
+    conv_epilogue_c8_plain<MB, false, true, true, false, false, NB, H, false, true>(a, acc, ct, n, half, x, y0, ly, sl);
   }
 }
 
@@ -1535,7 +1586,8 @@
 }
 
 
-int conv_bf16_launch(const EssConvDesc* d, const EssConvPlan& pl, const Geom& g, const ConvKArgs& a, hipStream_t st);
+int conv_bf16_launch(const EssConvDesc* d, const EssConvPlan& pl, const Geom& g, const ConvKArgs& a, hipStream_t st, int* query_nsl = nullptr,
+                     size_t stats_bytes = 0);
 int conv_bf16_pack_weights(const EssConvDesc* d, const EssConvPlan& pl, int w_kind, const float* w, const float* w2, void* packed,
                            hipStream_t st, bool split = false, bool f16 = false);
 int conv_bf16_pack_weights_multi(const EssConvDesc* descs, const int32_t* kinds, const float* const* w, void* const* packed, int count,
diff --git a/ess_amd/csrc/conv_fwd.hip b/ess_amd/csrc/conv_fwd.hip
--- a/ess_amd/csrc/conv_fwd.hip
+++ b/ess_amd/csrc/conv_fwd.hip
@@ -213,9 +213,10 @@
   return ess_launch_status("pack_rows");
 }
 
-extern "C" int ess_conv2d_forward(const EssConvDesc* d, const void* src0, const void* src1, const void* packed_w,
-                                  const float* scale, const float* shift, const void* residual, const float* aux0,
-                                  const float* aux1, void* out, void* out2, void* out_bf16, ess_stream_t stream) {
+static int conv2d_forward_impl(const EssConvDesc* d, const void* src0, const void* src1, const void* packed_w,
+                               const float* scale, const float* shift, const void* residual, const float* aux0,
+                               const float* aux1, void* out, void* out2, void* out_bf16, void* stats, size_t stats_bytes,
+                               int* query_nsl, ess_stream_t stream) {
   EssConvDesc dcopy;
   bool out_f16 = false;
   if (d && d->fmt_out == ESS_FMT_F16_C8 && d->compute != ESS_COMPUTE_F16) {
@@ -269,6 +270,7 @@
   a.split = rd.split ? 1 : 0;
   a.f16 = rd.f16 ? 1 : 0;
   a.hilo = rd.hilo ? 1 : 0;
+  a.stats = (double*)stats;
   if (rd.hilo && d->epilogue == ESS_EPI_LINEAR)
     ESS_CHECK_ARG(!residual && (d->C_out % pl.cout_tile) == 0 && d->fmt_out == ESS_FMT_BF16_C8, "conv(f16): a [hi | lo] output takes no residual and whole channel tiles");
   if (rd.hilo && d->epilogue == ESS_EPI_GRU_OUT)
@@ -283,7 +285,9 @@
   a.IH = g.IH; a.IW = g.IW; a.row_pitch = g.row_pitch; a.par_off = g.par_off; a.plane = g.plane;
   a.ck = pl.ck; a.n_chunks = pl.n_chunks; a.act = d->act; a.hid = d->hidden; a.out_split = d->out_split;
   hipStream_t st = (hipStream_t)stream;
-  if (is_bf16(d)) return conv_bf16_launch(d, pl, g, a, st);
+  if (is_bf16(d)) return conv_bf16_launch(d, pl, g, a, st, query_nsl, stats_bytes);
+  if (query_nsl) { *query_nsl = 0; return ESS_OK; }
+  ESS_CHECK_ARG(!stats, "conv: statistics partials exist for bf16 / f16 compute only");
   ESS_CHECK_ARG(g.IH * g.IW <= kpc32(d->ksize, d->stride) * 256, "conv: input tile of %d positions exceeds the staging capacity",
                 g.IH * g.IW);
   ESS_CHECK_ARG((int64_t)(d->C0 > d->C1 ? d->C0 : d->C1) * d->H_in * d->W_in * 4 < (int64_t)1 << 31,
@@ -304,3 +308,30 @@
   }
   return ess_launch_status("conv2d_forward");
 }
+
+extern "C" int ess_conv2d_forward(const EssConvDesc* d, const void* src0, const void* src1, const void* packed_w,
+                                  const float* scale, const float* shift, const void* residual, const float* aux0,
+                                  const float* aux1, void* out, void* out2, void* out_bf16, ess_stream_t stream) {
+  return conv2d_forward_impl(d, src0, src1, packed_w, scale, shift, residual, aux0, aux1, out, out2, out_bf16, nullptr, 0, nullptr, stream);
+}
+
+extern "C" int ess_conv2d_forward_stats(const EssConvDesc* d, const void* src0, const void* src1, const void* packed_w,
+                                        const float* scale, const float* shift, void* out, void* partials, size_t partials_bytes,
+                                        ess_stream_t stream) {
+  ESS_CHECK_ARG(partials != nullptr, "conv2d_forward_stats: null partials buffer");
+  return conv2d_forward_impl(d, src0, src1, packed_w, scale, shift, nullptr, nullptr, nullptr, out, nullptr, nullptr, partials, partials_bytes,
+                             nullptr, stream);
+}
+
+extern "C" size_t ess_conv2d_stats_bytes(const EssConvDesc* d, int32_t has_scale, int32_t has_shift, int32_t* n_slices) {
+  alignas(16) static const float dummy[4] = {0.f, 0.f, 0.f, 0.f};
+  if (n_slices) *n_slices = 0;
+  if (!d) return 0;
+  int nsl = 0;
+  const void* any = (const void*)dummy;
+  const int rc = conv2d_forward_impl(d, any, d->C1 ? any : nullptr, any, has_scale ? dummy : nullptr, has_shift ? dummy : nullptr, nullptr,
+                                     nullptr, nullptr, (void*)dummy, nullptr, nullptr, nullptr, 0, &nsl, nullptr);
+  if (rc != ESS_OK || nsl <= 0) return 0;
+  if (n_slices) *n_slices = nsl;
+  return (size_t)d->N * (size_t)(d->C_out / 8) * (size_t)nsl * 16 * sizeof(double);
+}
diff --git a/ess_amd/csrc/norm_c8.hip b/ess_amd/csrc/norm_c8.hip
--- a/ess_amd/csrc/norm_c8.hip
+++ b/ess_amd/csrc/norm_c8.hip
@@ -443,6 +443,24 @@
   __syncthreads();
 #pragma unroll
   for (int jj = 0; jj < 8; ++jj) { t0[jj] = tot[2 * jj]; t1[jj] = tot[2 * jj + 1]; }
+}
+
+__global__ __launch_bounds__(1024) void c8_finalize_kernel(const double* __restrict__ partials, double* __restrict__ sums, int nsl, int nseg,
+                                                           int seg_stride) {
+  __shared__ double part[64 * 16];
+  const int g = blockIdx.x, j = threadIdx.x & 15, k0 = threadIdx.x >> 4, ng = blockDim.x >> 4;
+  double t = 0;
+  for (int sgm = 0; sgm < nseg; ++sgm) {
+    const double* p = partials + ((size_t)sgm * seg_stride + g) * nsl * 16 + j;
+    for (int k = k0; k < nsl; k += ng) t += p[(size_t)k * 16];
+  }
+  part[k0 * 16 + j] = t;
+  __syncthreads();
+  if (threadIdx.x < 16) {
+    double tt = 0;
+    for (int i = 0; i < ng; ++i) tt += part[i * 16 + threadIdx.x];
+    sums[(size_t)g * 16 + threadIdx.x] = tt;
+  }
 }
 
 __global__ __launch_bounds__(256) void in_apply_c8_kernel(const u32x4n* __restrict__ x, const u32x4n* __restrict__ res,
@@ -925,3 +943,62 @@
                      (u32x4n*)d_residual, dgamma, dbeta, accumulate, N, CB, C, hw, relu, mask_x ? beta : nullptr);
   return ess_launch_status("batchnorm_train_backward_c8");
 }
+
+
+
+extern "C" int ess_norm_finalize_partials_c8(const void* partials, int32_t N, int32_t C, int32_t n_slices, int32_t batchnorm, void* sums,
+                                             size_t sums_bytes, ess_stream_t stream) {
+  ESS_CHECK_ARG(partials && sums && N > 0 && C > 0 && (C % 8) == 0 && n_slices > 0, "norm_finalize_partials_c8: bad arguments");
+  ESS_CHECK_ARG(((((uintptr_t)partials) | ((uintptr_t)sums)) & 7) == 0, "norm_finalize_partials_c8: the buffers hold doubles");
+  const int CB = C / 8, groups = batchnorm ? CB : N * CB;
+  ESS_CHECK_ARG(sums_bytes >= (size_t)groups * 16 * sizeof(double), "norm_finalize_partials_c8: sums need %zu bytes, got %zu",
+                (size_t)groups * 16 * sizeof(double), sums_bytes);
+  const int slices = batchnorm ? n_slices * N : n_slices;
+  int threads = 1024;
+  while (threads > 64 && threads / 16 >= 2 * slices) threads >>= 1;
+  hipLaunchKernelGGL(c8_finalize_kernel, dim3(groups), dim3(threads), 0, (hipStream_t)stream, (const double*)partials, (double*)sums, n_slices,
+                     batchnorm ? N : 1, batchnorm ? CB : 0);
+  return ess_launch_status("norm_finalize_partials_c8");
+}
+
+extern "C" int ess_instnorm_forward_c8_sums(const void* x, const void* residual, void* y, float* stats, int32_t N, int32_t C, int32_t hw,
+                                            float eps, int32_t relu, int32_t x_f16, const void* sums, ess_stream_t stream) {
+  ESS_CHECK_ARG(x && y && stats && sums && N > 0 && C > 0 && hw > 0, "instnorm_forward_c8_sums: bad arguments");
+  ESS_CHECK_ARG(relu == 0 || relu == 1, "instnorm_forward_c8_sums: relu must be 0 or 1");
+  ESS_CHECK_ARG(al16(x, residual, y) && (((uintptr_t)sums) & 7) == 0, "instnorm_forward_c8_sums: BF16_C8 tensors must be 16-byte aligned, sums 8-byte");
+  relu = (relu & 1) | (x_f16 ? 0x100 : 0);
+  const int CB = (C + 7) / 8, groups = N * CB;
+  hipLaunchKernelGGL(in_apply_c8_kernel, dim3(groups, chunks_for8(groups, hw)), dim3(256), 0, (hipStream_t)stream, (const u32x4n*)x,
+                     (const u32x4n*)residual, (u32x4n*)y, stats, (const double*)sums, 1, CB, C, hw, eps, relu);
+  return ess_launch_status("instnorm_forward_c8_sums");
+}
+
+extern "C" int ess_instnorm_forward_c8_mixed_sums(const void* x, const void* residual, void* y, void* y16, float* stats, int32_t N, int32_t C,
+                                                  int32_t hw, float eps, int32_t relu, int32_t x_fmt, int32_t res_f16, const void* sums,
+                                                  ess_stream_t stream) {
+  ESS_CHECK_ARG(x && y16 && stats && sums && N > 0 && C > 0 && hw > 0, "instnorm_forward_c8_mixed_sums: bad arguments");
+  ESS_CHECK_ARG(relu == 0 || relu == 1, "instnorm_forward_c8_mixed_sums: relu must be 0 or 1");
+  ESS_CHECK_ARG(x_fmt == 0 || x_fmt == 1, "instnorm_forward_c8_mixed_sums: x_fmt is 0 (BF16_C8) or 1 (F16_C8); no convolution leaves sums of a [hi | lo] pair");
+  ESS_CHECK_ARG(res_f16 >= 0 && res_f16 <= 2, "instnorm_forward_c8_mixed_sums: res_f16 is 0 (BF16_C8), 1 (F16_C8) or 2 (a [hi | lo] half pair: its hi parts are added)");
+  ESS_CHECK_ARG(al16(x, residual, y, y16) && (((uintptr_t)sums) & 7) == 0, "instnorm_forward_c8_mixed_sums: C8 tensors must be 16-byte aligned, sums 8-byte");
+  const int flags = (relu & 1) | (x_fmt ? 0x100 : 0) | (res_f16 ? 0x200 : 0) | (res_f16 == 2 ? 0x800 : 0);
+  const int CB = (C + 7) / 8, groups = N * CB;
+  hipLaunchKernelGGL(in_apply_c8_mix_kernel, dim3(groups, chunks_for8(groups, hw)), dim3(256), 0, (hipStream_t)stream, (const u32x4n*)x,
+                     (const u32x4n*)residual, (u32x4n*)y, (u32x4n*)y16, stats, (const double*)sums, 1, CB, C, hw, eps, flags);
+  return ess_launch_status("instnorm_forward_c8_mixed_sums");
+}
+
+extern "C" int ess_batchnorm_train_forward_c8_sums(const void* x, const void* residual, const float* gamma, const float* beta,
+                                                   float* running_mean, float* running_var, float momentum, float eps, void* y,
+                                                   float* stats, int32_t N, int32_t C, int32_t hw, int32_t relu, int32_t x_f16,
+                                                   const void* sums, ess_stream_t stream) {
+  ESS_CHECK_ARG(x && gamma && beta && y && stats && sums && N > 0 && C > 0 && hw > 0, "batchnorm_train_forward_c8_sums: bad arguments");
+  ESS_CHECK_ARG((running_mean == nullptr) == (running_var == nullptr), "batchnorm_train_forward_c8_sums: running stats come in pairs");
+  ESS_CHECK_ARG(al16(x, residual, y) && (((uintptr_t)sums) & 7) == 0, "batchnorm_train_forward_c8_sums: BF16_C8 tensors must be 16-byte aligned, sums 8-byte");
+  relu = (relu & 1) | (x_f16 ? 0x100 : 0);
+  const int CB = (C + 7) / 8;
+  hipLaunchKernelGGL(bn_apply_c8_kernel, dim3(N * CB, chunks_for8(N * CB, hw)), dim3(256), 0, (hipStream_t)stream, (const u32x4n*)x,
+                     (const u32x4n*)residual, gamma, beta, running_mean, running_var, momentum, eps, (u32x4n*)y, stats,
+                     (const double*)sums, 1, N, CB, C, hw, relu);
+  return ess_launch_status("batchnorm_train_forward_c8_sums");
+}
diff --git a/ess_amd/functional.py b/ess_amd/functional.py
--- a/ess_amd/functional.py
+++ b/ess_amd/functional.py
@@ -216,6 +216,15 @@
 
 def half_of(x):
     return copies.of(x).h16 or (hip.bf16_c8_to_f16_c8(x.detach().contiguous()), False)
+
+
+_CONV_NORM_STATS = os.environ.get('ESS_CONV_NORM_STATS', '0')[:1] == '1'
+
+
+def _wants_stats(norm, N, Cout, hw):
+    if not _CONV_NORM_STATS or norm is None or Cout % 8:
+        return False
+    return norm == 'bn' or hip.instnorm_c8_is_split(N, Cout // 8, hw)
 
 
 def _hilo_placeholder(N, C, H, W, device, buf):
@@ -336,7 +345,7 @@
 class Conv2dFn(torch.autograd.Function):
 
     @staticmethod
-    def forward(ctx, x0, x1, weight, bias, stride, pad, mode0, mode1, passthrough=False, out_c8=None, half=False):
+    def forward(ctx, x0, x1, weight, bias, stride, pad, mode0, mode1, passthrough=False, out_c8=None, half=False, norm=None):
         c8in = hip.is_c8(x0)
         if x1 is not None and hip.is_c8(x1) != c8in:
             raise hip.EssHipError('Conv2dFn: the two sources must use the same storage format')
@@ -367,7 +376,10 @@
                 out = _hilo_placeholder(N, Cout, spec.H_out, spec.W_out, x0.device, buf)
             elif out_c8 == PRE_NORM:
                 out = hip.f16_c8_empty(N, Cout, spec.H_out, spec.W_out, x0.device)
-                hip.conv_forward_h16(fspec, h0, h1, pw, None, shift, out=out.view(torch.float16), out_fmt=hip.FMT_F16_C8)
+                ws = _wants_stats(norm, N, Cout, spec.H_out * spec.W_out)
+                r = hip.conv_forward_h16(fspec, h0, h1, pw, None, shift, out=out.view(torch.float16), out_fmt=hip.FMT_F16_C8, want_stats=ws)
+                if ws and r[1] is not None:
+                    copies.attach(out, stats=r[1])
             elif not out_c8:
                 out = torch.empty(N, Cout, spec.H_out, spec.W_out, dtype=torch.float32, device=x0.device)
                 hip.conv_forward_h16(fspec, h0, h1, pw, None, shift, out=out, out_fmt=hip.FMT_F32_NCHW)
@@ -378,8 +390,11 @@
                 out_c8 = PRE_NORM
             shift = packed_rows(spec, bias) if bias is not None else None
             out = _empty_act(N, Cout, spec.H_out, spec.W_out, x0.device, out_c8)
-            hip.conv_forward(spec, x0, x1, packed_weight(spec, weight), None, shift, out=out, src_fmt=_fmt(x0),
-                             out_fmt=hip.FMT_F16_C8 if out_c8 == PRE_NORM else _fmt(out))
+            ws = bool(out_c8 == PRE_NORM and c8in and _wants_stats(norm, N, Cout, spec.H_out * spec.W_out))
+            r = hip.conv_forward(spec, x0, x1, packed_weight(spec, weight), None, shift, out=out, src_fmt=_fmt(x0),
+                                 out_fmt=hip.FMT_F16_C8 if out_c8 == PRE_NORM else _fmt(out), want_stats=ws)
+            if ws and r[1] is not None:
+                copies.attach(out, stats=r[1])
         ctx.spec = spec
         ctx.has_x1, ctx.has_bias = x1 is not None, bias is not None
         ctx.bias_ref = weakref.ref(bias) if bias is not None else None
@@ -477,7 +492,7 @@
                     GRAD_READY_HOOK(weight)
         if d_skip is not None and need0:
             d0 = d_skip if d0 is None else (hip.add_bf16(d0, d_skip.contiguous()) if c8in else hip.add(d0, d_skip.contiguous()))
-        return d0, d1, dw, db, None, None, None, None, None, None, None
+        return d0, d1, dw, db, None, None, None, None, None, None, None, None
 
 
 def _wgrad_stride2_by_phases(x, dy, dw, db, k):
@@ -500,12 +515,12 @@
                     dw[:, :, ky, kx] = tmp[:, :, 0 if ky == 0 else 1, 0 if kx == 0 else 1]
 
 
-def conv2d(x0, weight, bias=None, stride=1, pad=0, x1=None, mode0=hip.SRC_DIRECT, mode1=hip.SRC_DIRECT, out_c8=None, half=False):
-    return Conv2dFn.apply(x0, x1, weight, bias, stride, pad, mode0, mode1, False, out_c8, half)
-
-
-def conv2d_passthrough(x0, weight, bias=None, stride=1, pad=0, out_c8=None, half=False):
-    return Conv2dFn.apply(x0, None, weight, bias, stride, pad, hip.SRC_DIRECT, hip.SRC_DIRECT, True, out_c8, half)
+def conv2d(x0, weight, bias=None, stride=1, pad=0, x1=None, mode0=hip.SRC_DIRECT, mode1=hip.SRC_DIRECT, out_c8=None, half=False, norm=None):
+    return Conv2dFn.apply(x0, x1, weight, bias, stride, pad, mode0, mode1, False, out_c8, half, norm)
+
+
+def conv2d_passthrough(x0, weight, bias=None, stride=1, pad=0, out_c8=None, half=False, norm=None):
+    return Conv2dFn.apply(x0, None, weight, bias, stride, pad, hip.SRC_DIRECT, hip.SRC_DIRECT, True, out_c8, half, norm)
 
 
 class InstanceNormFn(torch.autograd.Function):
@@ -521,13 +536,14 @@
                 h = copies.of(residual).h16
                 if h is not None:
                     res = h[0]
-            y, y16, stats = hip.instnorm_forward_c8_mixed(xin, _channels(x), res, relu, eps, x_fmt)
+            y, y16, stats = hip.instnorm_forward_c8_mixed(xin, _channels(x), res, relu, eps, x_fmt,
+                                                          conv_stats=copies.of(x).stats if x_fmt == 1 else None)
             copies.attach(y, h16=(y16, False))
             ctx.relu, ctx.x_f16 = relu, x_fmt
             ctx.save_for_backward(xin, stats)
             return y
         if _blocked(x):
-            y, stats = hip.instnorm_forward_c8(x, _channels(x), residual, relu, eps, x_f16)
+            y, stats = hip.instnorm_forward_c8(x, _channels(x), residual, relu, eps, x_f16, conv_stats=copies.of(x).stats if x_f16 else None)
         else:
             y, stats = hip.instnorm_forward(x, residual, relu, eps)
         ctx.relu, ctx.x_f16 = relu, x_f16
@@ -563,7 +579,8 @@
         ctx.x_f16 = x_f16
         if _blocked(x):
             y, stats = hip.batchnorm_train_forward_c8(x, _channels(x), residual, gamma.detach(), beta.detach(), running_mean,
-                                                      running_var, momentum, eps, relu, x_f16)
+                                                      running_var, momentum, eps, relu, x_f16,
+                                                      conv_stats=copies.of(x).stats if x_f16 else None)
         else:
             y, stats = hip.batchnorm_train_forward(x, residual, gamma.detach(), beta.detach(), running_mean, running_var,
                                                    momentum, eps, relu)
diff --git a/ess_amd/hip.py b/ess_amd/hip.py
--- a/ess_amd/hip.py
+++ b/ess_amd/hip.py
@@ -56,6 +56,8 @@
     'ess_label_confusion', 'ess_augment_perspective_filter', 'ess_tuning_set', 'ess_tuning_get', 'ess_conv2d_s2d_preferred',
     'ess_to_f16_c8', 'ess_bf16_c8_to_f16_c8', 'ess_f16_c8_to_bf16_c8', 'ess_instnorm_forward_c8_mixed', 'ess_seg_head',
     'ess_event_normalize_samples', 'ess_state_carry_masked',
+    'ess_conv2d_forward_stats', 'ess_conv2d_stats_bytes', 'ess_norm_finalize_partials_c8', 'ess_instnorm_forward_c8_sums',
+    'ess_instnorm_forward_c8_mixed_sums', 'ess_batchnorm_train_forward_c8_sums',
 ]
 
 
@@ -93,6 +95,8 @@
         L.ess_norm_workspace.argtypes = [c_int32]
         L.ess_norm_workspace_c8.restype = c_size_t
         L.ess_norm_workspace_c8.argtypes = [c_int32]
+        L.ess_conv2d_stats_bytes.restype = c_size_t
+        L.ess_conv2d_stats_bytes.argtypes = [POINTER(EssConvDesc), c_int32, c_int32, POINTER(c_int32)]
         L.ess_voxel_normalize_workspace.restype = c_size_t
         L.ess_voxel_normalize_workspace.argtypes = [c_int32]
         L.ess_voxel_grid_trilinear_workspace.restype = c_size_t
@@ -146,6 +150,11 @@
             'ess_seg_head': [P, I, P, P, P, P, P, P, I, I, I, I, I, I, I, I, I, I, I, P],
             'ess_event_normalize_samples': [P, P, I, I64, P, P, P],
             'ess_state_carry_masked': [P, P, P, I, I, P, P],
+            'ess_conv2d_forward_stats': [D, P, P, P, P, P, P, P, c_size_t, P],
+            'ess_norm_finalize_partials_c8': [P, I, I, I, I, P, c_size_t, P],
+            'ess_instnorm_forward_c8_sums': [P, P, P, P, I, I, I, F, I, I, P, P],
+            'ess_instnorm_forward_c8_mixed_sums': [P, P, P, P, P, I, I, I, F, I, I, I, P, P],
+            'ess_batchnorm_train_forward_c8_sums': [P, P, P, P, P, P, F, F, P, P, I, I, I, I, I, P, P],
         }
         for name, argtypes in sig.items():
             fn = getattr(L, name)
@@ -258,8 +267,22 @@
     return out
 
 
+def conv_stats_bytes(desc, has_scale, has_shift):
+    nsl = c_int32(0)
+    nbytes = lib().ess_conv2d_stats_bytes(byref(desc), int(bool(has_scale)), int(bool(has_shift)), byref(nsl))
+    return int(nbytes), nsl.value
+
+
+def _conv_forward_stats(desc, src0, src1, packed_w, scale, shift, out, sdt, odt, nbytes, nsl):
+    groups = desc.N * (desc.C_out // 8)
+    buf = torch.empty(nbytes // 8 + groups * 16, dtype=torch.float64, device=out.device)
+    _check(lib().ess_conv2d_forward_stats(byref(desc), ptr(src0, sdt), ptr(src1, sdt), ptr(packed_w, torch.uint8), ptr(scale), ptr(shift),
+                                          ptr(out, odt), c_void_p(buf.data_ptr()), c_size_t(nbytes), stream()), 'ess_conv2d_forward_stats')
+    return buf, nsl
+
+
 def conv_forward(spec, src0, src1, packed_w, scale=None, shift=None, residual=None, aux0=None, aux1=None, out=None,
-                 out2=None, out_bf=None, src_fmt=FMT_F32_NCHW, out_fmt=FMT_F32_NCHW, aux_fmt=FMT_F32_NCHW):
+                 out2=None, out_bf=None, src_fmt=FMT_F32_NCHW, out_fmt=FMT_F32_NCHW, aux_fmt=FMT_F32_NCHW, want_stats=False):
     if is_f16_c8(src0) or is_f16_c8(src1) or is_f16_c8(residual):
         raise EssHipError('conv_forward: an F16_C8 (pre-norm) tensor is read by the norm kernels only, not as a BF16_C8 source / residual')
     if out_fmt == FMT_F16_C8 and not is_f16_c8(out):
@@ -272,11 +295,16 @@
     u16 = spec.desc.act == GRU_U_F16 and spec.desc.epilogue in (EPI_GRU_UR, EPI_GRU_OUT)
     udt_out = torch.float16 if (u16 and spec.desc.epilogue == EPI_GRU_UR and out_fmt == FMT_F32_C8) else odt
     udt_aux = torch.float16 if (u16 and spec.desc.epilogue == EPI_GRU_OUT and res_fmt == FMT_F32_C8) else torch.float32
+    if want_stats:
+        if out_fmt == FMT_F16_C8 and residual is None and aux0 is None and aux1 is None and out2 is None and out_bf is None:
+            nbytes, nsl = conv_stats_bytes(desc, scale is not None, shift is not None)
+            if nbytes:
+                return out, _conv_forward_stats(desc, src0, src1, packed_w, scale, shift, out, sdt, odt, nbytes, nsl)
     _check(lib().ess_conv2d_forward(byref(desc), ptr(src0, sdt), ptr(src1, sdt),
                                     ptr(packed_w, torch.uint8), ptr(scale), ptr(shift), ptr(residual, rdt), ptr(aux0), ptr(aux1, udt_aux),
                                     ptr(out, udt_out), ptr(out2, odt), ptr(out_bf, torch.bfloat16), stream()),
            'ess_conv2d_forward')
-    return out
+    return (out, None) if want_stats else out
 
 
 def c8_stageable(ksize, stride, pad):
@@ -435,12 +463,33 @@
     return dx, dres
 
 
-def instnorm_forward_c8(x, C, residual, relu, eps=1e-5, x_f16=False):
+def norm_finalize_partials(conv_stats, N, C, batchnorm):
+    buf, nsl = conv_stats
+    CB = C // 8
+    npart = N * CB * nsl * 16
+    if C % 8 or buf.numel() < npart + N * CB * 16:
+        raise EssHipError('norm_finalize_partials: the buffer does not belong to a tensor of this shape')
+    sums = buf.data_ptr() + 8 * npart
+    _check(lib().ess_norm_finalize_partials_c8(c_void_p(buf.data_ptr()), N, C, nsl, int(bool(batchnorm)), c_void_p(sums),
+                                               c_size_t(8 * (buf.numel() - npart)), stream()), 'ess_norm_finalize_partials_c8')
+    return c_void_p(sums)
+
+
+def instnorm_c8_is_split(N, CB, hw):
+    return hw > 5120 and not (hw <= 1024 * 19 and N * CB >= int(os.environ.get('ESS_IN1024_MIN_GROUPS', 256)))
+
+
+def instnorm_forward_c8(x, C, residual, relu, eps=1e-5, x_f16=False, conv_stats=None):
     N, CB, H, W, _ = x.shape
     y = torch.empty(x.shape, dtype=torch.bfloat16, device=x.device)
     stats = torch.empty(N * C, 2, dtype=torch.float32, device=x.device)
     L = lib()
     xdt, xf = torch.bfloat16, int(bool(x_f16))
+    if conv_stats is not None:
+        sums = norm_finalize_partials(conv_stats, N, C, False)
+        _check(L.ess_instnorm_forward_c8_sums(ptr(x, xdt), ptr(residual, torch.bfloat16), ptr(y, torch.bfloat16), ptr(stats), N, C,
+                                              H * W, c_float(eps), int(relu), xf, sums, stream()), 'ess_instnorm_forward_c8_sums')
+        return y, stats
     ws = workspace(L.ess_norm_workspace_c8(N * CB), x.device, 'norm8')
     _check(L.ess_instnorm_forward_c8(ptr(x, xdt), ptr(residual, torch.bfloat16), ptr(y, torch.bfloat16), ptr(stats), N, C,
                                      H * W, c_float(eps), int(relu), xf, c_void_p(ws.data_ptr()), c_size_t(ws.numel()), stream()),
@@ -461,12 +510,19 @@
     return dx
 
 
-def batchnorm_train_forward_c8(x, C, residual, gamma, beta, running_mean, running_var, momentum, eps, relu, x_f16=False):
+def batchnorm_train_forward_c8(x, C, residual, gamma, beta, running_mean, running_var, momentum, eps, relu, x_f16=False, conv_stats=None):
     N, CB, H, W, _ = x.shape
     y = torch.empty(x.shape, dtype=torch.bfloat16, device=x.device)
     stats = torch.empty(2, C, 2, dtype=torch.float32, device=x.device)
     L = lib()
     xdt, xf = torch.bfloat16, int(bool(x_f16))
+    if conv_stats is not None:
+        sums = norm_finalize_partials(conv_stats, N, C, True)
+        _check(L.ess_batchnorm_train_forward_c8_sums(ptr(x, xdt), ptr(residual, torch.bfloat16), ptr(gamma), ptr(beta),
+                                                     ptr(running_mean), ptr(running_var), c_float(momentum), c_float(eps),
+                                                     ptr(y, torch.bfloat16), ptr(stats), N, C, H * W, int(relu), xf, sums, stream()),
+               'ess_batchnorm_train_forward_c8_sums')
+        return y, stats
     ws = workspace(L.ess_norm_workspace_c8(CB), x.device, 'norm8')
     _check(L.ess_batchnorm_train_forward_c8(ptr(x, xdt), ptr(residual, torch.bfloat16), ptr(gamma), ptr(beta),
                                             ptr(running_mean), ptr(running_var), c_float(momentum), c_float(eps),
@@ -895,7 +951,7 @@
 
 
 def conv_forward_h16(spec, src0, src1, packed_w, scale=None, shift=None, residual=None, aux0=None, aux1=None, out=None, out2=None,
-                     out_h16=None, out_fmt=FMT_F32_NCHW, aux_fmt=FMT_F32_NCHW, src_fp32=False):
+                     out_h16=None, out_fmt=FMT_F32_NCHW, aux_fmt=FMT_F32_NCHW, src_fp32=False, want_stats=False):
     if spec.desc.compute != COMPUTE_F16:
         raise EssHipError('conv_forward_h16: the spec was not created with compute=COMPUTE_F16')
     sdt = torch.float32 if src_fp32 else torch.float16
@@ -907,23 +963,35 @@
     u16 = (spec.desc.act & 1) == GRU_U_F16 and spec.desc.epilogue in (EPI_GRU_UR, EPI_GRU_OUT)
     udt_out = torch.float16 if (u16 and spec.desc.epilogue == EPI_GRU_UR and out_fmt == FMT_F32_C8) else odt
     udt_aux = torch.float16 if (u16 and spec.desc.epilogue == EPI_GRU_OUT and res_fmt == FMT_F32_C8) else torch.float32
+    if want_stats:
+        if out_fmt == FMT_F16_C8 and not src_fp32 and residual is None and aux0 is None and aux1 is None and out2 is None and out_h16 is None:
+            nbytes, nsl = conv_stats_bytes(desc, scale is not None, shift is not None)
+            if nbytes:
+                return out, _conv_forward_stats(desc, src0, src1, packed_w, scale, shift, out, sdt, odt, nbytes, nsl)
     _check(lib().ess_conv2d_forward(byref(desc), ptr(src0, sdt), ptr(src1, sdt), ptr(packed_w, torch.uint8), ptr(scale), ptr(shift),
                                     ptr(residual, torch.float16 if half_out else torch.float32), ptr(aux0), ptr(aux1, udt_aux),
                                     ptr(out, udt_out), ptr(out2, odt), ptr(out_h16, torch.float16), stream()), 'ess_conv2d_forward(f16)')
-    return out
-
-
-def instnorm_forward_c8_mixed(x, C, residual, relu, eps=1e-5, x_fmt=1, want_bf16=True):
+    return (out, None) if want_stats else out
+
+
+def instnorm_forward_c8_mixed(x, C, residual, relu, eps=1e-5, x_fmt=1, want_bf16=True, conv_stats=None):
     N, nb, H, W, _ = x.shape
     CB = nb // 2 if x_fmt == 2 else nb
     y = torch.empty(N, CB, H, W, 8, dtype=torch.bfloat16, device=x.device) if want_bf16 else None
     y16 = torch.empty(N, CB, H, W, 8, dtype=torch.float16, device=x.device)
     stats = torch.empty(N * C, 2, dtype=torch.float32, device=x.device)
     L = lib()
-    ws = workspace(L.ess_norm_workspace_c8(N * CB), x.device, 'norm8')
     res_f16 = 0
     if residual is not None and residual.dtype == torch.float16:
         res_f16 = 2 if residual.shape[1] == 2 * CB else 1
+    if conv_stats is not None and x_fmt != 2:
+        sums = norm_finalize_partials(conv_stats, N, C, False)
+        _check(L.ess_instnorm_forward_c8_mixed_sums(ptr(x, x.dtype), ptr(residual, residual.dtype if residual is not None else torch.float16),
+                                                    ptr(y, torch.bfloat16), ptr(y16, torch.float16), ptr(stats), N, C, H * W, c_float(eps),
+                                                    int(relu), int(x_fmt), int(res_f16), sums, stream()),
+               'ess_instnorm_forward_c8_mixed_sums')
+        return y, y16, stats
+    ws = workspace(L.ess_norm_workspace_c8(N * CB), x.device, 'norm8')
     _check(L.ess_instnorm_forward_c8_mixed(ptr(x, x.dtype), ptr(residual, residual.dtype if residual is not None else torch.float16),
                                            ptr(y, torch.bfloat16), ptr(y16, torch.float16), ptr(stats), N, C, H * W, c_float(eps),
                                            int(relu), int(x_fmt), int(res_f16), c_void_p(ws.data_ptr()), c_size_t(ws.numel()), stream()),
diff --git a/ess_amd/models/style_networks.py b/ess_amd/models/style_networks.py
--- a/ess_amd/models/style_networks.py
+++ b/ess_amd/models/style_networks.py
@@ -23,7 +23,7 @@
         c = self.model[0]
         pre = Fn.pre_norm_fmt() if hip.is_c8(x) else None
         y = Fn.conv2d(x, c.weight, c.bias, c.stride[0], c.padding[0], x1=skip,
-                      mode0=hip.SRC_NEAREST_UP2 if up else hip.SRC_DIRECT, out_c8=pre, half=True)
+                      mode0=hip.SRC_NEAREST_UP2 if up else hip.SRC_DIRECT, out_c8=pre, half=True, norm='in')
         return Fn.instance_norm(y, None, True, self.model[1].eps, x_f16=pre == Fn.PRE_NORM)
 
     def forward(self, x):
@@ -50,11 +50,11 @@
         pre1 = pre
         if first and pre == Fn.PRE_NORM and Fn.mixed() and c1.out_channels % 64 == 0:
             pre1 = Fn.PRE_NORM_HILO
-        y, skip = Fn.conv2d_passthrough(x, c1.weight, c1.bias, c1.stride[0], 1, out_c8=pre1, half=True)
+        y, skip = Fn.conv2d_passthrough(x, c1.weight, c1.bias, c1.stride[0], 1, out_c8=pre1, half=True, norm='in')
         if copies.of(skip).h16 is None:
             copies.carry(skip, x, 'h16')
         y = Fn.instance_norm(y, None, True, self.model[1].eps, x_f16=pre == Fn.PRE_NORM)
-        y = Fn.conv2d(y, c2.weight, c2.bias, 1, 1, out_c8=pre, half=True)
+        y = Fn.conv2d(y, c2.weight, c2.bias, 1, 1, out_c8=pre, half=True, norm='in')
         return Fn.instance_norm(y, skip, False, self.model[4].eps, x_f16=pre == Fn.PRE_NORM)
 
 
@@ -171,9 +171,9 @@
             pre = Fn.pre_norm_fmt()
             if passthrough:
                 y, skip = Fn.Conv2dFn.apply(x, None, conv.weight, None, conv.stride[0], conv.padding[0], hip.SRC_DIRECT,
-                                            hip.SRC_DIRECT, True, pre)
+                                            hip.SRC_DIRECT, True, pre, False, 'bn')
             else:
-                y = Fn.conv2d(x, conv.weight, None, conv.stride[0], conv.padding[0], out_c8=pre)
+                y = Fn.conv2d(x, conv.weight, None, conv.stride[0], conv.padding[0], out_c8=pre, norm='bn')
             out = Fn.batch_norm_train(y, bn.weight, bn.bias, bn.running_mean, bn.running_var, residual, relu,
                                       bn.momentum, bn.eps, x_f16=pre == Fn.PRE_NORM)
             _PENDING_BN_COUNTERS.append(bn.num_batches_tracked)
diff --git a/include/ess_hip.h b/include/ess_hip.h
--- a/include/ess_hip.h
+++ b/include/ess_hip.h
@@ -82,6 +82,10 @@
                        const float* scale, const float* shift, const void* residual, const float* aux0,
                        const float* aux1, void* out, void* out2, void* out_bf16, ess_stream_t stream);
 
+int ess_conv2d_forward_stats(const EssConvDesc* d, const void* src0, const void* src1, const void* packed_w, const float* scale,
+                             const float* shift, void* out, void* partials, size_t partials_bytes, ess_stream_t stream);
+size_t ess_conv2d_stats_bytes(const EssConvDesc* d, int32_t has_scale, int32_t has_shift, int32_t* n_slices);
+
 int ess_to_bf16_c8(const float* x, void* y, int32_t N, int32_t C, int32_t H, int32_t W, ess_stream_t stream);
 int ess_from_bf16_c8(const void* x, float* y, int32_t N, int32_t C, int32_t H, int32_t W, ess_stream_t stream);
 int ess_to_f16_c8(const float* x, void* y, int32_t N, int32_t C, int32_t H, int32_t W, int32_t hilo, ess_stream_t stream);
@@ -119,6 +123,17 @@
                                     const float* stats, void* dx, void* d_residual, float* dgamma, float* dbeta, int32_t accumulate,
                                     int32_t N, int32_t C, int32_t hw, int32_t relu, int32_t x_f16, void* workspace,
                                     size_t workspace_bytes, ess_stream_t stream);
+int ess_norm_finalize_partials_c8(const void* partials, int32_t N, int32_t C, int32_t n_slices, int32_t batchnorm, void* sums,
+                                  size_t sums_bytes, ess_stream_t stream);
+int ess_instnorm_forward_c8_sums(const void* x, const void* residual, void* y, float* stats, int32_t N, int32_t C, int32_t hw,
+                                 float eps, int32_t relu, int32_t x_f16, const void* sums, ess_stream_t stream);
+int ess_instnorm_forward_c8_mixed_sums(const void* x, const void* residual, void* y, void* y16, float* stats, int32_t N, int32_t C,
+                                       int32_t hw, float eps, int32_t relu, int32_t x_fmt, int32_t res_f16, const void* sums,
+                                       ess_stream_t stream);
+int ess_batchnorm_train_forward_c8_sums(const void* x, const void* residual, const float* gamma, const float* beta,
+                                        float* running_mean, float* running_var, float momentum, float eps, void* y, float* stats,
+                                        int32_t N, int32_t C, int32_t hw, int32_t relu, int32_t x_f16, const void* sums,
+                                        ess_stream_t stream);
 
 int ess_batchnorm_train_forward(const float* x, const float* residual, const float* gamma, const float* beta,
                                 float* running_mean, float* running_var, float momentum, float eps, float* y,
```

Result: no change. 1740 (-0.3%).
